# Coda-Research-Group/LearnedMetricIndex

Hardware: AMD Instinct MI355X
Metric: queries/sec @ recall@10, 768-d 10M index, 10k query batch (higher is better)
Workload: dtype f16 prefilter (f32 accumulate) + f32 exact re-rank; outputs identical to the all-f32 path

## Files before the change

### include/lmi_hip.h

```cpp
#ifndef LMI_HIP_H
#define LMI_HIP_H

#include <stdint.h>

#ifdef __cplusplus
extern "C" {
#endif

#define LMI_ABI_VERSION 1
#define LMI_API __attribute__((visibility("default")))
#define LMI_METRIC_IP 0
#define LMI_METRIC_L2 1
#define LMI_K_PER_BUCKET 10
#define LMI_MAX_K 64
#define LMI_MAX_LAYERS 8

typedef struct lmi_index lmi_index;

enum {
    LMI_T_INFERENCE = 0,
    LMI_T_ROUTE = 1,
    LMI_T_SCAN = 2,
    LMI_T_MERGE = 3,
    LMI_T_TOTAL = 4,
// ... 31 lines not shown
LMI_API int lmi_set_metric(lmi_index *h, int metric);

LMI_API int lmi_buckets_begin(lmi_index *h, int64_t N, int d, int L, const int64_t *labels,
                      const uint32_t *ids, const uint8_t *owned);
LMI_API int lmi_buckets_add_rows(lmi_index *h, const float *rows, int64_t row0, int64_t nrows, int on_device);
LMI_API int lmi_buckets_add_owned_rows(lmi_index *h, const float *rows, const int64_t *index, int64_t nrows,
                               int on_device);
LMI_API int lmi_buckets_end(lmi_index *h);
LMI_API int lmi_buckets_insert(lmi_index *h, const float *rows, const int64_t *labels, const uint32_t *ids, int64_t nrows,
                               int on_device, int64_t *n_stored);
LMI_API int lmi_buckets_delete(lmi_index *h, const uint32_t *ids, int64_t n, int64_t *n_removed);
LMI_API int lmi_bucket_sizes(lmi_index *h, int64_t *sizes);
LMI_API int lmi_bucket_read(lmi_index *h, int bucket, float *rows, uint32_t *ids);

LMI_API int lmi_mlp_topk(lmi_index *h, const float *queries_nav, int nq, int nb, int32_t *bucket_order,
                 float *logits, int on_device);

LMI_API int lmi_mlp_proba(lmi_index *h, const float *queries_nav, int nq, float *probs, int32_t *classes,
                  int on_device);

LMI_API int lmi_scan_topk(lmi_index *h, const float *queries_search, int nq, const int32_t *bucket_order,
                  int nb, int k, float *dists, uint32_t *ids, uint32_t *keys, int on_device);

LMI_API int lmi_search(lmi_index *h, const float *queries_nav, const float *queries_search, int nq, int nb,
               int k, float *dists, uint32_t *ids, uint32_t *keys, int32_t *bucket_order,
               int on_device);

LMI_API int lmi_merge_gathered(lmi_index *h, const float *gathered_dists, const uint32_t *gathered_ids,
                       const uint32_t *gathered_keys, int world, int64_t world_stride, int nq,
                       int kout, float *dists, uint32_t *ids, int on_device);

LMI_API int lmi_copy_out(lmi_index *h, void *dst, const void *src, int64_t bytes);
LMI_API int lmi_copy_out_many(lmi_index *h, int n, void *const *dst, const void *const *src, const int64_t *bytes);
LMI_API int lmi_pipeline_submit(lmi_index *h, void *s_in, void *s_nav, void *s_run, void *ev_in, void *ev_nav, void *ev_out,
                                const float *qn_host, const float *qs_host, float *qn_dev, float *qs_dev, int nq, int nb, int k,
                                float *dists_out, uint32_t *ids_out, int32_t *bo_dev, int32_t *bo_host, int overlap_nav);

LMI_API int lmi_comm_unique_id(void *id128);
LMI_API int lmi_comm_init(lmi_index *h, int rank, int world, const void *id128, void **comm);
LMI_API int lmi_comm_destroy(void *comm);
LMI_API int lmi_allgather_merge(lmi_index *h, void *comm, int rank, int world, const float *local_dists,
                        const uint32_t *local_ids, const uint32_t *local_keys, int nq, int kout, float *dists,
                        uint32_t *ids);

LMI_API int lmi_knn_ip(int device, const float *xq, int64_t nq, const float *xb, int64_t nb, int d, int k,
               float *D, int64_t *I);

LMI_API int lmi_timings(lmi_index *h, float *ms );
LMI_API int lmi_timings_reset(lmi_index *h);
LMI_API int lmi_set_timing(lmi_index *h, int level);
LMI_API int lmi_timings_mean(lmi_index *h, float *ms , int *n_calls );
LMI_API int lmi_scan_stats(lmi_index *h, double *flops, int64_t *pairs, int64_t *items);
LMI_API int lmi_set_prefilter(lmi_index *h, int on);
LMI_API int lmi_clone_view(lmi_index *h, lmi_index **out);
LMI_API int lmi_debug_peek(lmi_index *h, const char *name, void *dst, int64_t bytes);
LMI_API int lmi_prefilter_stats(lmi_index *h, int *active, int64_t *survivors, int64_t *fallbacks);
LMI_API int lmi_set_chunk_rows(lmi_index *h, int rows);
LMI_API int lmi_workspace_bytes(lmi_index *h, int nq, int n_buckets, int64_t *bytes);

LMI_API int lmi_debug_emit_all(lmi_index *h, int on);
LMI_API int lmi_debug_read_candidates(lmi_index *h, int64_t slot, int cap, uint32_t *rows, float *shat,
                              int *count, float *eps2, float *qscale, float *xscale);
LMI_API int lmi_debug_layout(lmi_index *h, int32_t *rb_start, int32_t *cap_rb, int64_t *n_rb_total, int64_t *alloc_rb,
                             int64_t *counters);

#ifdef __cplusplus
}
#endif
#endif
```

### learnedmetricindex_amd/_capi.py

```python
from __future__ import annotations

import ctypes
import os
from typing import Optional, Sequence

import numpy as np

_HERE = os.path.dirname(os.path.abspath(__file__))
LIB_PATH = os.environ.get("LMI_LIB") or os.path.join(_HERE, "liblmi_hip.so")
K_PER_BUCKET = 10
T_INFERENCE, T_ROUTE, T_SCAN, T_MERGE, T_TOTAL, T_PF_SAMPLE, T_PF_EMIT, T_RESCORE, T_FALLBACK, T_CLOCK_MHZ, T_COUNT = (
    0, 1, 2, 3, 4, 5, 6, 7, 8, 9, 12)

_lib = None

_f32p = ctypes.POINTER(ctypes.c_float)
_i32p = ctypes.POINTER(ctypes.c_int32)
_i64p = ctypes.POINTER(ctypes.c_int64)
_u32p = ctypes.POINTER(ctypes.c_uint32)
_u8p = ctypes.POINTER(ctypes.c_uint8)
_vp = ctypes.c_void_p

SIGNATURES = {
    "lmi_abi_version": (ctypes.c_int, []),
    "lmi_last_error": (ctypes.c_char_p, []),
    "lmi_build_info": (ctypes.c_char_p, []),
    "lmi_create": (ctypes.c_int, [ctypes.c_int, ctypes.POINTER(_vp)]),
    "lmi_destroy": (ctypes.c_int, [_vp]),
    "lmi_set_stream": (ctypes.c_int, [_vp, _vp]),
    "lmi_set_mlp": (ctypes.c_int, [_vp, ctypes.c_int, _i32p, ctypes.POINTER(_vp), ctypes.POINTER(_vp)]),
    "lmi_set_fused_mlp": (ctypes.c_int, [_vp, ctypes.c_int]),
    "lmi_set_metric": (ctypes.c_int, [_vp, ctypes.c_int]),
    "lmi_nav_set_model": (ctypes.c_int, [_vp, ctypes.c_int, ctypes.c_int, _i32p, ctypes.POINTER(_vp), ctypes.POINTER(_vp)]),
    "lmi_nav_set_tree": (ctypes.c_int, [_vp, ctypes.c_int, _vp, _vp, _vp]),
    "lmi_nav_order": (ctypes.c_int, [_vp, _vp, ctypes.c_int, ctypes.c_int, _vp, _vp, ctypes.c_int]),
    "lmi_search_tree": (ctypes.c_int, [_vp, _vp, _vp, ctypes.c_int, ctypes.c_int, ctypes.c_int, _vp, _vp, _vp, _vp, _vp, ctypes.c_int]),
    "lmi_buckets_begin": (ctypes.c_int, [_vp, ctypes.c_int64, ctypes.c_int, ctypes.c_int, _vp, _vp, _vp]),
    "lmi_buckets_add_rows": (ctypes.c_int, [_vp, _vp, ctypes.c_int64, ctypes.c_int64, ctypes.c_int]),
    "lmi_buckets_add_owned_rows": (ctypes.c_int, [_vp, _vp, _vp, ctypes.c_int64, ctypes.c_int]),
    "lmi_buckets_end": (ctypes.c_int, [_vp]),
    "lmi_buckets_insert": (ctypes.c_int, [_vp, _vp, _vp, _vp, ctypes.c_int64, ctypes.c_int, _i64p]),
    "lmi_buckets_delete": (ctypes.c_int, [_vp, _vp, ctypes.c_int64, _i64p]),
    "lmi_bucket_sizes": (ctypes.c_int, [_vp, _vp]),
    "lmi_mlp_topk": (ctypes.c_int, [_vp, _vp, ctypes.c_int, ctypes.c_int, _vp, _vp, ctypes.c_int]),
    "lmi_mlp_proba": (ctypes.c_int, [_vp, _vp, ctypes.c_int, _vp, _vp, ctypes.c_int]),
    "lmi_scan_topk": (ctypes.c_int, [_vp, _vp, ctypes.c_int, _vp, ctypes.c_int, ctypes.c_int, _vp, _vp, _vp,
                                     ctypes.c_int]),
    "lmi_search": (ctypes.c_int, [_vp, _vp, _vp, ctypes.c_int, ctypes.c_int, ctypes.c_int, _vp, _vp, _vp, _vp,
                                  ctypes.c_int]),
    "lmi_merge_gathered": (ctypes.c_int, [_vp, _vp, _vp, _vp, ctypes.c_int, ctypes.c_int64, ctypes.c_int,
                                          ctypes.c_int, _vp, _vp, ctypes.c_int]),
    "lmi_comm_unique_id": (ctypes.c_int, [_vp]),
    "lmi_comm_init": (ctypes.c_int, [_vp, ctypes.c_int, ctypes.c_int, _vp, ctypes.POINTER(_vp)]),
    "lmi_comm_destroy": (ctypes.c_int, [_vp]),
    "lmi_allgather_merge": (ctypes.c_int, [_vp, _vp, ctypes.c_int, ctypes.c_int, _vp, _vp, _vp, ctypes.c_int, ctypes.c_int,
                                           _vp, _vp]),
    "lmi_bucket_read": (ctypes.c_int, [_vp, ctypes.c_int, _vp, _vp]),
    "lmi_copy_out": (ctypes.c_int, [_vp, _vp, _vp, ctypes.c_int64]),
    "lmi_copy_out_many": (ctypes.c_int, [_vp, ctypes.c_int, _vp, _vp, _vp]),
    "lmi_pipeline_submit": (ctypes.c_int, [_vp] * 7 + [_vp, _vp, _vp, _vp, ctypes.c_int, ctypes.c_int, ctypes.c_int, _vp, _vp, _vp, _vp, ctypes.c_int]),
    "lmi_knn_ip": (ctypes.c_int, [ctypes.c_int, _vp, ctypes.c_int64, _vp, ctypes.c_int64, ctypes.c_int,
                                  ctypes.c_int, _vp, _vp]),
    "lmi_timings": (ctypes.c_int, [_vp, _vp]),
    "lmi_timings_reset": (ctypes.c_int, [_vp]),
    "lmi_set_timing": (ctypes.c_int, [_vp, ctypes.c_int]),
    "lmi_timings_mean": (ctypes.c_int, [_vp, _vp, ctypes.POINTER(ctypes.c_int)]),
    "lmi_scan_stats": (ctypes.c_int, [_vp, ctypes.POINTER(ctypes.c_double), _i64p, _i64p]),
    "lmi_set_chunk_rows": (ctypes.c_int, [_vp, ctypes.c_int]),
    "lmi_workspace_bytes": (ctypes.c_int, [_vp, ctypes.c_int, ctypes.c_int, _i64p]),
    "lmi_set_prefilter": (ctypes.c_int, [_vp, ctypes.c_int]),
    "lmi_debug_peek": (ctypes.c_int, [_vp, ctypes.c_char_p, _vp, ctypes.c_int64]),
    "lmi_clone_view": (ctypes.c_int, [_vp, ctypes.POINTER(_vp)]),
    "lmi_prefilter_stats": (ctypes.c_int, [_vp, ctypes.POINTER(ctypes.c_int), _i64p, _i64p]),
    "lmi_debug_emit_all": (ctypes.c_int, [_vp, ctypes.c_int]),
    "lmi_debug_read_candidates": (ctypes.c_int, [_vp, ctypes.c_int64, ctypes.c_int, _vp, _vp,
                                                 ctypes.POINTER(ctypes.c_int), _f32p, _f32p, _f32p]),
    "lmi_debug_layout": (ctypes.c_int, [_vp, _vp, _vp, _i64p, _i64p, _vp]),
}


class LmiError(RuntimeError):
    """Raised when a C-ABI call returns non-zero (message from lmi_last_error)."""


def lib() -> ctypes.CDLL:
    global _lib
    if _lib is None:
        if not os.path.exists(LIB_PATH):
            raise LmiError(
                f"{LIB_PATH} is missing: build it with learnedmetricindex_amd/csrc/build.sh "
                "(or __graft_entry__.build()); there is no CPU fallback")
        import torch

        L = ctypes.CDLL(LIB_PATH)
        for name, (res, args) in SIGNATURES.items():
            fn = getattr(L, name)
            fn.restype = res
            fn.argtypes = args
        if L.lmi_abi_version() != 1:
            raise LmiError("liblmi_hip.so ABI version mismatch")
        _lib = L
    return _lib


def _check(rc: int) -> None:
    if rc != 0:
        raise LmiError(lib().lmi_last_error().decode("utf-8", "replace"))


def _ptr(a) -> int:
    if a is None:
        return None
    if isinstance(a, np.ndarray):
        return a.ctypes.data
    return a.data_ptr()


def _np(a, dtype) -> np.ndarray:
    return np.ascontiguousarray(a, dtype=dtype)


class Index:

    METRICS = {"ip": 0, "l2": 1}

    def __init__(self, device: int = 0, chunk_rows: Optional[int] = None, prefilter: Optional[bool] = None,
                 metric: str = "ip"):
        self._h = _vp()
        _check(lib().lmi_create(int(device), ctypes.byref(self._h)))
        self.device = int(device)
        self.n_classes = None
        self.d_nav = None
        self.d = None
        self.L = None
        if chunk_rows is not None:
            _check(lib().lmi_set_chunk_rows(self._h, int(chunk_rows)))
        if prefilter is None and os.environ.get("LMI_PREFILTER") is not None:
            prefilter = os.environ["LMI_PREFILTER"] not in ("0", "off", "false")
        if prefilter is not None:
            self.set_prefilter(prefilter)
        if metric != "ip":
            _check(lib().lmi_set_metric(self._h, self.METRICS[metric]))
        self.metric = metric

    def close(self) -> None:
        for c in getattr(self, "_views", []):
            c.close()
        self._views = []
        if getattr(self, "_h", None) is not None and self._h:
            lib().lmi_destroy(self._h)
            self._h = None

    def clone_view(self) -> "Index":
        v = Index.__new__(Index)
        v._h = _vp()
        _check(lib().lmi_clone_view(self._h, ctypes.byref(v._h)))
        for a in ("device", "n_classes", "d_nav", "d", "L", "N", "metric"):
            setattr(v, a, getattr(self, a, None))
        v._views = []
        v._parent = self
        self.__dict__.setdefault("_views", []).append(v)
        return v

    def __del__(self):
        try:
            self.close()
        except Exception:
            pass

    def set_prefilter(self, on) -> None:
        _check(lib().lmi_set_prefilter(self._h, int(on)))

    def debug_peek(self, name: str, nbytes: int) -> np.ndarray:
        out = np.empty(nbytes, np.uint8)
        _check(lib().lmi_debug_peek(self._h, name.encode(), out.ctypes.data_as(_vp), nbytes))
        return out

    def prefilter_stats(self):
        a = ctypes.c_int(0)
        sv = ctypes.c_int64(0)
        fb = ctypes.c_int64(0)
        _check(lib().lmi_prefilter_stats(self._h, ctypes.byref(a), ctypes.byref(sv), ctypes.byref(fb)))
        return bool(a.value), sv.value, fb.value

    def debug_emit_all(self, on: bool) -> None:
        _check(lib().lmi_debug_emit_all(self._h, 1 if on else 0))

    def debug_read_candidates(self, slot: int, cap: int = 1024):
        rows = np.empty(cap, dtype=np.uint32)
        shat = np.empty(cap, dtype=np.float32)
        cnt = ctypes.c_int(0)
        e2, qs, xs = ctypes.c_float(0), ctypes.c_float(0), ctypes.c_float(0)
        _check(lib().lmi_debug_read_candidates(self._h, int(slot), int(cap), _ptr(rows), _ptr(shat), ctypes.byref(cnt),
                                               ctypes.byref(e2), ctypes.byref(qs), ctypes.byref(xs)))
        n = max(0, min(cnt.value, cap))
        return rows[:n], shat[:n], cnt.value, e2.value, qs.value, xs.value

    def debug_layout(self) -> dict:
        rb_start = np.empty(self.L + 1, dtype=np.int32)
        cap_rb = np.empty(self.L, dtype=np.int32)
        counters = np.empty(4, dtype=np.int64)
        n_rb, alloc = ctypes.c_int64(0), ctypes.c_int64(0)
        _check(lib().lmi_debug_layout(self._h, _ptr(rb_start), _ptr(cap_rb), ctypes.byref(n_rb), ctypes.byref(alloc),
                                      _ptr(counters)))
        return dict(rb_start=rb_start, cap_rb=cap_rb, n_rb_total=n_rb.value, alloc_rb=alloc.value, counters=counters)

    def set_stream(self, stream_ptr: int) -> None:
        _check(lib().lmi_set_stream(self._h, _vp(stream_ptr)))

    def set_mlp(self, layers: Sequence) -> None:
        Ws = [_np(W, np.float32) for W, _ in layers]
        bs = [_np(b, np.float32) for _, b in layers]
        dims = [Ws[0].shape[1]] + [W.shape[0] for W in Ws]
        for i, (W, b) in enumerate(zip(Ws, bs)):
            assert W.shape == (dims[i + 1], dims[i]) and b.shape == (dims[i + 1],)
        n = len(Ws)
        dims_c = (ctypes.c_int32 * (n + 1))(*dims)
        Wp = (_vp * n)(*[W.ctypes.data for W in Ws])
        bp = (_vp * n)(*[b.ctypes.data for b in bs])
        _check(lib().lmi_set_mlp(self._h, n, dims_c, Wp, bp))
        self.d_nav, self.n_classes = dims[0], dims[-1]

    def set_fused_mlp(self, mode: int) -> None:
        _check(lib().lmi_set_fused_mlp(self._h, int(mode)))

# ... 261 lines not shown
```

### learnedmetricindex_amd/csrc/lmi_front.h

```cpp
#pragma once
#include "lmi_prefilter.h"

namespace lmi {

constexpr int FR_THREADS = 1024, FR_WAVES = FR_THREADS / 64;
constexpr int FR_MAX_L = 512;
constexpr int FR_MAX_SLOTS = 1 << 17;
constexpr int FR_SLICE_G = 48;
constexpr int FR_LIST = 512;
constexpr int FP_THREADS = 512, FP_WAVES = FP_THREADS / 64;
constexpr int FR_MAX_D = 64 * 4 * 8;
static_assert(FR_SLICE_G % 2 == 0, "the 16 x 32 fragment shape pairs k16-groups");

struct FrontParams {
    const int* bucket_order;
    int nq, nb, L;
    const unsigned* epoch_dev;
    unsigned long long* gran;
    int* cb_bucket;
    int* colmap;
    RouteArrays R;
    FillRanges Z;
    const float* q;
    int d, KG16, f16x16;
    float* qnorm; float* qdelta; float* qscale;
    uint4* qfrag16;
    int* slot_col;
    float* eps2;
    const unsigned* bnorm; const unsigned* bdelta;
    float* pf_bound;
    long long ncols;
    int bound_rows;
    unsigned long long* ts;
    unsigned long long* dbg;
};
#define FR_DBG(base, slot) do { if (P.dbg && threadIdx.x == 0 && (base) >= 0) P.dbg[(base) + (slot)] = wall_clock64(); } while (0)

__host__ __device__ inline int fr_lpad(int L) { return (L + 3) & ~3; }
__host__ __device__ inline size_t fr_route_lds(int L) { return (size_t)fr_lpad(L) * 4; }
__host__ __device__ inline size_t fr_pack_lds(int L, int KG16) {
    const size_t pack = (size_t)(KG16 < FR_SLICE_G ? KG16 : FR_SLICE_G) * 1024, grp = (size_t)fr_lpad(L) * 12 + route_group_lds(L) + 16;
    return pack > grp ? pack : grp;
}

template <bool VEC>
__device__ __forceinline__ void fr_load8(const float* __restrict__ row, int d, int k0, bool ok, float (&v)[8]) {
    if constexpr (VEC) {
        const int kk = ok ? k0 : 0;
        const float4 lo = *reinterpret_cast<const float4*>(row + kk), hi = *reinterpret_cast<const float4*>(row + kk + 4);
        v[0] = ok ? lo.x : 0.0f; v[1] = ok ? lo.y : 0.0f; v[2] = ok ? lo.z : 0.0f; v[3] = ok ? lo.w : 0.0f;
        v[4] = ok ? hi.x : 0.0f; v[5] = ok ? hi.y : 0.0f; v[6] = ok ? hi.z : 0.0f; v[7] = ok ? hi.w : 0.0f;
    } else {
#pragma unroll
        for (int j = 0; j < 8; ++j) {
            const bool in = ok && k0 + j < d;
            const float x = row[in ? k0 + j : 0];
            v[j] = in ? x : 0.0f;
        }
    }
}

template <int NB, int U>
struct FrChunk {
    int id[U][NB];
    int rows[U][NB];
    __device__ __forceinline__ void load(const int* __restrict__ bo, int q_first, int lane, int q_end) {
#pragma unroll
        for (int u = 0; u < U; ++u) {
            const int q = q_first + 64 * u + lane;
            const int qq = min(q, q_end - 1);
#pragma unroll
            for (int r = 0; r < NB; ++r) id[u][r] = bo[(size_t)qq * NB + r];
        }
#pragma unroll
        for (int u = 0; u < U; ++u) {
            const bool live = q_first + 64 * u + lane < q_end;
#pragma unroll
            for (int r = 0; r < NB; ++r) id[u][r] = live ? id[u][r] : -1;
        }
    }
    __device__ __forceinline__ void sizes(const int* nbr, int L) {
// ... 207 lines not shown
        return;
    }
    const unsigned long long alloc = P.gran[P.L];
    const int n_cb = (unsigned)(alloc >> 32) == epoch_v ? (int)(unsigned)alloc : 0;
    const int cb = bid - 1;
    if (cb >= n_cb) return;
    char* stage = fp_smem;
    const int b = P.cb_bucket[cb];
    const int d = P.d, KG16 = P.KG16;
    const int nchunk_row = (d + 7) >> 3;
    constexpr int CPW = 64 / GS;
    constexpr int NCOL = (32 + FP_WAVES * CPW - 1) / (FP_WAVES * CPW);
    const int gl = lane % GS, sub = lane / GS;
    const float xn = __uint_as_float(P.bnorm[b]), dx = __uint_as_float(P.bdelta[b]);
    const float guard = norm_guard(d);
    {
        const float ninf = -INFINITY;
        const float4 f4 = make_float4(ninf, ninf, ninf, ninf);
        const long long per_row = (long long)n_cb * 8;
        const long long total = (long long)P.bound_rows * per_row;
        const long long lo = (long long)cb * P.bound_rows * 8, hi = min(total, lo + (long long)P.bound_rows * 8);
        for (long long i = lo + tid; i < hi; i += FP_THREADS) {
            const long long row = i / per_row, x = i - row * per_row;
            *reinterpret_cast<float4*>(P.pf_bound + (size_t)row * (size_t)P.ncols + (size_t)x * 4) = f4;
        }
    }
    float v[NCOL][CP][8];
    int qi[NCOL];
#pragma unroll
    for (int c = 0; c < NCOL; ++c) {
        const int cc = w * CPW + sub + c * FP_WAVES * CPW;
        qi[c] = cc < 32 ? P.colmap[(size_t)cb * 32 + cc] : -1;
    }
#pragma unroll
    for (int c = 0; c < NCOL; ++c) {
        const float* row = P.q + (size_t)(qi[c] < 0 ? 0 : qi[c]) * d;
#pragma unroll
        for (int i = 0; i < CP; ++i) {
            const int j = gl + GS * i;
            fr_load8<VEC>(row, d, 8 * j, qi[c] >= 0 && j < nchunk_row, v[c][i]);
        }
    }
#pragma unroll
    for (int c = 0; c < NCOL; ++c) {
        const int cc = w * CPW + sub + c * FP_WAVES * CPW;
        float mx = 0.0f;
#pragma unroll
        for (int i = 0; i < CP; ++i)
#pragma unroll
            for (int t = 0; t < 8; ++t) mx = fmaxf(mx, fabsf(v[c][i][t]));
#pragma unroll
        for (int o = GS / 2; o > 0; o >>= 1) mx = fmaxf(mx, __shfl_xor(mx, o));
        const float s = scale_of_max(__float_as_uint(mx));
        float acc = 0.0f, dl = 0.0f;
#pragma unroll
        for (int i = 0; i < CP; ++i)
#pragma unroll
            for (int t = 0; t < 8; ++t) {
                const float vs = v[c][i][t] * s;
                const float e = (float)(_Float16)vs - vs;
                acc += vs * vs;
                dl += e * e;
                v[c][i][t] = vs;
            }
#pragma unroll
        for (int o = GS / 2; o > 0; o >>= 1) { acc += __shfl_xor(acc, o); dl += __shfl_xor(dl, o); }
        if (gl == 0 && cc < 32) {
            const size_t col = (size_t)cb * 32 + cc;
            if (qi[c] >= 0) {
                const float qn = sqrtf(acc) * guard, dq = sqrtf(dl) * guard;
                P.qnorm[qi[c]] = qn; P.qdelta[qi[c]] = dq; P.qscale[qi[c]] = s;
                const float e = dq * (xn + dx) + qn * dx + 4.0f * (float)(KG16 * 16) * 5.96046448e-8f * (qn + dq) * (xn + dx);
                P.eps2[col] = 2.0f * e * 1.001f;
            } else {
                P.eps2[col] = 0.0f;
            }
        }
    }
    for (int g0 = 0; g0 < KG16; g0 += FR_SLICE_G) {
        const int gs = min(FR_SLICE_G, KG16 - g0);
#pragma unroll
        for (int c = 0; c < NCOL; ++c) {
            const int cc = w * CPW + sub + c * FP_WAVES * CPW;
#pragma unroll
            for (int i = 0; i < CP; ++i) {
                const int j = gl + GS * i;
                const int g = j >> 1, hh = j & 1;
                if (cc < 32 && g >= g0 && g < g0 + gs) {
                    half8 h;
#pragma unroll
                    for (int t = 0; t < 8; ++t) h[t] = (_Float16)v[c][i][t];
                    int slot;
                    if (P.f16x16) {
                        slot = (2 * (g >> 1) + (cc >> 4) - g0) * 64 + 16 * (2 * (g & 1) + hh) + (cc & 15);
                        slot ^= ((slot >> 4) & 3) | (((slot >> 7) & 3) << 2);
                    } else {
                        slot = (g - g0) * 64 + hh * 32 + cc;
                    }
                    *reinterpret_cast<uint4*>(stage + (size_t)slot * 16) = *reinterpret_cast<uint4*>(&h);
                }
            }
        }
        __syncthreads();
        uint4* dst = P.qfrag16 + ((size_t)cb * (size_t)KG16 + (size_t)g0) * 64;
        for (int i = tid; i < gs * 64; i += FP_THREADS) {
            const int src = P.f16x16 ? (i ^ (((i >> 4) & 3) | (((i >> 7) & 3) << 2))) : i;
            dst[i] = *reinterpret_cast<const uint4*>(stage + (size_t)src * 16);
        }
        __syncthreads();
    }
}
#undef FR_DBG

}
```

### learnedmetricindex_amd/csrc/lmi_hip.hip

```cpp
#include "lmi_kernels.h"
#include "lmi_prefilter.h"
#include "lmi_pass2.h"
#include "lmi_pass2_small.h"
#include "lmi_mlp_fused.h"
#include "lmi_rescore.h"
#include "lmi_front.h"
#include "lmi_tail.h"
#include "lmi_mutate.h"

#include <algorithm>
#include <cfloat>
#include <cstdarg>
#include <cstdio>
#include <cstring>
#include <dlfcn.h>
#include <mutex>
#include <string>
#include <vector>

#include "lmi_hip.h"
#include <rccl/rccl.h>

using namespace lmi;

// ... 57 lines not shown
}

struct lmi_index {
    int device = 0;
    hipStream_t stream = nullptr;
    hipStream_t side = nullptr;
    hipEvent_t side_fork = nullptr, side_join = nullptr;
    int num_cus = 256;
    int scan_blocks_per_cu = 2;

    int n_layers = 0;
    std::vector<int> dims;
    std::vector<int> n_rb;
    std::vector<int> KG;
    std::vector<DevBuf> Wf;
    std::vector<DevBuf> bias;

    struct NodeModel {
        int n_layers = 0;
        std::vector<int> dims, n_rb, KG;
        std::vector<DevBuf> Wf, bias;
    };
    std::vector<NodeModel> node_models;
    int fused_mlp = 1;
    bool desc_dirty = true;
    DevBuf d_models;
    int fm_s0 = 0, fm_s1 = 0, fm_act0 = 0, fm_lds = 0, fm_logits_lds = 0;
    bool fm_ok = false;
    std::vector<int> h_child_offset, h_child_model, h_child_bucket;
    DevBuf d_child_offset, d_child_model, d_child_bucket;
    bool tree_set = false;
    DevBuf gather_send, gather_recv;
    DevBuf pq_prob, pq_ent, pq_len, nav_len, nav_slab, nav_ent, nav_count, nav_colq, nav_active;

    bool building = false, built = false;
    int64_t N = 0;
    int d = 0, L = 0, KGs = 0;
    int metric = 0, d_user = 0;
    DevBuf aug_rows, q_aug, qn2;
    int chunk_rows = 2048;
    bool chunk_rows_auto = true;
    int64_t n_rb_total = 0;
    std::vector<int> h_nb_rows, h_rb_start, h_nch;
    DevBuf slab, ids_slab, pos, d_nb_rows, d_rb_start, d_nch;
    int64_t rows_added = 0, owned_total = 0;
    bool indexed_ingest = false;
    DevBuf stage;
    bool prefilter = true;
    bool pf_hw_ok = false;
    bool have16 = false;
    int KG16 = 0;
    int dp = 0;
    DevBuf slab16, rowmajor, xscale, xmaxbits, bnorm, bdelta, qdelta;
    DevBuf qnorm, qscale, qfrag16, eps2, cand_cnt, cand_row, cand_s, fallback, pf_bound, nkeep, surv_row, rs_flag, rs_active;
    DevBuf grp_scratch;
    bool ps_wide = false;
    int ps_force_wide = -1;
    int n_nonempty = 1;
    DevBuf x_log, x_ext, x_off, fb_list;
    unsigned x_cap = 0;
    DevBuf redo;
    size_t stamps_off = 0;
    bool pf_small = true;
    bool pf_redo = true;
    bool rescore_streamed = true;
    int last_nslots = 0, last_nb = 0;
    long long last_ncols = 0;
    bool last_fast = false;
    bool pf_qbound = true;
    bool pf_primary = true;
    bool debug_emit_all = false;

    DevBuf act[2], xfrag, logits, order, q_nav, q_srch;
    DevBuf m, cb_start, item_base, part_base, stats, head, slot_local, slot_col, colmap, qfrag, grp, col_thr;
    DevBuf part_score, part_row, rank_d, rank_id, out_d, out_id, out_key;
    static constexpr int EV_RING = 128;
    hipEvent_t ev_ring[EV_RING][10] = {};
    bool valid_ring[EV_RING][10] = {};
    int ev_cur = 0;
    int timing_level = 2;
    long long ev_calls = 0;
    hipEvent_t* ev = ev_ring[0];
    bool* ev_valid = valid_ring[0];
    long long h_stats[4] = {0, 0, 0, 0};
    bool stats_pending = false;
    DevBuf ts_ring;
    unsigned ts_mask[EV_RING] = {};
    unsigned long long* ts_set = nullptr;
    double wall_khz = 100000.0;
    DevBuf fr_dbg;
    DevBuf cb_alloc, cb_bucket;
    unsigned* h_oflag = nullptr;
    int overflow_armed = 0;
    bool fr_bump_pending = false;
    int use_tail = 1;
    bool graded_chunks = true;
    int chunk_lvl_rows[3] = {0, 0, 0};
    float chunk_frac[2] = {0.16f, 0.05f};
    bool use_front = true;

    std::vector<int> h_cap_rb;
    std::vector<unsigned char> h_owned;
    std::vector<unsigned char> h_any;
    lmi_index* parent = nullptr;
    int live_clones = 0;
    int64_t mut_paths[4] = {0, 0, 0, 0};
    DevBuf mut_pos, mut_ids, mut_list, mut_keep, mut_src, mut_stage, mut_word;
};

static int frag16x16(const lmi_index* h) { return (h->pf_small && h->KG16 <= PS_MAXKG) ? 0 : 1; }


static int set_dev(lmi_index* h) {
    HIPCHK(hipSetDevice(h->device));
    return 0;
}

extern "C" LMI_API int lmi_abi_version(void) { return LMI_ABI_VERSION; }
#ifndef LMI_SOURCE_SHA16
#define LMI_SOURCE_SHA16 "unknown"
#endif
#define LMI_STR2(x) #x
#define LMI_STR(x) LMI_STR2(x)
extern "C" LMI_API const char* lmi_build_info(void) {
    return "src=" LMI_SOURCE_SHA16 " p2_waves=" LMI_STR(LMI_P2_WAVES) " p2_bring=" LMI_STR(LMI_P2_BR) " pf_cap=" LMI_STR(LMI_PF_CAP);
}
extern "C" LMI_API const char* lmi_last_error(void) { return g_err.c_str(); }

extern "C" LMI_API int lmi_create(int device, lmi_index** out) {
    if (!out) return fail("lmi_create: out is NULL");
    int ndev = 0;
    HIPCHK(hipGetDeviceCount(&ndev));
    if (device < 0 || device >= ndev) return fail("lmi_create: device %d out of range (%d devices)", device, ndev);
    HIPCHK(hipSetDevice(device));
    hipDeviceProp_t prop;
    HIPCHK(hipGetDeviceProperties(&prop, device));
    if (std::string(prop.gcnArchName).rfind("gfx950", 0) != 0)
        return fail("lmi_create: device %d is %s; this library is built for gfx950 only", device, prop.gcnArchName);
    lmi_index* h = new lmi_index();
    h->device = device;
    h->num_cus = prop.multiProcessorCount;
    HIPCHK(hipFuncSetAttribute(reinterpret_cast<const void*>(&route_group_kernel<false>),
                               hipFuncAttributeMaxDynamicSharedMemorySize, 160 * 1024 - 256));
    int occ = 0;
    HIPCHK(hipOccupancyMaxActiveBlocksPerMultiprocessor(&occ, scan_kernel, 256, SCAN_LDS));
    h->scan_blocks_per_cu = std::max(1, std::min(occ, RB == 1 ? 2 : 1));
    {
        static std::mutex mu;
        static int cached = -1;
        std::lock_guard<std::mutex> lock(mu);
        if (cached < 0) {
            int* d_ok = nullptr;
            int ok = 0;
            HIPCHK(hipMalloc(&d_ok, sizeof(int)));
            pf_selftest_kernel<<<1, 64>>>(d_ok);
            HIPCHK(hipGetLastError());
            HIPCHK(hipMemcpy(&ok, d_ok, sizeof(int), hipMemcpyDeviceToHost));
            HIPCHK(hipFree(d_ok));
            cached = ok;
        }
        h->pf_hw_ok = cached == 1;
        if (!h->pf_hw_ok) h->prefilter = false;
    }
// ... 4 lines not shown
    if (const char* e = getenv("LMI_PF_PRIMARY")) h->pf_primary = e[0] && e[0] != '0';
    if (const char* e = getenv("LMI_PS_WIDE")) h->ps_force_wide = e[0] == '1' ? 1 : e[0] == '0' ? 0 : -1;
    if (const char* e = getenv("LMI_FRONT")) h->use_front = !(e[0] == '0');
    if (const char* e = getenv("LMI_P2_GRADED")) h->graded_chunks = !(e[0] == '0');
    if (const char* e = getenv("LMI_P2_CHUNKS")) (void)sscanf(e, "%d,%d,%d", &h->chunk_lvl_rows[0], &h->chunk_lvl_rows[1], &h->chunk_lvl_rows[2]);
    if (const char* e = getenv("LMI_P2_CHUNK_FRAC")) (void)sscanf(e, "%f,%f", &h->chunk_frac[0], &h->chunk_frac[1]);
    if (const char* e = getenv("LMI_TAIL")) h->use_tail = e[0] == '0' ? 0 : e[0] == '2' ? 2 : 1;
    if (const char* e = getenv("LMI_FR_DEBUG")) { if (e[0] == '1') { CHK(h->fr_dbg.reserve(256)); HIPCHK(hipMemset(h->fr_dbg.p, 0, 256)); } }
    {
        int khz = 0;
        if (hipDeviceGetAttribute(&khz, hipDeviceAttributeWallClockRate, device) == hipSuccess && khz > 0) h->wall_khz = (double)khz;
    }
#define LMI_PS_ATTR(K) \
    HIPCHK(hipFuncSetAttribute(reinterpret_cast<const void*>(&pass2_small_kernel<K, false, false>), hipFuncAttributeMaxDynamicSharedMemorySize, ps_lds_bytes(K, false))); \
    HIPCHK(hipFuncSetAttribute(reinterpret_cast<const void*>(&pass2_small_kernel<K, true, false>), hipFuncAttributeMaxDynamicSharedMemorySize, ps_lds_bytes(K, false))); \
    if constexpr (ps_has_wide(K)) { \
        HIPCHK(hipFuncSetAttribute(reinterpret_cast<const void*>(&pass2_small_kernel<K, false, ps_has_wide(K)>), hipFuncAttributeMaxDynamicSharedMemorySize, ps_lds_bytes(K, true))); \
        HIPCHK(hipFuncSetAttribute(reinterpret_cast<const void*>(&pass2_small_kernel<K, true, ps_has_wide(K)>), hipFuncAttributeMaxDynamicSharedMemorySize, ps_lds_bytes(K, true))); \
    }
    LMI_PS_ATTR(1) LMI_PS_ATTR(2) LMI_PS_ATTR(3) LMI_PS_ATTR(4) LMI_PS_ATTR(5) LMI_PS_ATTR(6) LMI_PS_ATTR(7) LMI_PS_ATTR(8)
#undef LMI_PS_ATTR
    HIPCHK(hipFuncSetAttribute(reinterpret_cast<const void*>(&rescore_kernel<1, false>), hipFuncAttributeMaxDynamicSharedMemorySize, 160 * 1024));
    HIPCHK(hipFuncSetAttribute(reinterpret_cast<const void*>(&rescore_kernel<1, true>), hipFuncAttributeMaxDynamicSharedMemorySize, RC_SMALL_LDS_CAP));
    HIPCHK(hipFuncSetAttribute(reinterpret_cast<const void*>(&rescore_kernel<2, false>), hipFuncAttributeMaxDynamicSharedMemorySize, 160 * 1024));
    HIPCHK(hipFuncSetAttribute(reinterpret_cast<const void*>(&rescore_kernel<2, true>), hipFuncAttributeMaxDynamicSharedMemorySize, RC_SMALL_LDS_CAP));
    HIPCHK(hipFuncSetAttribute(reinterpret_cast<const void*>(&rescore_kernel<3, false>), hipFuncAttributeMaxDynamicSharedMemorySize, 160 * 1024));
    HIPCHK(hipFuncSetAttribute(reinterpret_cast<const void*>(&rescore_kernel<3, true>), hipFuncAttributeMaxDynamicSharedMemorySize, RC_SMALL_LDS_CAP));
    HIPCHK(hipFuncSetAttribute(reinterpret_cast<const void*>(&rescore_kernel<4, false>), hipFuncAttributeMaxDynamicSharedMemorySize, 160 * 1024));
    HIPCHK(hipFuncSetAttribute(reinterpret_cast<const void*>(&rescore_kernel<4, true>), hipFuncAttributeMaxDynamicSharedMemorySize, RC_SMALL_LDS_CAP));
#define LMI_TL_ATTR(GV) \
    HIPCHK(hipFuncSetAttribute(reinterpret_cast<const void*>(&tail_kernel<GV>), hipFuncAttributeMaxDynamicSharedMemorySize, RC_SMALL_LDS_CAP));
    LMI_TL_ATTR(1) LMI_TL_ATTR(2) LMI_TL_ATTR(3) LMI_TL_ATTR(4)
#undef LMI_TL_ATTR
    *out = h;
    return 0;
}

extern "C" LMI_API int lmi_destroy(lmi_index* h) {
    if (!h) return 0;
    (void)hipSetDevice(h->device);
    (void)hipStreamSynchronize(h->stream);
    if (h->parent) h->parent->live_clones--;
    if (h->side) {
        (void)hipStreamSynchronize(h->side);
        (void)hipStreamDestroy(h->side);
        (void)hipEventDestroy(h->side_fork);
        (void)hipEventDestroy(h->side_join);
    }
    for (auto& b : h->Wf) b.release();
    for (auto& b : h->bias) b.release();
    DevBuf* bufs[] = {&h->slab, &h->ids_slab, &h->pos, &h->d_nb_rows, &h->d_rb_start, &h->d_nch, &h->stage,
                      &h->act[0], &h->act[1], &h->xfrag, &h->logits, &h->order, &h->q_nav, &h->q_srch, &h->m,
                      &h->cb_start, &h->item_base, &h->part_base, &h->stats, &h->head, &h->slot_local,
                      &h->slot_col, &h->colmap, &h->qfrag, &h->grp, &h->col_thr, &h->slab16, &h->rowmajor, &h->xscale, &h->xmaxbits, &h->bnorm, &h->bdelta, &h->qdelta, &h->qnorm, &h->qscale, &h->qfrag16, &h->eps2, &h->cand_cnt, &h->cand_row, &h->cand_s, &h->fallback, &h->pf_bound, &h->nkeep, &h->redo, &h->part_score, &h->part_row, &h->rank_d,
                      &h->rank_id, &h->out_d, &h->out_id, &h->out_key, &h->x_log, &h->x_ext, &h->x_off, &h->fb_list, &h->grp_scratch, &h->ts_ring, &h->fr_dbg, &h->cb_alloc, &h->cb_bucket};
    for (DevBuf* b : bufs) b->release();
    if (h->h_oflag) (void)hipHostFree(h->h_oflag);
    for (auto& m : h->node_models) { for (auto& b : m.Wf) b.release(); for (auto& b : m.bias) b.release(); }
    DevBuf* nav[] = {&h->d_models, &h->d_child_offset, &h->d_child_model, &h->d_child_bucket, &h->pq_prob, &h->pq_ent, &h->pq_len, &h->surv_row, &h->rs_flag, &h->rs_active, &h->gather_send, &h->gather_recv, &h->aug_rows, &h->q_aug, &h->qn2,
                     &h->nav_len, &h->nav_slab, &h->nav_ent, &h->nav_count, &h->nav_colq, &h->nav_active,
                     &h->mut_pos, &h->mut_ids, &h->mut_list, &h->mut_keep, &h->mut_src, &h->mut_stage, &h->mut_word};
    for (DevBuf* b : nav) b->release();
    for (int r = 0; r < lmi_index::EV_RING; ++r)
        for (int i = 0; i < 10; ++i)
            if (h->ev_ring[r][i]) (void)hipEventDestroy(h->ev_ring[r][i]);
    delete h;
    return 0;
}

static int build_descs(lmi_index* h);

extern "C" LMI_API int lmi_clone_view(lmi_index* h, lmi_index** out) {
    if (!h || !out) return fail("lmi_clone_view: NULL argument");
    if (h->building) return fail("lmi_clone_view: the parent's index is being built");
    CHK(set_dev(h));
    CHK(build_descs(h));
    HIPCHK(hipStreamSynchronize(h->stream));
    lmi_index* c = new lmi_index(*h);
    c->stream = nullptr; c->side = nullptr; c->side_fork = nullptr; c->side_join = nullptr;
    for (auto& b : c->Wf) b.borrow();
    for (auto& b : c->bias) b.borrow();
    for (auto& m : c->node_models) { for (auto& b : m.Wf) b.borrow(); for (auto& b : m.bias) b.borrow(); }
    DevBuf* shared[] = {&c->d_models, &c->d_child_offset, &c->d_child_model, &c->d_child_bucket, &c->slab, &c->ids_slab, &c->pos,
                        &c->d_nb_rows, &c->d_rb_start, &c->d_nch, &c->slab16, &c->rowmajor, &c->xscale, &c->xmaxbits, &c->bnorm, &c->bdelta};
    for (DevBuf* b : shared) b->borrow();
    DevBuf* own[] = {&c->gather_send, &c->gather_recv, &c->pq_prob, &c->pq_ent, &c->pq_len, &c->nav_len, &c->nav_slab, &c->nav_ent,
                     &c->nav_count, &c->nav_colq, &c->nav_active, &c->aug_rows, &c->q_aug, &c->qn2, &c->stage, &c->qdelta, &c->qnorm,
                     &c->qscale, &c->qfrag16, &c->eps2, &c->cand_cnt, &c->cand_row, &c->cand_s, &c->fallback, &c->pf_bound, &c->nkeep, &c->redo,
                     &c->surv_row, &c->rs_flag, &c->rs_active, &c->act[0], &c->act[1], &c->xfrag, &c->logits, &c->order, &c->q_nav,
                     &c->q_srch, &c->m, &c->cb_start, &c->item_base, &c->part_base, &c->stats, &c->head, &c->slot_local, &c->slot_col,
                     &c->colmap, &c->qfrag, &c->grp, &c->col_thr, &c->part_score, &c->part_row, &c->rank_d, &c->rank_id, &c->out_d,
                     &c->out_id, &c->out_key, &c->x_log, &c->x_ext, &c->x_off, &c->fb_list, &c->grp_scratch, &c->ts_ring, &c->fr_dbg, &c->cb_alloc, &c->cb_bucket,
                     &c->mut_pos, &c->mut_ids, &c->mut_list, &c->mut_keep, &c->mut_src, &c->mut_stage, &c->mut_word};
    for (DevBuf* b : own) b->forget();
    c->ts_set = nullptr;
    memset(c->ts_mask, 0, sizeof(c->ts_mask));
    c->h_oflag = nullptr;
    c->overflow_armed = 0;
    c->x_cap = 0;
    memset(c->ev_ring, 0, sizeof(c->ev_ring));
    memset(c->valid_ring, 0, sizeof(c->valid_ring));
    c->ev_cur = 0; c->ev_calls = 0;
    c->ev = c->ev_ring[0]; c->ev_valid = c->valid_ring[0];
    c->stats_pending = false;
    c->last_nslots = 0; c->last_fast = false;
    c->parent = h;
    c->live_clones = 0;
    h->live_clones++;
    *out = c;
    return 0;
}

extern "C" LMI_API int lmi_set_stream(lmi_index* h, void* s) {
    if (!h) return fail("lmi_set_stream: NULL handle");
    h->stream = reinterpret_cast<hipStream_t>(s);
    return 0;
}

extern "C" LMI_API int lmi_set_chunk_rows(lmi_index* h, int rows) {
    if (!h) return fail("lmi_set_chunk_rows: NULL handle");
    if (rows < P2_TILE_ROWS || rows % P2_TILE_ROWS) return fail("lmi_set_chunk_rows: rows must be a positive multiple of %d", P2_TILE_ROWS);
    if (h->building || h->built) return fail("lmi_set_chunk_rows: must be called before lmi_buckets_begin");
    h->chunk_rows = rows;
    h->chunk_rows_auto = false;
    return 0;
}

extern "C" LMI_API int lmi_set_metric(lmi_index* h, int metric) {
    if (!h) return fail("lmi_set_metric: NULL handle");
    if (metric != LMI_METRIC_IP && metric != LMI_METRIC_L2) return fail("lmi_set_metric: unknown metric %d", metric);
    if ((h->built || h->building) && metric != h->metric) return fail("lmi_set_metric: the metric is fixed once lmi_buckets_begin has run");
    h->metric = metric;
    return 0;
}

extern "C" LMI_API int lmi_set_prefilter(lmi_index* h, int on) {
    if (!h) return fail("lmi_set_prefilter: NULL handle");
    if ((h->built || h->building) && (on != 0) != h->prefilter)
        return fail("lmi_set_prefilter: the mode is fixed once lmi_buckets_begin has run (the index is stored differently)");
    if (on && !h->pf_hw_ok) return fail("lmi_set_prefilter: fp16 subnormal self-test failed on this device; the prefilter's error bound does not hold");
    if (on != 0 && on != 1) return fail("lmi_set_prefilter: mode %d unknown (0: all-f32 scan, 1: fp16 prefilter + exact re-rank)", on);
    h->prefilter = on != 0;
    return 0;
}

static int pack_from_host(lmi_index* h, const float* src, int rows, int cols, int n_rb, int KG, DevBuf& dst) {
    CHK(h->stage.reserve((size_t)rows * cols * sizeof(float)));
    HIPCHK(hipMemcpyAsync(h->stage.p, src, (size_t)rows * cols * sizeof(float), hipMemcpyHostToDevice, h->stream));
    CHK(dst.reserve((size_t)n_rb * KG * 1024));
    long long total = (long long)n_rb * 32 * KG;
    pack_gather_kernel<<<cdiv(total, 256), 256, 0, h->stream>>>(h->stage.as<float>(), cols, nullptr, rows,
                                                               (long long)n_rb * 32, KG, dst.as<float4>());
    HIPCHK(hipGetLastError());
    HIPCHK(hipStreamSynchronize(h->stream));
    return 0;
}

static int pack_model(lmi_index* h, const char* who, int n_layers, const int* dims, const float* const* W, const float* const* b,
                      std::vector<int>& o_dims, std::vector<int>& o_nrb, std::vector<int>& o_KG, std::vector<DevBuf>& o_W,
                      std::vector<DevBuf>& o_b) {
    if (n_layers < 1 || n_layers > LMI_MAX_LAYERS) return fail("%s: n_layers %d out of range", who, n_layers);
    for (int i = 0; i <= n_layers; ++i)
        if (dims[i] < 1) return fail("%s: dims[%d] = %d", who, i, dims[i]);
    for (auto& x : o_W) x.release();
    for (auto& x : o_b) x.release();
    o_dims.assign(dims, dims + n_layers + 1);
    o_nrb.assign(n_layers, 0);
    o_KG.assign(n_layers, 0);
    o_W.assign(n_layers, DevBuf());
    o_b.assign(n_layers, DevBuf());
    for (int i = 0; i < n_layers; ++i) {
        o_nrb[i] = cdiv(dims[i + 1], 32);
        o_KG[i] = (i == 0) ? cdiv(dims[0], 8) : o_nrb[i - 1] * 4;
        if (!W[i] || !b[i]) return fail("%s: NULL weight/bias for layer %d", who, i);
        CHK(pack_from_host(h, W[i], dims[i + 1], dims[i], o_nrb[i], o_KG[i], o_W[i]));
        std::vector<float> bp((size_t)o_nrb[i] * 32, 0.0f);
        std::copy(b[i], b[i] + dims[i + 1], bp.begin());
        CHK(o_b[i].reserve(bp.size() * sizeof(float)));
        HIPCHK(hipMemcpy(o_b[i].p, bp.data(), bp.size() * sizeof(float), hipMemcpyHostToDevice));
    }
    return 0;
}

extern "C" LMI_API int lmi_set_mlp(lmi_index* h, int n_layers, const int* dims, const float* const* W,
                           const float* const* b) {
    if (!h) return fail("lmi_set_mlp: NULL handle");
    CHK(set_dev(h));
    h->desc_dirty = true;
// ... 235 lines not shown
            augment_copy_kernel<<<cdiv((long long)n * h->d, 256), 256, 0, h->stream>>>(src, h->d_user, h->d, n, h->aug_rows.as<float>());
            HIPCHK(hipGetLastError());
            augment_norm_kernel<<<cdiv(n, 256), 256, 0, h->stream>>>(src, h->d_user, h->d, n, h->aug_rows.as<float>(), nullptr);
            HIPCHK(hipGetLastError());
            src = h->aug_rows.as<float>();
        }
        if (h->prefilter) {
            long long total = (long long)n * h->d;
            scatter_rows_kernel<<<cdiv(total, 256), 256, 0, h->stream>>>(src, h->d, pos, row0 + off, idx, (long long)n_total, n,
                                                                        h->rowmajor.as<float>(), h->dp);
        } else {
            long long total = (long long)n * h->KGs;
            pack_scatter_kernel<<<cdiv(total, 256), 256, 0, h->stream>>>(src, h->d, pos, row0 + off, idx, (long long)n_total, n,
                                                                        h->KGs, h->slab.as<float4>());
        }
        HIPCHK(hipGetLastError());
        if (!on_device) HIPCHK(hipStreamSynchronize(h->stream));
    }
    return 0;
}

extern "C" LMI_API int lmi_buckets_add_rows(lmi_index* h, const float* rows, int64_t row0, int64_t nrows, int on_device) {
    if (!h || !h->building) return fail("lmi_buckets_add_rows: call lmi_buckets_begin first");
    if (h->indexed_ingest) return fail("lmi_buckets_add_rows: this build already uses lmi_buckets_add_owned_rows");
    if (row0 < 0 || nrows < 0 || row0 + nrows > h->N) return fail("lmi_buckets_add_rows: rows [%lld,%lld) outside [0,%lld)", (long long)row0, (long long)(row0 + nrows), (long long)h->N);
    if (nrows == 0) return 0;
    CHK(add_rows_impl(h, rows, row0, nullptr, nrows, on_device, h->pos.as<int>(), h->N));
    h->rows_added += nrows;
    return 0;
}

extern "C" LMI_API int lmi_buckets_add_owned_rows(lmi_index* h, const float* rows, const int64_t* index, int64_t nrows,
                                          int on_device) {
    if (!h || !h->building) return fail("lmi_buckets_add_owned_rows: call lmi_buckets_begin first");
    if (h->rows_added > 0 && !h->indexed_ingest) return fail("lmi_buckets_add_owned_rows: this build already uses lmi_buckets_add_rows");
    if (nrows < 0 || (nrows > 0 && (!rows || !index))) return fail("lmi_buckets_add_owned_rows: bad arguments");
    if (!on_device)
        for (int64_t i = 0; i < nrows; ++i)
            if (index[i] < 0 || index[i] >= h->N) return fail("lmi_buckets_add_owned_rows: index[%lld] = %lld outside [0,%lld)", (long long)i, (long long)index[i], (long long)h->N);
    h->indexed_ingest = true;
    if (nrows == 0) return 0;
    CHK(add_rows_impl(h, rows, 0, index, nrows, on_device, h->pos.as<int>(), h->N));
    h->rows_added += nrows;
    return 0;
}

static int prefilter_images(lmi_index* h) {
    h->KG16 = (h->pf_small && cdiv(h->d, 16) <= PS_MAXKG) ? (int)cdiv(h->d, 16) : (int)rup(cdiv(h->d, 16), PF_STAGE_G);
    const long long n_rows = (long long)h->n_rb_total * 32;
    CHK(h->xmaxbits.reserve(16));
    CHK(h->xscale.reserve(16));
    CHK(h->bnorm.reserve((size_t)h->L * 4));
    CHK(h->bdelta.reserve((size_t)h->L * 4));
    CHK(h->slab16.reserve((size_t)h->n_rb_total * h->KG16 * 1024 + 8192));
    HIPCHK(hipMemsetAsync(h->xmaxbits.p, 0, 16, h->stream));
    HIPCHK(hipMemsetAsync(h->bnorm.p, 0, (size_t)h->L * 4, h->stream));
    HIPCHK(hipMemsetAsync(h->bdelta.p, 0, (size_t)h->L * 4, h->stream));
    absmax_kernel<<<h->num_cus * 8, 256, 0, h->stream>>>(h->rowmajor.as<float>(), n_rows * h->dp, h->xmaxbits.as<unsigned>());
    HIPCHK(hipGetLastError());
    make_scale_kernel<<<1, 1, 0, h->stream>>>(h->xmaxbits.as<unsigned>(), h->xscale.as<float>());
    HIPCHK(hipGetLastError());
    const long long total = n_rows * h->KG16 * 2;
    convert16_kernel<<<cdiv(total, 256), 256, 0, h->stream>>>(h->rowmajor.as<float>(), h->d, h->dp, n_rows, h->KG16,
                                                             h->xscale.as<float>(), h->slab16.as<uint4>(), frag16x16(h));
    HIPCHK(hipGetLastError());
    dim3 g(64, h->L);
    bucket_norm_kernel<<<g, 256, 0, h->stream>>>(h->rowmajor.as<float>(), h->d, h->dp, h->d_rb_start.as<int>(),
                                                h->d_nb_rows.as<int>(), h->xscale.as<float>(), h->bnorm.as<unsigned>(),
                                                h->bdelta.as<unsigned>());
    HIPCHK(hipGetLastError());
    HIPCHK(hipStreamSynchronize(h->stream));
    h->have16 = true;
    return 0;
}

extern "C" LMI_API int lmi_buckets_end(lmi_index* h) {
    if (!h || !h->building) return fail("lmi_buckets_end: call lmi_buckets_begin first");
    const int64_t expect = h->indexed_ingest ? h->owned_total : h->N;
    if (h->rows_added != expect) return fail("lmi_buckets_end: %lld of %lld rows were added", (long long)h->rows_added, (long long)expect);
    CHK(set_dev(h));
    HIPCHK(hipStreamSynchronize(h->stream));
    h->pos.release();
    h->have16 = false;
    if (h->prefilter && h->n_rb_total > 0) CHK(prefilter_images(h));
    h->building = false;
    h->built = true;
    return 0;
}

extern "C" LMI_API int lmi_bucket_sizes(lmi_index* h, int64_t* sizes) {
    if (!h || !(h->built || h->building)) return fail("lmi_bucket_sizes: no buckets");
    for (int b = 0; b < h->L; ++b) sizes[b] = h->h_nb_rows[b];
    return 0;
}

extern "C" LMI_API int lmi_bucket_read(lmi_index* h, int bucket, float* rows, uint32_t* ids) {
    if (!h || !h->built) return fail("lmi_bucket_read: the bucket index is not built");
    if (bucket < 0 || bucket >= h->L) return fail("lmi_bucket_read: bucket %d outside [0,%d)", bucket, h->L);
    const int64_t n = h->h_nb_rows[bucket];
    if (n == 0) return 0;
    CHK(set_dev(h));
    const int64_t p0 = (int64_t)h->h_rb_start[bucket] * 32;
    const int du = h->d_user;
    if (rows && h->prefilter) {
        HIPCHK(hipMemcpy2DAsync(rows, (size_t)du * 4, h->rowmajor.as<float>() + (size_t)p0 * h->dp, (size_t)h->dp * 4, (size_t)du * 4, (size_t)n,
                                hipMemcpyDeviceToHost, h->stream));
    } else if (rows) {
        CHK(h->stage.reserve((size_t)n * du * 4));
        long long total = n * cdiv(du, 8);
        unpack_kernel<<<cdiv(total, 256), 256, 0, h->stream>>>(h->slab.as<float4>(), h->KGs, p0, n, du, h->stage.as<float>());
        HIPCHK(hipGetLastError());
        HIPCHK(hipMemcpyAsync(rows, h->stage.p, (size_t)n * du * 4, hipMemcpyDeviceToHost, h->stream));
    }
    if (ids) HIPCHK(hipMemcpyAsync(ids, h->ids_slab.as<uint32_t>() + p0, (size_t)n * 4, hipMemcpyDeviceToHost, h->stream));
    HIPCHK(hipStreamSynchronize(h->stream));
    return 0;
}

namespace {
struct SlabImage { DevBuf* buf; size_t rb_bytes, extra; };
int slab_images(lmi_index* h, SlabImage* im) {
    int n = 0;
// ... 173 lines not shown
    HIPCHK(hipGetLastError());
    CHK(add_rows_impl(h, rows, 0, nullptr, nrows, on_device, h->mut_pos.as<int>(), nrows));
    std::vector<int> list((size_t)L * 5);
    int* l_b = list.data();
    int* l_row0 = l_b + L;
    int* l_nrows = l_row0 + L;
    int* l_rb0 = l_nrows + L;
    int* l_nrb = l_rb0 + L;
    int nr = 0, max_rows = 0, max_rb = 0;
    for (int b = 0; b < L; ++b) {
        if (!add[b]) continue;
        const int r0 = start[b] * 32 + h->h_nb_rows[b], r1 = r0 + (int)add[b];
        l_b[nr] = b;
        l_row0[nr] = r0;
        l_nrows[nr] = r1 - r0;
        l_rb0[nr] = r0 / 32;
        l_nrb[nr] = cdiv(r1, 32) - r0 / 32;
        max_rows = std::max(max_rows, l_nrows[nr]);
        max_rb = std::max(max_rb, l_nrb[nr]);
        ++nr;
        h->h_nb_rows[b] += (int)add[b];
        h->h_any[b] = 1;
    }
    for (int64_t i = 0; i < nrows; ++i) h->h_any[labels[i]] = 1;
    h->N += nrows;
    CHK(mut_derive(h));
    if (h->prefilter) {
        HIPCHK(hipMemcpyAsync(h->mut_list.p, list.data(), list.size() * 4, hipMemcpyHostToDevice, h->stream));
        const int* d_list = h->mut_list.as<int>();
        bool rescale = !h->have16;
        if (!rescale) {
            HIPCHK(hipMemsetAsync(h->mut_word.p, 0, 4, h->stream));
            dim3 g(std::min(64, cdiv((long long)max_rows * h->d, 256)), nr);
            absmax_ranges_kernel<<<g, 256, 0, h->stream>>>(h->rowmajor.as<float>(), h->d, h->dp, d_list + L, d_list + 2 * L, h->mut_word.as<unsigned>());
            HIPCHK(hipGetLastError());
            unsigned mbits = 0;
            float sc = 1.0f;
            HIPCHK(hipMemcpyAsync(&mbits, h->mut_word.p, 4, hipMemcpyDeviceToHost, h->stream));
            HIPCHK(hipMemcpyAsync(&sc, h->xscale.p, 4, hipMemcpyDeviceToHost, h->stream));
            HIPCHK(hipStreamSynchronize(h->stream));
            float m;
            memcpy(&m, &mbits, 4);
            rescale = !(m * sc < 1.0f);
        }
        if (rescale) {
            CHK(prefilter_images(h));
        } else {
            dim3 gc(std::min(1024, cdiv((long long)max_rb * 32 * h->KG16 * 2, 256)), nr);
            convert16_ranges_kernel<<<gc, 256, 0, h->stream>>>(h->rowmajor.as<float>(), h->d, h->dp, d_list + 3 * L, d_list + 4 * L, h->KG16,
                                                               h->xscale.as<float>(), h->slab16.as<uint4>(), frag16x16(h));
            HIPCHK(hipGetLastError());
            dim3 gn(std::min(64, cdiv(max_rows, 256)), nr);
            bucket_norm_ranges_kernel<<<gn, 256, 0, h->stream>>>(h->rowmajor.as<float>(), h->d, h->dp, d_list, d_list + L, d_list + 2 * L,
                                                                  h->xscale.as<float>(), h->bnorm.as<unsigned>(), h->bdelta.as<unsigned>());
            HIPCHK(hipGetLastError());
        }
    }
    HIPCHK(hipStreamSynchronize(h->stream));
    for (int i = 0; i < 4; ++i) h->mut_paths[i] += paths[i];
    if (n_stored) *n_stored = stored;
    return 0;
}

extern "C" LMI_API int lmi_buckets_delete(lmi_index* h, const uint32_t* ids, int64_t n, int64_t* n_removed) {
    CHK(mut_check(h, "lmi_buckets_delete"));
    if (n < 0 || (n > 0 && !ids)) return fail("lmi_buckets_delete: bad arguments");
    if (n_removed) *n_removed = 0;
    if (n == 0 || h->owned_total == 0) return 0;
    std::vector<uint32_t> del(ids, ids + n);
    std::sort(del.begin(), del.end());
    del.erase(std::unique(del.begin(), del.end()), del.end());
    const int L = h->L;
    const int64_t slab_rows = h->n_rb_total * 32;
    CHK(set_dev(h));
    CHK(h->mut_ids.reserve(del.size() * 4));
    CHK(h->mut_keep.reserve((size_t)slab_rows * 4));
    CHK(h->mut_src.reserve((size_t)slab_rows * 4));
    CHK(h->mut_word.reserve((size_t)L * 4));
    CHK(h->mut_list.reserve((size_t)L * 4 * 4 + (size_t)L * 8 + 16));
    CHK(h->mut_pos.reserve((size_t)L * 5 * 4));
    HIPCHK(hipStreamSynchronize(h->stream));
    HIPCHK(hipMemcpyAsync(h->mut_ids.p, del.data(), del.size() * 4, hipMemcpyHostToDevice, h->stream));
    HIPCHK(hipMemsetAsync(h->mut_word.p, 0, (size_t)L * 4, h->stream));
    int max_n = 0;
    for (int b = 0; b < L; ++b) max_n = std::max(max_n, h->h_nb_rows[b]);
    mark_deleted_kernel<<<dim3(std::max(1, std::min(64, cdiv(max_n, 256))), L), 256, 0, h->stream>>>(
        h->ids_slab.as<uint32_t>(), h->d_rb_start.as<int>(), h->d_nb_rows.as<int>(), h->mut_ids.as<uint32_t>(), (int)del.size(),
        h->mut_keep.as<int>(), h->mut_word.as<int>());
    HIPCHK(hipGetLastError());
    std::vector<int> cnt(L);
    HIPCHK(hipMemcpyAsync(cnt.data(), h->mut_word.p, (size_t)L * 4, hipMemcpyDeviceToHost, h->stream));
    HIPCHK(hipStreamSynchronize(h->stream));
    std::vector<int> hit, span;
    int64_t removed = 0, max_span = 0;
    for (int b = 0; b < L; ++b)
        if (cnt[b] > 0) {
            hit.push_back(b);
            span.push_back(cdiv(h->h_nb_rows[b], 32) * 32);
            max_span = std::max<int64_t>(max_span, span.back());
            removed += cnt[b];
        }
    if (removed == 0) return 0;
    const int nh = (int)hit.size();
    const bool frag = !h->prefilter;
    const int pitch = frag ? h->d : h->dp;
    const int64_t budget = std::max<int64_t>(max_span, (1ll << 30) / ((int64_t)pitch * 4));
    std::vector<int> gb, gspan, gfirst;
// ... 27 lines not shown
    const int* d_hit = h->mut_list.as<int>();
    const long long* d_goff = reinterpret_cast<const long long*>(h->mut_list.as<char>() + off_bytes);
    compact_map_kernel<<<nh, CM_THREADS, 0, h->stream>>>(d_hit, d_hit + nh, h->d_rb_start.as<int>(), h->d_nb_rows.as<int>(), h->mut_keep.as<int>(),
                                                        h->mut_src.as<int>());
    HIPCHK(hipGetLastError());
    const int per_row = frag ? cdiv(pitch, 8) : pitch / 4;
    for (size_t g = 0; g + 1 < gfirst.size(); ++g) {
        const int i0 = gfirst[g], ng = gfirst[g + 1] - i0;
        int64_t gmax = 0;
        for (int i = i0; i < i0 + ng; ++i) gmax = std::max<int64_t>(gmax, gspan[i]);
        dim3 gg(std::max(1, std::min(1024, cdiv(gmax * per_row, 256))), ng);
        if (frag)
            gather_compact_kernel<true><<<gg, 256, 0, h->stream>>>(h->slab.as<float>(), pitch, h->KGs, h->ids_slab.as<uint32_t>(), d_hit + 2 * nh + i0,
                                                                  d_goff + i0, d_hit + 3 * nh + i0, h->d_rb_start.as<int>(), h->mut_src.as<int>(), st_rows, st_ids);
        else
            gather_compact_kernel<false><<<gg, 256, 0, h->stream>>>(h->rowmajor.as<float>(), pitch, 0, h->ids_slab.as<uint32_t>(), d_hit + 2 * nh + i0,
                                                                   d_goff + i0, d_hit + 3 * nh + i0, h->d_rb_start.as<int>(), h->mut_src.as<int>(), st_rows, st_ids);
        HIPCHK(hipGetLastError());
        for (int i = i0; i < i0 + ng; ++i) {
            const int b = gb[i];
            const size_t p0 = (size_t)h->h_rb_start[b] * 32;
            const long long sp = gspan[i], off = goff[i];
            if (frag) {
                pack_gather_kernel<<<cdiv(sp * h->KGs, 256), 256, 0, h->stream>>>(st_rows + off * pitch, pitch, nullptr, (int)sp, sp, h->KGs,
                                                                                  h->slab.as<float4>() + (p0 >> 5) * h->KGs * 64);
                HIPCHK(hipGetLastError());
            } else {
                HIPCHK(hipMemcpyAsync(h->rowmajor.as<float>() + p0 * pitch, st_rows + off * pitch, (size_t)sp * pitch * 4, hipMemcpyDeviceToDevice, h->stream));
            }
            HIPCHK(hipMemcpyAsync(h->ids_slab.as<uint32_t>() + p0, st_ids + off, (size_t)sp * 4, hipMemcpyDeviceToDevice, h->stream));
        }
    }
    std::vector<int> old_nrb(nh);
    for (int i = 0; i < nh; ++i) {
        const int b = hit[i];
        old_nrb[i] = span[i] / 32;
        h->h_nb_rows[b] -= cnt[b];
        if (h->h_nb_rows[b] == 0) h->h_any[b] = 0;
    }
    h->N -= removed;
    CHK(mut_derive(h));
    std::vector<int> list((size_t)5 * nh);
    if (h->prefilter && h->have16) {
        for (int i = 0; i < nh; ++i) {
            const int b = hit[i];
            list[i] = b;
            list[nh + i] = h->h_rb_start[b] * 32;
            list[2 * nh + i] = h->h_nb_rows[b];
            list[3 * nh + i] = h->h_rb_start[b];
            list[4 * nh + i] = old_nrb[i];
        }
        HIPCHK(hipMemcpyAsync(h->mut_pos.p, list.data(), list.size() * 4, hipMemcpyHostToDevice, h->stream));
        const int* d_list = h->mut_pos.as<int>();
        reset_norms_kernel<<<cdiv(nh, 256), 256, 0, h->stream>>>(d_list, nh, h->bnorm.as<unsigned>(), h->bdelta.as<unsigned>());
        HIPCHK(hipGetLastError());
        int max_rb = 0, max_rows = 1;
        for (int i = 0; i < nh; ++i) { max_rb = std::max(max_rb, old_nrb[i]); max_rows = std::max(max_rows, list[2 * nh + i]); }
        dim3 gc(std::max(1, std::min(1024, cdiv((long long)max_rb * 32 * h->KG16 * 2, 256))), nh);
        convert16_ranges_kernel<<<gc, 256, 0, h->stream>>>(h->rowmajor.as<float>(), h->d, h->dp, d_list + 3 * nh, d_list + 4 * nh, h->KG16,
                                                           h->xscale.as<float>(), h->slab16.as<uint4>(), frag16x16(h));
        HIPCHK(hipGetLastError());
        dim3 gn(std::min(64, cdiv(max_rows, 256)), nh);
        bucket_norm_ranges_kernel<<<gn, 256, 0, h->stream>>>(h->rowmajor.as<float>(), h->d, h->dp, d_list, d_list + nh, d_list + 2 * nh,
                                                              h->xscale.as<float>(), h->bnorm.as<unsigned>(), h->bdelta.as<unsigned>());
        HIPCHK(hipGetLastError());
    }
    HIPCHK(hipStreamSynchronize(h->stream));
    if (n_removed) *n_removed = removed;
    return 0;
}

static void begin_call(lmi_index* h) {
    h->ev_cur = (h->ev_cur + 1) % lmi_index::EV_RING;
    h->ev = h->ev_ring[h->ev_cur];
    h->ev_valid = h->valid_ring[h->ev_cur];
    for (int i = 0; i < 10; ++i) h->ev_valid[i] = false;
    ++h->ev_calls;
    h->ts_mask[h->ev_cur] = 0u;
    h->ts_set = nullptr;
    if (h->timing_level == 2) {
        if (!h->ts_ring.p && h->ts_ring.reserve((size_t)lmi_index::EV_RING * ST_COUNT * 8) != 0) return;
        h->ts_set = h->ts_ring.as<unsigned long long>() + (size_t)h->ev_cur * ST_COUNT;
    }
}
static unsigned long long* tsp(lmi_index* h, int idx) {
    if (!h->ts_set) return nullptr;
    h->ts_mask[h->ev_cur] |= 1u << idx;
    return h->ts_set + idx;
}
static int stamp_end(lmi_index* h, int idx) {
    if (unsigned long long* p = tsp(h, idx)) {
        stamp_kernel<<<1, 1, 0, h->stream>>>(p);
        HIPCHK(hipGetLastError());
    }
    return 0;
}

static int record(lmi_index* h, int i) {
    if (h->timing_level == 0 || h->timing_level == 2 || (h->timing_level == 1 && i != 0 && i != 1 && i != 4)) return 0;
    if (!h->ev[i]) HIPCHK(hipEventCreateWithFlags(&h->ev[i], hipEventDisableSystemFence));
    HIPCHK(hipEventRecord(h->ev[i], h->stream));
    h->ev_valid[i] = true;
    return 0;
}

static int input_ptr(lmi_index* h, const void* src, size_t bytes, int on_device, DevBuf& buf, const void** out) {
    if (on_device) { *out = src; return 0; }
    CHK(buf.reserve(bytes));
    HIPCHK(hipMemcpyAsync(buf.p, src, bytes, hipMemcpyHostToDevice, h->stream));
    *out = buf.p;
    return 0;
}

static int side_ensure(lmi_index* h) {
    if (!h->side) {
        HIPCHK(hipStreamCreateWithFlags(&h->side, hipStreamNonBlocking));
        HIPCHK(hipEventCreateWithFlags(&h->side_fork, hipEventDisableTiming));
// ... 233 lines not shown
    CHK(h->part_score.reserve((size_t)part_lists * KPB * 4));
    CHK(h->part_row.reserve((size_t)part_lists * KPB * 4));
    CHK(h->rank_d.reserve((size_t)nslots * KPB * 4));
    CHK(h->rank_id.reserve((size_t)nslots * KPB * 4));

    RouteArrays R;
    R.nb_rows = h->d_nb_rows.as<int>();
    R.nch = h->d_nch.as<int>();
    R.m = h->m.as<int>();
    R.m0 = R.m + L;
    R.cb_start = h->cb_start.as<int>();
    R.item_base = h->item_base.as<int>();
    R.part_base = h->part_base.as<long long>();
    R.stats = h->stats.as<long long>();
    R.grp_bucket = h->grp.as<int>();
    R.grp_base = R.grp_bucket + (size_t)NGRP * L;
    R.grp_n = R.grp_base + (size_t)NGRP * (L + 1);
    R.grp_total = R.grp_n + NGRP;
    R.grp_base1 = R.grp_total + NGRP;
    R.grp_total1 = R.grp_base1 + (size_t)NGRP * (L + 1);
    R.dbg = nullptr;
    const bool v2 = h->prefilter && h->have16;
    R.chunk_rb = h->chunk_rows / 32;
    R.chunk_rb_b = (v2 && h->graded_chunks) ? R.grp_total1 + NGRP : nullptr;
    {
        const int base = h->chunk_rows;
        int rows[3] = {base, base / 2, base / 4};
        if (h->pf_small && h->KG16 <= PS_MAXKG) rows[0] = 2 * base;
        for (int i = 0; i < 3; ++i) {
            if (h->chunk_lvl_rows[i] > 0) rows[i] = h->chunk_lvl_rows[i];
            rows[i] = std::max(P2_TILE_ROWS, rows[i] / P2_TILE_ROWS * P2_TILE_ROWS);
            R.chunk_lvl[i] = rows[i] / 32;
        }
        R.chunk_frac[0] = h->chunk_frac[0];
        R.chunk_frac[1] = h->chunk_frac[1];
    }
    h->ps_wide = false;
    if (v2 && h->pf_small && h->KG16 <= PS_MAXKG) {
        const double per_bucket = (double)nq * nb / std::max(1, std::min(h->n_nonempty, (int)std::min<long long>((long long)nq * nb, 1 << 30)));
        h->ps_wide = h->ps_force_wide >= 0 ? h->ps_force_wide != 0 : ps_use_wide(h->KG16, per_bucket);
    }
    R.tile_cb = !v2 ? 4 : (h->pf_small && h->KG16 <= PS_MAXKG) ? ps_tile_cb(h->KG16, h->ps_wide) : P2_MAXCB;
    R.sample_max = (v2 && h->pf_small && h->KG16 <= PF_SAMPLE_LOWD_KG) ? PF_SAMPLE_LOWD : PF_SAMPLE;
    R.sample_items = v2 ? 1 : 0;
    const bool qbound = v2 && h->pf_qbound && nb > 1 && kout <= KPB;
    R.primary_nb = (qbound && h->pf_primary) ? nb : 0;

    const size_t ncols = (size_t)ncb_bound * 32;
    FillRanges Z;
    Z.count = 0;
    bool fill_ok = true;
    auto fill = [&](void* ptr, long long words, unsigned value) { fill_ok = Z.add(ptr, words, value) && fill_ok; };
    const bool use_front = fast && h->use_front && L <= FR_MAX_L && nslots <= FR_MAX_SLOTS && h->d <= FR_MAX_D;
    if (!use_front) fill(h->m.p, 3ll * L, 0u);
    fill(h->head.p, 64, 0u);
    if (!use_front) fill(h->colmap.p, (long long)ncols, 0xFFFFFFFFu);
    fill(h->col_thr.p, (long long)ncols, 0xFF800000u );
    if (fast) {
        CHK(h->qnorm.reserve((size_t)nq * 4));
        CHK(h->qdelta.reserve((size_t)nq * 4));
        CHK(h->qscale.reserve((size_t)nq * 4));
        CHK(h->qfrag16.reserve((size_t)ncb_bound * h->KG16 * 1024 + 8192));
        CHK(h->eps2.reserve(ncols * 4));
        CHK(h->cand_cnt.reserve(ncols * 4));
        CHK(h->cand_row.reserve(ncols * PF_CAP * 4));
        CHK(h->cand_s.reserve(ncols * PF_CAP * 4));
        CHK(h->fallback.reserve((size_t)nslots * 4));
        CHK(h->nkeep.reserve((size_t)nslots * 4));
        const size_t bound_words = ncols * P2_NSL * 16;
        CHK(h->pf_bound.reserve(bound_words * 4 + 4096));
        if (!use_front) fill(h->pf_bound.p, (long long)bound_words, 0xFF800000u );
        fill(h->cand_cnt.p, (long long)ncols, 0u);
        fill(h->stats.as<long long>() + 2, 4, 0u);
        CHK(h->redo.reserve((size_t)(1 + L) * 4 + ncols));
        fill(h->redo.p, (long long)(1 + L) + (long long)((ncols + 3) / 4), 0u);
        CHK(h->fb_list.reserve((size_t)(8 + nslots) * 4));
        fill(h->fb_list.p, 8, 0u);
        if (h->x_cap == 0) {
            const size_t cap = (size_t)1 << LMI_PF_X_LOG2;
            CHK(h->x_log.reserve(cap * 16));
            CHK(h->x_ext.reserve(cap * 8));
            h->x_cap = (unsigned)cap;
        }
        CHK(h->x_off.reserve(ncols * 4));
        if (rescore_is_streamed(h)) {
            const int groups = nslots / rescore_group_size(nb), sub_cap = cdiv(groups, RC_SUB);
            CHK(h->rs_flag.reserve((size_t)groups * 4));
            CHK(h->rs_active.reserve((size_t)(RC_SUB + RC_SUB * sub_cap) * 4 + (size_t)(1 + groups) * 4));
            fill(h->rs_flag.p, groups, 0u);
            fill(h->rs_active.p, RC_SUB, 0u);
            fill(h->rs_active.as<int>() + RC_SUB + RC_SUB * sub_cap, 1, 0u);
        }
    }
    if (!fill_ok) return fail("internal: more than %d fill ranges queued (%s:%d)", FillRanges::MAXR, __FILE__, __LINE__);
    Z.ts = nullptr;
    if (!use_front) {
    Z.ts = tsp(h, ST_FRONT);
    fill_ranges_kernel<<<h->num_cus * 4, 256, 0, h->stream>>>(Z);
    HIPCHK(hipGetLastError());
    route_count_kernel<<<cdiv(nslots, 256), 256, 0, h->stream>>>(d_order, nslots, L, R, h->slot_local.as<int>());
    HIPCHK(hipGetLastError());
    route_scan_kernel<<<1, 256, 0, h->stream>>>(L, R);
    HIPCHK(hipGetLastError());
    CHK(side_fork(h));
    if (L <= ROUTE_MAX_BUCKETS) {
        route_group_kernel<false><<<1, 1024, route_group_lds(L), h->side>>>(L, R, nullptr);
    } else {
        CHK(h->grp_scratch.reserve(route_group_lds(L) + (size_t)L * 4));
        route_group_kernel<true><<<1, 1024, 0, h->side>>>(L, R, h->grp_scratch.as<char>());
    }
    HIPCHK(hipGetLastError());
    route_fill_kernel<<<cdiv(nslots, 256), 256, 0, h->stream>>>(d_order, h->slot_local.as<int>(), nslots, nb,
                                                               R.cb_start, R.m0, h->colmap.as<int>(), h->slot_col.as<int>());
    HIPCHK(hipGetLastError());
    }
    ScanParams S;
// ... 13 lines not shown
    S.grp_total = R.grp_total;
    S.part_base = R.part_base;
    S.head = h->head.as<unsigned>();
    S.col_thr = h->col_thr.as<float>();
    S.part_score = h->part_score.as<float>();
    S.part_row = h->part_row.as<unsigned>();
    S.ts_start = nullptr;
    S.ts_end_cell = nullptr;
    unsigned long long* const p2_end_cell = reinterpret_cast<unsigned long long*>(h->head.as<unsigned>() + 32);
    unsigned long long* const scan_end_cell = reinterpret_cast<unsigned long long*>(h->head.as<unsigned>() + 34);
    if (!fast) {
        long long total = ncb_bound * 32 * h->KGs;
        pack_gather_kernel<<<cdiv(total, 256), 256, 0, h->stream>>>(d_qs, h->d, h->colmap.as<int>(), nq, ncb_bound * 32,
                                                                   h->KGs, h->qfrag.as<float4>());
        HIPCHK(hipGetLastError());
        CHK(side_join(h));
        CHK(record(h, 2));
        S.ts_start = tsp(h, ST_SCAN0);
        if (S.ts_start) { S.ts_end_cell = scan_end_cell; (void)tsp(h, ST_SCAN1); }
        scan_kernel<<<h->num_cus * h->scan_blocks_per_cu, 256, SCAN_LDS, h->stream>>>(S);
        HIPCHK(hipGetLastError());
        CHK(record(h, 3));
    } else {
        if (use_front) {
            FrontParams A;
            A.bucket_order = d_order;
            A.nq = nq; A.nb = nb; A.L = L;
            if (!h->cb_alloc.p) {
                CHK(h->cb_alloc.reserve((size_t)(FR_MAX_L + 2) * 8));
                HIPCHK(hipMemsetAsync(h->cb_alloc.p, 0, (size_t)(FR_MAX_L + 2) * 8, h->stream));
                front_epoch_bump_kernel<<<1, 1, 0, h->stream>>>(reinterpret_cast<unsigned*>(h->cb_alloc.as<unsigned long long>() + FR_MAX_L + 1));
                HIPCHK(hipGetLastError());
            }
            CHK(h->cb_bucket.reserve((size_t)ncb_bound * 4));
            unsigned* const epoch_dev = reinterpret_cast<unsigned*>(h->cb_alloc.as<unsigned long long>() + FR_MAX_L + 1);
            if (h->fr_bump_pending) {
                front_epoch_bump_kernel<<<1, 1, 0, h->stream>>>(epoch_dev);
                HIPCHK(hipGetLastError());
            }
            h->fr_bump_pending = true;
            A.epoch_dev = epoch_dev;
            A.gran = h->cb_alloc.as<unsigned long long>();
            A.cb_bucket = h->cb_bucket.as<int>();
            A.colmap = h->colmap.as<int>();
            A.R = R;
            A.R.dbg = h->fr_dbg.as<unsigned long long>();
            A.Z = Z;
            A.q = d_qs;
            A.d = h->d; A.KG16 = h->KG16; A.f16x16 = frag16x16(h);
            A.qnorm = h->qnorm.as<float>(); A.qdelta = h->qdelta.as<float>(); A.qscale = h->qscale.as<float>();
            A.qfrag16 = h->qfrag16.as<uint4>();
            A.slot_col = h->slot_col.as<int>();
            A.eps2 = h->eps2.as<float>();
            A.bnorm = h->bnorm.as<unsigned>(); A.bdelta = h->bdelta.as<unsigned>();
            A.pf_bound = h->pf_bound.as<float>();
            A.ncols = (long long)ncols;
            A.bound_rows = P2_NSL * 16;
            A.ts = tsp(h, ST_FRONT);
            A.dbg = h->fr_dbg.as<unsigned long long>();
            const size_t rlds = fr_route_lds(L);
            switch (nb) {
#define LMI_FR_CASE(NBV) case NBV: route_kernel<NBV><<<L, FR_THREADS, rlds, h->stream>>>(A); break;
                LMI_FR_CASE(1) LMI_FR_CASE(2) LMI_FR_CASE(3) LMI_FR_CASE(4) LMI_FR_CASE(5) LMI_FR_CASE(6) LMI_FR_CASE(8) LMI_FR_CASE(10) LMI_FR_CASE(16)
#undef LMI_FR_CASE
                default: route_kernel<0><<<L, FR_THREADS, rlds, h->stream>>>(A); break;
            }
            HIPCHK(hipGetLastError());
            A.ts = nullptr;
            const int pgrid = 1 + (int)ncb_bound;
            const size_t plds = fr_pack_lds(L, h->KG16);
            const int nchunk = (h->d + 7) / 8;
            const bool vec = h->d % 8 == 0;
#define LMI_FP_LAUNCH(GSV, CPV) { if (vec) pack_kernel<GSV, CPV, true><<<pgrid, FP_THREADS, plds, h->stream>>>(A); \
                                  else pack_kernel<GSV, CPV, false><<<pgrid, FP_THREADS, plds, h->stream>>>(A); }
            if (nchunk <= 8) LMI_FP_LAUNCH(8, 1)
            else if (nchunk <= 16) LMI_FP_LAUNCH(16, 1)
            else if (nchunk <= 32) LMI_FP_LAUNCH(32, 1)
            else if (nchunk <= 64) LMI_FP_LAUNCH(64, 1)
            else if (nchunk <= 128) LMI_FP_LAUNCH(64, 2)
            else LMI_FP_LAUNCH(64, 4)
#undef LMI_FP_LAUNCH
            HIPCHK(hipGetLastError());
        } else {
        query_norm_kernel<<<cdiv(nq, 4), 256, 0, h->stream>>>(d_qs, nq, h->d, h->qnorm.as<float>(), h->qdelta.as<float>(),
                                                              h->qscale.as<float>());
        HIPCHK(hipGetLastError());
        {
            long long total = (long long)ncols * h->KG16 * 2;
            pack_queries16_kernel<<<cdiv(total, 256), 256, 0, h->stream>>>(d_qs, h->d, h->colmap.as<int>(), (long long)ncols,
                                                                          h->KG16, h->qscale.as<float>(), h->qfrag16.as<uint4>(), frag16x16(h));
            HIPCHK(hipGetLastError());
        }
        slot_bound_kernel<<<cdiv(nslots, 256), 256, 0, h->stream>>>(d_order, h->slot_col.as<int>(), nslots, nb, h->KG16 * 16,
                                                                   h->qnorm.as<float>(), h->qdelta.as<float>(),
                                                                   h->bnorm.as<unsigned>(), h->bdelta.as<unsigned>(), h->eps2.as<float>());
        HIPCHK(hipGetLastError());
        CHK(side_join(h));
        }
        CHK(record(h, 2));
        PrefilterParams F;
        F.slab16 = h->slab16.as<uint4>();
        F.qfrag16 = h->qfrag16.as<uint4>();
        F.KG16 = h->KG16;
        F.L = L;
        F.chunk_rb = S.chunk_rb;
        F.chunk_rb_b = R.chunk_rb_b;
        F.tile_cb = R.tile_cb;
        F.sample_max = R.sample_max;
        F.rb_start = S.rb_start;
        F.nb_rows = R.nb_rows;
        F.nch = R.nch;
        F.m = R.m;
        F.m0 = R.m0;
        F.cb_start = R.cb_start;
        F.grp_bucket = R.grp_bucket;
        F.grp_base = R.grp_base;
        F.grp_n = R.grp_n;
        F.grp_total = R.grp_total;
        F.grp_base1 = R.grp_base1;
        F.grp_total1 = R.grp_total1;
        F.ncols = (long long)ncols;
        F.head = S.head;
        F.bound = h->pf_bound.as<float>();
        F.bound1 = S.col_thr;
        F.eps2 = h->eps2.as<float>();
        F.cand_cnt = h->cand_cnt.as<unsigned>();
        F.cand_row = h->cand_row.as<unsigned>();
        F.cand_s = h->cand_s.as<float>();
        F.redo_count = nullptr; F.redo_bucket = nullptr; F.redo_col = nullptr;
        unsigned* fbw = h->fb_list.as<unsigned>();
        F.x.log = h->x_log.as<uint4>();
        F.x.cap = h->x_cap;
        F.x.head = fbw + 3;
        F.x.fail = fbw + 1;
        F.x.launch = 0;
        h->stamps_off = (ncols * P2_NSL * 16 * 4 + 255) / 256 * 256;
        F.stamps = reinterpret_cast<unsigned long long*>(static_cast<char*>(h->pf_bound.p) + h->stamps_off);
        F.ts_start = tsp(h, ST_P1);
        F.ts_end_cell = nullptr;
#if defined(LMI_P2_STAMPS)
        HIPCHK(hipMemsetAsync(F.stamps, 0, 2 * 8 * 12 * 8, h->stream));
#endif
        {
            CHK(launch_pass2<true>(h, F));
            bound_merge2_kernel<<<cdiv((long long)ncols, 64), 256, 0, h->stream>>>(F.bound, (long long)ncols, F.bound1,
                use_front ? reinterpret_cast<unsigned*>(h->cb_alloc.as<unsigned long long>() + FR_MAX_L + 1) : nullptr);
            HIPCHK(hipGetLastError());
            h->fr_bump_pending = false;
            if (qbound) {
                query_bound_kernel<<<cdiv(nq, 256), 256, 0, h->stream>>>(h->slot_col.as<int>(), nq, nb, F.eps2, F.bound1);
                HIPCHK(hipGetLastError());
            }
        }
        if (h->debug_emit_all) {
            FillRanges D;
            D.count = 1; D.p[0] = reinterpret_cast<unsigned*>(F.bound1); D.n[0] = (long long)ncols; D.v[0] = 0xFF800000u; D.ts = nullptr;
            fill_ranges_kernel<<<h->num_cus * 4, 256, 0, h->stream>>>(D);
            HIPCHK(hipGetLastError());
        }
        CHK(record(h, 5));

        F.ts_start = tsp(h, ST_P2);
        F.ts_end_cell = F.ts_start ? p2_end_cell : nullptr;
        if (F.ts_start) { (void)tsp(h, ST_CLK_WALL); (void)tsp(h, ST_CLK_CYC); }
        CHK(launch_pass2<false>(h, F));
        F.ts_start = nullptr;
        F.ts_end_cell = nullptr;
        CHK(record(h, 6));
        use_tail = rescore_is_streamed(h) && h->use_tail && (rescore_group_size(nb) == nb || h->use_tail == 2) &&
                   RC_WAVES * tail_wave_lds(h->dp, rescore_group_size(nb), true) <= RC_SMALL_LDS_CAP;
        tail_merges = use_tail && rescore_group_size(nb) == nb;
        if (use_tail && !h->h_oflag) {
            HIPCHK(hipHostMalloc(reinterpret_cast<void**>(&h->h_oflag), 64, hipHostMallocMapped));
            *h->h_oflag = 0u;
        }
        if (use_tail && *reinterpret_cast<volatile unsigned*>(h->h_oflag) != 0u) { h->overflow_armed = 1000; *h->h_oflag = 0u; }
        const bool overflow_sorted = h->pf_redo && !h->debug_emit_all && (!use_tail || h->overflow_armed > 0);
        if (use_tail && h->overflow_armed > 0) --h->overflow_armed;
        if (overflow_sorted) {
            unsigned* rc = h->redo.as<unsigned>();
            int* rb = reinterpret_cast<int*>(rc + 1);
            unsigned char* rcol = reinterpret_cast<unsigned char*>(rc + 1 + L);
            overflow_rebound_kernel<<<cdiv(nslots, 256), 256, 0, h->stream>>>(h->slot_col.as<int>(), d_order, nslots, F.cand_cnt, F.cand_s,
                                                                             F.bound1, rc, rb, rcol, F.x.fail, F.x.cap, h->x_off.as<unsigned>(), fbw + 4);
            HIPCHK(hipGetLastError());
            PrefilterParams F2 = F;
            F2.x.cap = 0;
            F2.x.fail = fbw + 2;
            F2.x.launch = 1;
            F2.head = F.head + 16;
            F2.redo_count = rc; F2.redo_bucket = rb; F2.redo_col = rcol;
            CHK(launch_pass2<false>(h, F2));
        }
        RescoreParams Q;
        Q.bucket_order = d_order;
        Q.slot_col = h->slot_col.as<int>();
        Q.nslots = nslots;
        Q.nb = nb;
        Q.d = h->d;
        Q.raw = raw;
        Q.rb_start = S.rb_start;
        Q.nb_rows = R.nb_rows;
        Q.cand_cnt = F.cand_cnt;
        Q.cand_row = F.cand_row;
        Q.cand_s = F.cand_s;
        Q.eps2 = F.eps2;
        Q.rows = h->rowmajor.as<float>();
        Q.dp = h->dp;
        Q.q = d_qs;
        Q.qn2 = d_qn2;
        Q.ids_slab = h->ids_slab.as<unsigned>();
        Q.rank_d = h->rank_d.as<float>();
        Q.rank_id = h->rank_id.as<unsigned>();
        Q.fallback = h->fallback.as<int>();
        Q.nkeep = h->nkeep.as<int>();
        Q.fb_count = reinterpret_cast<int*>(fbw);
        Q.fb_list = reinterpret_cast<int*>(fbw + 8);
        const bool sorted_overflow = overflow_sorted;
        Q.x_fail = fbw + 1;
        Q.x_off = sorted_overflow ? h->x_off.as<unsigned>() : nullptr;
        Q.x_ext = h->x_ext.as<uint2>();
        Q.x_log = F.x.log;
        Q.x_head = F.x.head;
        Q.x_cap = F.x.cap;
        Q.redo_col = sorted_overflow ? reinterpret_cast<const unsigned char*>(h->redo.as<unsigned>() + 1 + L) : nullptr;
        Q.ts = h->ts_set;
        Q.p2_end = p2_end_cell;
        if (Q.ts) { (void)tsp(h, ST_TAIL); (void)tsp(h, ST_P2END); (void)tsp(h, ST_FB); }
        Q.merge_pending = nullptr; Q.m_kout = 0; Q.m_out_d = nullptr; Q.m_out_id = nullptr; Q.m_out_key = nullptr;
        Q.host_oflag = use_tail ? h->h_oflag : nullptr;
#ifndef LMI_ABL_NOEMIT
        if (use_tail) {
            const int G = rescore_group_size(nb), groups = nslots / G;
            CHK(h->surv_row.reserve((size_t)nslots * RC_KEEP * 4));
            const int sub_cap = cdiv(groups, RC_SUB);
            SelectOut O;
            O.surv_row = h->surv_row.as<unsigned>();
            O.G = G;
            O.grp_flag = nullptr;
            O.active = h->rs_active.as<int>();
            O.sub_cap = sub_cap;
            O.big = O.active + RC_SUB + RC_SUB * sub_cap;
            TailParams T;
            T.ngroups = groups; T.merge = tail_merges ? 1 : 0; T.kout = kout;
// ... 723 lines not shown
    if (cap_rb) std::copy(h->h_cap_rb.begin(), h->h_cap_rb.end(), cap_rb);
    if (n_rb_total) *n_rb_total = h->n_rb_total;
    if (alloc) *alloc = alloc_rb(h);
    if (counters) std::copy(h->mut_paths, h->mut_paths + 4, counters);
    return 0;
}

extern "C" LMI_API int lmi_debug_read_candidates(lmi_index* h, int64_t slot, int cap, uint32_t* rows, float* shat,
                                         int* count, float* eps2, float* qscale, float* xscale) {
    if (!h) return fail("lmi_debug_read_candidates: NULL handle");
    if (!h->last_fast) return fail("lmi_debug_read_candidates: the last scan did not use the prefilter");
    if (slot < 0 || slot >= h->last_nslots) return fail("lmi_debug_read_candidates: slot outside the last scan's %d", h->last_nslots);
    CHK(set_dev(h));
    HIPCHK(hipStreamSynchronize(h->stream));
    int col = -1;
    HIPCHK(hipMemcpy(&col, h->slot_col.as<int>() + slot, 4, hipMemcpyDeviceToHost));
    unsigned cnt = 0;
    float e2 = 0.0f, qs = 1.0f, xs[2] = {1.0f, 1.0f};
    if (col >= 0) {
        HIPCHK(hipMemcpy(&cnt, h->cand_cnt.as<unsigned>() + col, 4, hipMemcpyDeviceToHost));
        HIPCHK(hipMemcpy(&e2, h->eps2.as<float>() + col, 4, hipMemcpyDeviceToHost));
        HIPCHK(hipMemcpy(&qs, h->qscale.as<float>() + slot / h->last_nb, 4, hipMemcpyDeviceToHost));
        HIPCHK(hipMemcpy(xs, h->xscale.p, 8, hipMemcpyDeviceToHost));
        const unsigned n = std::min<unsigned>(std::min<unsigned>(cnt, (unsigned)PF_CAP), (unsigned)std::max(cap, 0));
        if (n && rows) HIPCHK(hipMemcpy(rows, h->cand_row.as<unsigned>() + (size_t)col * PF_CAP, (size_t)n * 4, hipMemcpyDeviceToHost));
        if (n && shat) HIPCHK(hipMemcpy(shat, h->cand_s.as<float>() + (size_t)col * PF_CAP, (size_t)n * 4, hipMemcpyDeviceToHost));
    }
    if (count) *count = col >= 0 ? (int)cnt : -1;
    if (eps2) *eps2 = e2;
    if (qscale) *qscale = qs;
    if (xscale) *xscale = xs[0];
    return 0;
}

extern "C" LMI_API int lmi_debug_peek(lmi_index* h, const char* name, void* dst, int64_t bytes) {
    if (!h || !name || !dst) return fail("lmi_debug_peek: NULL argument");
    CHK(set_dev(h));
    HIPCHK(hipStreamSynchronize(h->stream));
    DevBuf* b = nullptr;
    size_t off = 0;
    if (!strcmp(name, "pf_bound")) b = &h->pf_bound;
    if (!strcmp(name, "fr_dbg")) b = &h->fr_dbg;
    if (!strcmp(name, "pf_stamps")) { b = &h->pf_bound; off = h->stamps_off; }
    if (!strcmp(name, "cand_total")) {
        if (bytes != 8 || !h->last_fast) return fail("lmi_debug_peek: cand_total is 8 bytes after a prefilter scan");
        unsigned long long* d_acc = reinterpret_cast<unsigned long long*>(h->stats.as<long long>() + 2);
        HIPCHK(hipMemsetAsync(d_acc, 0, 8, h->stream));
        sum_u32_kernel<<<64, 256, 0, h->stream>>>(h->cand_cnt.as<unsigned>(), h->last_ncols, d_acc);
        HIPCHK(hipGetLastError());
        HIPCHK(hipStreamSynchronize(h->stream));
        HIPCHK(hipMemcpy(dst, d_acc, 8, hipMemcpyDeviceToHost));
        return 0;
    }
    if (!strcmp(name, "pf_redo")) b = &h->redo;
    if (!strcmp(name, "pf_fallback")) b = &h->fb_list;
    if (!b) return fail("lmi_debug_peek: unknown buffer '%s'", name);
    if (bytes < 0 || off + (size_t)bytes > b->cap) return fail("lmi_debug_peek: %lld bytes asked of a %zu-byte buffer", (long long)bytes, b->cap);
    if (bytes) HIPCHK(hipMemcpy(dst, static_cast<char*>(b->p) + off, (size_t)bytes, hipMemcpyDeviceToHost));
    return 0;
}

extern "C" LMI_API int lmi_scan_stats(lmi_index* h, double* flops, int64_t* pairs, int64_t* items) {
    if (!h) return fail("lmi_scan_stats: NULL handle");
    CHK(set_dev(h));
    if (h->stats_pending) {
        HIPCHK(hipStreamSynchronize(h->stream));
        HIPCHK(hipMemcpy(h->h_stats, h->stats.p, 32, hipMemcpyDeviceToHost));
        h->stats_pending = false;
    }
    if (pairs) *pairs = h->h_stats[0];
    if (items) *items = h->h_stats[1];
    if (flops) *flops = 2.0 * h->d * (double)h->h_stats[0];
    return 0;
}
```

### learnedmetricindex_amd/csrc/lmi_mutate.h

```cpp
#pragma once
#include "lmi_prefilter.h"

namespace lmi {

__global__ void scatter_ids_kernel(const uint32_t* __restrict__ ids, const int* __restrict__ pos, long long n,
                                   uint32_t* __restrict__ ids_slab) {
    const long long i = (long long)blockIdx.x * blockDim.x + threadIdx.x;
    if (i >= n) return;
    const int p = pos[i];
    if (p >= 0) ids_slab[p] = ids[i];
}


__global__ void absmax_ranges_kernel(const float* __restrict__ rows, int d, int pitch, const int* __restrict__ row0,
                                     const int* __restrict__ nrows, unsigned* __restrict__ out) {
    const int r = blockIdx.y;
    const long long n = (long long)nrows[r] * d;
    const float* x = rows + (size_t)row0[r] * pitch;
    float m = 0.0f;
    for (long long i = (long long)blockIdx.x * blockDim.x + threadIdx.x; i < n; i += (long long)gridDim.x * blockDim.x) {
        const long long row = i / d;
        m = fmaxf(m, fabsf(x[row * pitch + (i - row * d)]));
    }
#pragma unroll
    for (int o = 32; o > 0; o >>= 1) m = fmaxf(m, __shfl_xor(m, o));
    if ((threadIdx.x & 63) == 0) atomicMax(out, __float_as_uint(m));
}

__global__ void convert16_ranges_kernel(const float* __restrict__ rows, int d, int pitch, const int* __restrict__ rb0,
                                        const int* __restrict__ nrb, int KG16, const float* __restrict__ scale,
                                        uint4* __restrict__ dst, int f16x16) {
    const int r = blockIdx.y;
    const long long p0 = (long long)rb0[r] * 32;
    const long long n = (long long)nrb[r] * 32 * KG16 * 2;
    const float s = scale[0];
    for (long long idx = (long long)blockIdx.x * blockDim.x + threadIdx.x; idx < n; idx += (long long)gridDim.x * blockDim.x)
        convert16_one(rows, d, pitch, p0 + (idx >> 1) / KG16, (int)((idx >> 1) % KG16), (int)(idx & 1), KG16, s, dst, f16x16);
}

__global__ void bucket_norm_ranges_kernel(const float* __restrict__ rows, int d, int pitch, const int* __restrict__ bucket,
                                          const int* __restrict__ row0, const int* __restrict__ nrows,
                                          const float* __restrict__ scale, unsigned* __restrict__ bnorm_bits,
                                          unsigned* __restrict__ bdelta_bits) {
    const int r = blockIdx.y;
    const float s = scale[0];
    const float guard = norm_guard(d);
    float best = 0.0f, bestd = 0.0f;
    for (int row = blockIdx.x * blockDim.x + threadIdx.x; row < nrows[r]; row += gridDim.x * blockDim.x)
        row_norms(rows + ((size_t)row0[r] + row) * pitch, d, s, guard, best, bestd);
    if (best > 0.0f) atomicMax(bnorm_bits + bucket[r], __float_as_uint(best));
    if (bestd > 0.0f) atomicMax(bdelta_bits + bucket[r], __float_as_uint(bestd));
}

__global__ void reset_norms_kernel(const int* __restrict__ bucket, int n, unsigned* __restrict__ bnorm_bits,
                                   unsigned* __restrict__ bdelta_bits) {
    const int i = blockIdx.x * blockDim.x + threadIdx.x;
    if (i >= n) return;
    bnorm_bits[bucket[i]] = 0u;
    bdelta_bits[bucket[i]] = 0u;
}

__global__ void mark_deleted_kernel(const uint32_t* __restrict__ ids_slab, const int* __restrict__ rb_start,
                                    const int* __restrict__ nb_rows, const uint32_t* __restrict__ del, int n_del,
                                    int* __restrict__ keep, int* __restrict__ removed) {
    const int b = blockIdx.y;
    const int n_b = nb_rows[b];
    const size_t base = (size_t)rb_start[b] * 32;
    int cnt = 0;
    for (int row = blockIdx.x * blockDim.x + threadIdx.x; row < n_b; row += gridDim.x * blockDim.x) {
        const uint32_t id = ids_slab[base + row];
        int lo = 0, hi = n_del;
        while (lo < hi) {
            const int mid = (lo + hi) >> 1;
            if (del[mid] < id) lo = mid + 1;
            else hi = mid;
        }
        const int hit = lo < n_del && del[lo] == id;
        keep[base + row] = !hit;
        cnt += hit;
    }
#pragma unroll
    for (int o = 32; o > 0; o >>= 1) cnt += __shfl_xor(cnt, o);
    if ((threadIdx.x & 63) == 0 && cnt) atomicAdd(removed + b, cnt);
}

constexpr int CM_THREADS = 1024;
__global__ __launch_bounds__(CM_THREADS) void compact_map_kernel(const int* __restrict__ hit, const int* __restrict__ span,
                                                                const int* __restrict__ rb_start, const int* __restrict__ nb_rows,
                                                                const int* __restrict__ keep, int* __restrict__ src) {
    __shared__ int sc[CM_THREADS];
    const int b = hit[blockIdx.x];
    const int n_b = nb_rows[b];
    const size_t base = (size_t)rb_start[b] * 32;
    const int t = threadIdx.x;
    int carry = 0;
    for (int r0 = 0; r0 < n_b; r0 += CM_THREADS) {
        const int row = r0 + t;
        const int f = row < n_b ? keep[base + row] : 0;
        sc[t] = f;
        __syncthreads();
        for (int o = 1; o < CM_THREADS; o <<= 1) {
            const int v = t >= o ? sc[t - o] : 0;
            __syncthreads();
            sc[t] += v;
            __syncthreads();
        }
        if (f) src[base + carry + sc[t] - 1] = row;
        carry += sc[CM_THREADS - 1];
        __syncthreads();
    }
    for (int j = carry + t; j < span[blockIdx.x]; j += CM_THREADS) src[base + j] = -1;
}
// ... 36 lines not shown
```

### learnedmetricindex_amd/csrc/lmi_pass2.h

```cpp
#pragma once
#include <type_traits>

#include "lmi_prefilter.h"

namespace lmi {

constexpr int P2_G = 2;
constexpr int P2_MAXCB = 12;
#ifndef LMI_P2_WAVES
#define LMI_P2_WAVES 8
#endif
constexpr int P2_WAVES = LMI_P2_WAVES;
static_assert(P2_WAVES == 4 || P2_WAVES == 8, "");
constexpr int P2_BLOCKS_PER_CU = 8 / P2_WAVES;
constexpr int P2_TILE_RB = 8;
constexpr int P2_TILE_ROWS = 32 * P2_TILE_RB;
constexpr int P2_SLOT_BYTES = P2_MAXCB * P2_G * 1024;
constexpr int P2_RING = 3;
constexpr int P2_NSL = 16;
constexpr int P2_NSL_BIG = 8;
static_assert(P2_NSL * 16 == P2_NSL_BIG * 32, "bound_merge2_kernel reads 256 values per column either way");
constexpr int P2_LIST = 64 + 1;
constexpr int P2_AREG0 = 232;
#define LMI_P2_NUM_VGPR_ATTR 116
static_assert(2 * LMI_P2_NUM_VGPR_ATTR == P2_AREG0 && P2_AREG0 + 8 * P2_RING == 256, "three 8-register sets at the top of the file");

typedef unsigned u32x2 __attribute__((ext_vector_type(2)));
typedef unsigned u32x4 __attribute__((ext_vector_type(4)));

template <int I, int N, class F>
__device__ __forceinline__ void static_for(F&& f) {
    if constexpr (I < N) {
        f(std::integral_constant<int, I>{});
        static_for<I + 1, N>(f);
    }
}

__device__ __forceinline__ int p2_sample_tiles(int n_b, int smax) { return sample_tiles256(n_b, smax); }
static_assert(P2_TILE_RB == 8, "sample_tiles256 counts 256-row tiles");

#ifdef LMI_P2_STAMPS
#ifndef LMI_P2_STAMPS_SAMPLE
#define LMI_P2_STAMPS_SAMPLE 0
#endif
#define P2_STAMP(PH) if (SAMPLE == (LMI_P2_STAMPS_SAMPLE != 0)) { const unsigned long long t_ = __builtin_readcyclecounter(); st_acc[PH] += t_ - st_last; st_last = t_; }
#else
#define P2_STAMP(PH)
#endif
#if defined(LMI_P2_STAMPS) && defined(LMI_P2_STAMPS_FINE)
#define P2_STAMP_FINE(PH) P2_STAMP(PH)
#else
#define P2_STAMP_FINE(PH)
#endif

template <int NCB, bool SAMPLE>
struct Tile2 {
    static constexpr int G = P2_G;
    static constexpr int Q = G * NCB;
#ifndef LMI_P2_BR
#define LMI_P2_BR 3
#endif
    static constexpr int BR = LMI_P2_BR;
    static_assert(BR == 3 || BR == 6, "3 Q must be a multiple of BR for every NCB");
    static constexpr int D = NCB < BR - 1 ? NCB : BR - 1;
    static constexpr int PBL = (NCB + 1) / 2;
    static constexpr int PA = G;
    static_assert(G == 2, "written out for two k-groups per stage");

    const PrefilterParams& P;
    unsigned ring;
    uint4* ring_p;
    uint2* sList;
    float* sThr;
    uint4* sPend;
    int lane, w;
    unsigned lds_lane;
    typedef float f32x4v __attribute__((ext_vector_type(4)));
    f32x4v acc[NCB][2][2];
    half8 b[BR];
    unsigned pend_pos;
#ifdef LMI_P2_STAMPS
    unsigned long long st_acc[12], st_last;
#endif

    static constexpr int breg(int slot, int q) { return (slot * Q + q) % BR; }
    static constexpr int areg(int set, int g) { return P2_AREG0 + 8 * set + 4 * g; }
    static constexpr int younger(int q) {
#if defined(LMI_ABL_NOLDSB) || defined(LMI_ABL_NOLGKM) || defined(LMI_ABL_NOLDS)
        return 15;
#endif
        return (q + D - 1 < Q - 1 ? q + D - 1 : Q - 1) - q;
    }

    template <int OFF>
    static __device__ __forceinline__ void lds_rd(half8& r, unsigned addr) {
        asm volatile("ds_read_b128 %0, %1 offset:%2" : "=v"(r) : "v"(addr), "n"(OFF) : "memory");
    }
    template <int N>
    static __device__ __forceinline__ void lgkm_wait(half8& y) {
        asm volatile("s_waitcnt lgkmcnt(%1)" : "+v"(y) : "n"(N) : "memory");
    }

    template <int SLOT, int QI>
    __device__ __forceinline__ void mfma_q() {
        constexpr int ch = QI / NCB, n = QI % NCB, R = areg(SLOT, 0);
        asm volatile("v_mfma_f32_16x16x32_f16 %0, v[%c3:%c4], %2, %0\n\tv_mfma_f32_16x16x32_f16 %1, v[%c5:%c6], %2, %1"
                     : "+v"(acc[n][0][ch]), "+v"(acc[n][1][ch]) : "v"(b[breg(SLOT, QI)]), "n"(R), "n"(R + 3), "n"(R + 4), "n"(R + 7));
    }
    template <int SLOT, int QI>
    __device__ __forceinline__ void mfma_q0() {
        constexpr int ch = QI / NCB, n = QI % NCB, R = areg(SLOT, 0);
        asm volatile("v_mfma_f32_16x16x32_f16 %0, v[%c3:%c4], %2, 0\n\tv_mfma_f32_16x16x32_f16 %1, v[%c5:%c6], %2, 0"
                     : "=&v"(acc[n][0][ch]), "=&v"(acc[n][1][ch]) : "v"(b[breg(SLOT, QI)]), "n"(R), "n"(R + 3), "n"(R + 4), "n"(R + 7));
    }
    template <int SLOT, int QI>
    __device__ __forceinline__ void read_b() {
        constexpr int g = QI / NCB, n = QI % NCB;
#ifdef LMI_ABL_NOLDSB
        if constexpr (QI % 4 != 0) { asm volatile("" : "+v"(b[breg(SLOT, QI)])); return; }
#endif
#ifdef LMI_ABL_NOLDS
        asm volatile("" : "+v"(b[breg(SLOT, QI)])); return;
#endif
        lds_rd<(n * G + g) * 1024>(b[breg(SLOT, QI)], lds_lane + SLOT * P2_SLOT_BYTES);
    }

    template <int SLOT, int QI, int WAIT, bool ZERO, int RSLOT, int RQ>
    __device__ __forceinline__ void step() {
        constexpr int ch = QI / NCB, n = QI % NCB, R = areg(SLOT, 0);
#if defined(LMI_ABL_NOLDS) || defined(LMI_ABL_NOLDSB)
        if constexpr (WAIT >= 0) lgkm_wait<WAIT>(b[breg(SLOT, QI)]);
        if constexpr (ZERO) mfma_q0<SLOT, QI>(); else mfma_q<SLOT, QI>();
        if constexpr (RQ >= 0) read_b<RSLOT, RQ>();
        return;
#endif
#define P2_MFMA_ACC "v_mfma_f32_16x16x32_f16 %0, v[%c4:%c5], %3, %0\n\tv_mfma_f32_16x16x32_f16 %1, v[%c6:%c7], %3, %1"
#define P2_MFMA_ZERO "v_mfma_f32_16x16x32_f16 %0, v[%c4:%c5], %3, 0\n\tv_mfma_f32_16x16x32_f16 %1, v[%c6:%c7], %3, 0"
        if constexpr (RQ >= 0) {
            constexpr int rg = RQ / NCB, rn = RQ % NCB;
            constexpr int OFF = (rn * G + rg) * 1024;
            const unsigned addr = lds_lane + RSLOT * P2_SLOT_BYTES;
            half8& bn = b[breg(RSLOT, RQ)];
            static_assert(breg(RSLOT, RQ) != breg(SLOT, QI), "the read's destination is the MFMAs' operand");
            if constexpr (WAIT >= 0) {
                if constexpr (ZERO)
                    asm volatile("s_waitcnt lgkmcnt(%c10)\n\tds_read_b128 %2, %8 offset:%c9\n\t" P2_MFMA_ZERO
                                 : "=&v"(acc[n][0][ch]), "=&v"(acc[n][1][ch]), "=&v"(bn) : "v"(b[breg(SLOT, QI)]), "n"(R), "n"(R + 3), "n"(R + 4), "n"(R + 7), "v"(addr), "n"(OFF), "n"(WAIT) : "memory");
                else
                    asm volatile("s_waitcnt lgkmcnt(%c10)\n\tds_read_b128 %2, %8 offset:%c9\n\t" P2_MFMA_ACC
                                 : "+v"(acc[n][0][ch]), "+v"(acc[n][1][ch]), "=&v"(bn) : "v"(b[breg(SLOT, QI)]), "n"(R), "n"(R + 3), "n"(R + 4), "n"(R + 7), "v"(addr), "n"(OFF), "n"(WAIT) : "memory");
            } else {
                if constexpr (ZERO)
                    asm volatile("ds_read_b128 %2, %8 offset:%c9\n\t" P2_MFMA_ZERO
                                 : "=&v"(acc[n][0][ch]), "=&v"(acc[n][1][ch]), "=&v"(bn) : "v"(b[breg(SLOT, QI)]), "n"(R), "n"(R + 3), "n"(R + 4), "n"(R + 7), "v"(addr), "n"(OFF) : "memory");
                else
                    asm volatile("ds_read_b128 %2, %8 offset:%c9\n\t" P2_MFMA_ACC
                                 : "+v"(acc[n][0][ch]), "+v"(acc[n][1][ch]), "=&v"(bn) : "v"(b[breg(SLOT, QI)]), "n"(R), "n"(R + 3), "n"(R + 4), "n"(R + 7), "v"(addr), "n"(OFF) : "memory");
            }
        } else {
            static_assert(WAIT >= 0, "");
            half8 dummy;
            if constexpr (ZERO)
                asm volatile("s_waitcnt lgkmcnt(%c8)\n\t" P2_MFMA_ZERO
                             : "=&v"(acc[n][0][ch]), "=&v"(acc[n][1][ch]), "=&v"(dummy) : "v"(b[breg(SLOT, QI)]), "n"(R), "n"(R + 3), "n"(R + 4), "n"(R + 7), "n"(WAIT) : "memory");
            else
                asm volatile("s_waitcnt lgkmcnt(%c8)\n\t" P2_MFMA_ACC
                             : "+v"(acc[n][0][ch]), "+v"(acc[n][1][ch]), "=&v"(dummy) : "v"(b[breg(SLOT, QI)]), "n"(R), "n"(R + 3), "n"(R + 4), "n"(R + 7), "n"(WAIT) : "memory");
        }
#undef P2_MFMA_ACC
#undef P2_MFMA_ZERO
    }

    __device__ __forceinline__ bool is_loader() const { return P2_WAVES == 4 ? true : w >= 4; }
    struct Stream {
        const char* a;
        const uint4* b0;
        int bo[PBL];
    };
    template <int SET>
    __device__ __forceinline__ void load_a(const Stream& S) {
#ifdef LMI_ABL_NOLOAD
        return;
#endif
        constexpr int R = areg(SET, 0);
        asm volatile("s_nop 4\n\tglobal_load_dwordx4 v[%c2:%c3], %0, %1\n\tglobal_load_dwordx4 v[%c4:%c5], %0, %1 offset:1024"
                     :: "v"(lds_lane), "s"(S.a), "n"(R), "n"(R + 3), "n"(R + 4), "n"(R + 7) : "memory");
    }
    template <int DST>
    __device__ __forceinline__ void dma_b(const Stream& S) {
#ifdef LMI_ABL_NOLOAD
        return;
#endif
        uint4* slot = ring_p + DST * (P2_SLOT_BYTES / 16);
        const int lw = w & 3;
        static_for<0, PBL>([&](auto jc) {
            constexpr int j = decltype(jc)::value;
            const int cb = min((lw >> 1) + 2 * j, NCB - 1);
            glds16(reinterpret_cast<const float4*>(S.b0 + S.bo[j] + lane), reinterpret_cast<float4*>(slot + (cb * G + (lw & 1)) * 64));
        });
    }

    template <int SLOT, int DST>
    __device__ __forceinline__ void stage(const Stream& S, bool loader, bool pend, bool last, bool first, bool prev_first) {
        constexpr int PS = (SLOT + P2_RING - 1) % P2_RING;
        static_assert(PS == DST, "ring of three: the stage two ahead reuses the previous stage's slot");
        if (loader) dma_b<DST>(S);
        static_for<0, D>([&](auto i) {
            constexpr int I = decltype(i)::value;
            if (pend) {
                if constexpr (PS == 0) {
                    if (prev_first) step<PS, Q - D + I, -1, true, SLOT, I>(); else step<PS, Q - D + I, -1, false, SLOT, I>();
                } else {
                    step<PS, Q - D + I, -1, false, SLOT, I>();
                }
            } else {
                read_b<SLOT, I>();
            }
        });
        load_a<DST>(S);
        static_for<0, Q - D>([&](auto qi) {
            constexpr int q = decltype(qi)::value;
            if constexpr (SLOT == 0) {
                if (first) step<SLOT, q, younger(q), true, SLOT, q + D>(); else step<SLOT, q, younger(q), false, SLOT, q + D>();
            } else {
                step<SLOT, q, younger(q), false, SLOT, q + D>();
            }
        });
        if (last) {
            static_for<Q - D, Q>([&](auto qi) {
                constexpr int q = decltype(qi)::value;
                if constexpr (SLOT == 0) {
                    if (first) step<SLOT, q, 0, true, -1, -1>(); else step<SLOT, q, 0, false, -1, -1>();
                } else {
                    step<SLOT, q, 0, false, -1, -1>();
                }
            });
        }
    }

    static __device__ __forceinline__ int lane_id() {
        unsigned z = 0u;
        asm volatile("" : "+v"(z));
        return (int)__builtin_amdgcn_mbcnt_hi(~0u, __builtin_amdgcn_mbcnt_lo(~0u, z));
    }
    __device__ __forceinline__ void flush_pending(int ln) {
        if (is_loader()) asm volatile("s_waitcnt vmcnt(%1)" : "+v"(pend_pos) : "n"(2 * (PA + PBL)) : "memory");
        else asm volatile("s_waitcnt vmcnt(%1)" : "+v"(pend_pos) : "n"(2 * PA) : "memory");
        if (pend_pos != 0xffffffffu) {
            u32x4 e;
            const unsigned pa = (unsigned)reinterpret_cast<uintptr_t>(sPend + w * 64) + (unsigned)ln * 16u;
            asm volatile("ds_read_b128 %0, %1\n\ts_waitcnt lgkmcnt(0)" : "=v"(e) : "v"(pa) : "memory");
            cand_store(P, (size_t)e.x, pend_pos, e.y, __uint_as_float(e.z));
        }
        pend_pos = 0xffffffffu;
    }

    __device__ __forceinline__ void epilogue_emit(int rb_tile0, int n_b, size_t col0) {
        const int ln = lane_id();
        const int quad = ln >> 4, c16 = ln & 15;
#ifdef LMI_ABL_NOEPI
#pragma unroll
        for (int n = 0; n < NCB; ++n) asm volatile("" :: "v"(acc[n][0][0]), "v"(acc[n][1][0]), "v"(acc[n][0][1]), "v"(acc[n][1][1]));
        return;
#endif
        const unsigned row0 = (unsigned)((rb_tile0 + w) * 32);
        if (row0 + 32u > (unsigned)n_b) {
            int lim = n_b - (int)row0 - 4 * quad;
#pragma unroll
            for (int n = 0; n < NCB; ++n) {
                asm volatile("" : "+v"(lim));
#pragma unroll
                for (int rh = 0; rh < 2; ++rh)
#pragma unroll
                    for (int r = 0; r < 4; ++r)
                        if (16 * rh + r >= lim) { acc[n][rh][0][r] = __builtin_nanf(""); acc[n][rh][1][r] = __builtin_nanf(""); }
            }
        }
        const unsigned list_addr = (unsigned)reinterpret_cast<uintptr_t>(sList + w * P2_LIST);
        int tot = 0;
        const unsigned kb = (unsigned)((c16 << 8) | (4 * quad));
        const unsigned thr_addr = (unsigned)reinterpret_cast<uintptr_t>(sThr) + (unsigned)c16 * 4u;
        constexpr int TB = 2;
        float thr[2][TB][2];
        auto thr_load = [&](int nb0, float (&t)[TB][2]) __attribute__((always_inline)) {
#pragma unroll
            for (int i = 0; i < TB; ++i) {
                const int n = min(nb0 + i, NCB - 1);
                asm volatile("ds_read_b32 %0, %1" : "=v"(t[i][0]) : "v"(thr_addr + (unsigned)(n * 128)) : "memory");
                asm volatile("ds_read_b32 %0, %1" : "=v"(t[i][1]) : "v"(thr_addr + (unsigned)(n * 128 + 64)) : "memory");
            }
        };
        thr_load(0, thr[0]);
#pragma unroll
        for (int n = 0; n < NCB; ++n) {
            constexpr int dummy = 0; (void)dummy;
            if (n % TB == 0) {
                asm volatile("s_waitcnt lgkmcnt(0)" ::: "memory");
#pragma unroll
                for (int i = 0; i < TB; ++i) asm volatile("" : "+v"(thr[(n / TB) & 1][i][0]), "+v"(thr[(n / TB) & 1][i][1]));
                if (n + TB < NCB) thr_load(n + TB, thr[((n / TB) + 1) & 1]);
            }
            float gm[2][2], t0, mh[2];
#pragma unroll
            for (int ch = 0; ch < 2; ++ch) {
#pragma unroll
                for (int rh = 0; rh < 2; ++rh) {
                    asm("v_max3_f32 %0, %1, %2, %3" : "=v"(t0) : "v"(acc[n][rh][ch][0]), "v"(acc[n][rh][ch][1]), "v"(acc[n][rh][ch][2]));
                    asm("v_max_f32 %0, %1, %2" : "=v"(gm[ch][rh]) : "v"(t0), "v"(acc[n][rh][ch][3]));
                }
                asm("v_max_f32 %0, %1, %2" : "=v"(mh[ch]) : "v"(gm[ch][0]), "v"(gm[ch][1]));
            }
            const float th0 = thr[(n / TB) & 1][n % TB][0], th1 = thr[(n / TB) & 1][n % TB][1];
            bool any = (mh[0] >= th0) | (mh[1] >= th1);
#ifdef LMI_ABL_NOEMIT
            any = any && th0 == 12345.678f;
#endif
            if (__builtin_expect(__ballot(any) == 0ull, 1)) continue;
#pragma unroll
            for (int ch = 0; ch < 2; ++ch) {
                const float th = ch ? th1 : th0;
#pragma unroll
                for (int rh = 0; rh < 2; ++rh) {
                    if (__ballot(gm[ch][rh] >= th) == 0ull) continue;
#pragma unroll
                    for (int r = 0; r < 4; ++r) {
                        const bool pass = acc[n][rh][ch][r] >= th;
                        const unsigned long long mask = __ballot(pass);
                        if (__builtin_expect(mask != 0ull, 0)) {
                            if (pass) {
                                const int my = tot + (int)__builtin_amdgcn_mbcnt_hi((unsigned)(mask >> 32), __builtin_amdgcn_mbcnt_lo((unsigned)mask, 0u));
                                const unsigned key = kb + (unsigned)(((n * 32 + 16 * ch) << 8) | (16 * rh + r));
                                const unsigned la = list_addr + (unsigned)min(my, 64) * 8u;
                                const unsigned sb = __float_as_uint(acc[n][rh][ch][r]);
                                const u32x2 ent = {key, sb};
                                asm volatile("ds_write_b64 %0, %1" :: "v"(la), "v"(ent) : "memory");
                            }
                            tot += (int)__popcll(mask);
                        }
                    }
                }
            }
        }
        flush_pending(ln);
        if (tot > 0 && tot <= 64) {
            if (ln < tot) {
                u32x2 e;
                const unsigned la = list_addr + (unsigned)ln * 8u;
                asm volatile("s_waitcnt lgkmcnt(0)\n\tds_read_b64 %0, %1\n\ts_waitcnt lgkmcnt(0)" : "=v"(e) : "v"(la) : "memory");
                const unsigned pcol = (unsigned)(col0 + (e.x >> 8));
                const u32x4 pe = {pcol, row0 + (e.x & 255u), e.y, 0u};
                const unsigned pa = (unsigned)reinterpret_cast<uintptr_t>(sPend + w * 64) + (unsigned)ln * 16u;
                asm volatile("ds_write_b128 %0, %1" :: "v"(pa), "v"(pe) : "memory");
#ifdef LMI_ABL_NOATOMIC
                pend_pos = (unsigned)ln;
#else
                const unsigned* cnt_addr = P.cand_cnt + pcol;
                const unsigned one = 1u;
                asm volatile("global_atomic_add %0, %1, %2, off sc0" : "=v"(pend_pos) : "v"(cnt_addr), "v"(one) : "memory");
#endif
            }
        } else if (tot > 64) {
#pragma unroll
            for (int n = 0; n < NCB; ++n) {
#pragma unroll
                for (int ch = 0; ch < 2; ++ch) {
                    const float th = sThr[n * 32 + 16 * ch + c16];
                    unsigned rowq = row0 + 4u * (unsigned)quad;
                    asm volatile("" : "+v"(rowq));
#pragma unroll
                    for (int rh = 0; rh < 2; ++rh)
#pragma unroll
                        for (int r = 0; r < 4; ++r)
                            if (acc[n][rh][ch][r] >= th) {
                                const size_t col = col0 + n * 32 + 16 * ch + c16;
                                const unsigned pos = atomicAdd(P.cand_cnt + col, 1u);
                                cand_store(P, col, pos, rowq + (unsigned)(16 * rh + r), acc[n][rh][ch][r]);
                            }
                }
            }
        }
    }

    __device__ __forceinline__ void epilogue_sample(int rb_tile0, int n_b, size_t col0, int m_left, int list_j, bool use_atomic, int rb_in_tile) {
        const int ln = lane_id();
        const int quad = ln >> 4, c16 = ln & 15;
        const unsigned row0 = (unsigned)((rb_tile0 + w) * 32);
        const bool ragged = row0 + 32u > (unsigned)n_b;
        int lim = ragged ? n_b - (int)row0 - 4 * quad : 64;
#pragma unroll
        for (int n = 0; n < NCB; ++n) {
            if (ragged) {
                asm volatile("" : "+v"(lim));
#pragma unroll
                for (int rh = 0; rh < 2; ++rh)
#pragma unroll
                    for (int r = 0; r < 4; ++r)
                        if (16 * rh + r >= lim) { acc[n][rh][0][r] = -INFINITY; acc[n][rh][1][r] = -INFINITY; }
            }
#pragma unroll
            for (int ch = 0; ch < 2; ++ch) {
                float m0, m1, m2;
                asm("v_max3_f32 %0, %1, %2, %3" : "=v"(m0) : "v"(acc[n][0][ch][0]), "v"(acc[n][0][ch][1]), "v"(acc[n][0][ch][2]));
                asm("v_max3_f32 %0, %1, %2, %3" : "=v"(m1) : "v"(acc[n][1][ch][0]), "v"(acc[n][1][ch][1]), "v"(acc[n][1][ch][2]));
                asm("v_max3_f32 %0, %1, %2, %3" : "=v"(m2) : "v"(m0), "v"(m1), "v"(acc[n][0][ch][3]));
                asm("v_max_f32 %0, %1, %2" : "=v"(m2) : "v"(m2), "v"(acc[n][1][ch][3]));
                const float mx = m2;
                if (n * 32 + 16 * ch + c16 < m_left) {
                    float* dst = P.bound + ((size_t)(list_j * 32 + (rb_in_tile + w) * 4 + quad)) * (size_t)P.ncols + (col0 + n * 32 + 16 * ch + c16);
                    if (!use_atomic) *dst = mx;
                    else {
                        if (mx >= 0.0f) atomicMax(reinterpret_cast<int*>(dst), __float_as_int(mx));
                        else atomicMin(reinterpret_cast<unsigned*>(dst), __float_as_uint(mx));
                    }
                }
            }
        }
    }

    template <typename Q>
    __device__ __forceinline__ void run(int b_, int cbt0_, int ch_, int m_use_, int nt_, Q& queue) {
        const int b = __builtin_amdgcn_readfirstlane(b_), cbt0 = __builtin_amdgcn_readfirstlane(cbt0_);
        const int ch = __builtin_amdgcn_readfirstlane(ch_), m_use = __builtin_amdgcn_readfirstlane(m_use_);
        const int nt = __builtin_amdgcn_readfirstlane(nt_);
#ifdef LMI_P2_STAMPS
        for (int i = 0; i < 12; ++i) st_acc[i] = 0;
        st_last = __builtin_readcyclecounter();
#endif
        const int tid = threadIdx.x;
        lane = tid & 63;
        w = __builtin_amdgcn_readfirstlane(tid >> 6);
        lds_lane = ring + (unsigned)lane * 16u;
        const int KG = P.KG16, NS = KG / G;
        const int n_b = P.nb_rows[b];
        const int nrb_b = (n_b + 31) >> 5;
        const int stride = SAMPLE ? sample_stride(n_b, P.sample_max) : 1;
        const int crb = (!SAMPLE && P.chunk_rb_b) ? P.chunk_rb_b[b] : P.chunk_rb;
        const int rb0 = SAMPLE ? ch * stride * P2_TILE_RB : ch * crb;
        const int nrb_all = SAMPLE ? P2_TILE_RB : min(crb, nrb_b - rb0);
        constexpr int VPT = P2_TILE_RB / P2_WAVES;
        const int nvt = SAMPLE ? nt * VPT : (nrb_all + P2_WAVES - 1) / P2_WAVES;
        const int tile_step = 2 * stride * P2_TILE_RB;
        auto vt_rb = [&](int v) __attribute__((always_inline)) { return SAMPLE ? rb0 + (v / VPT) * tile_step + (v % VPT) * P2_WAVES : rb0 + v * P2_WAVES; };
        const int cb_tile = P.cb_start[b] + cbt0;
        const int m_left = m_use - cbt0 * 32;
        const size_t col0 = (size_t)cb_tile * 32;
        const uint4* aslab = P.slab16 + ((size_t)P.rb_start[b] * KG) * 64;
        const size_t rb_stride = (size_t)KG * 64;
        const int rb_last = nrb_b - 1;
        const bool loader = is_loader();
        const int lw = w & 3;
        const uint4* bbase0 = P.qfrag16 + ((size_t)cb_tile * KG) * 64;
        pend_pos = 0xffffffffu;
        int vt_n = 0, t_n = 0;
        Stream S;
        const char* abase = reinterpret_cast<const char*>(aslab) - ring;
        S.a = abase + ((size_t)min(rb0 + w, rb_last) * rb_stride) * 16;
        S.b0 = bbase0;
#pragma unroll
        for (int j = 0; j < PBL; ++j) S.bo[j] = (min((lw >> 1) + 2 * j, NCB - 1) * KG + (lw & 1)) * 64;
        const int NSR = (NS + P2_RING - 1) / P2_RING * P2_RING;
#define P2_ADVANCE                                                                               \
        if (++t_n < NS) { S.a += G * 1024; S.b0 += G * 64; }                                     \
        else if (t_n == NSR) {                                                                   \
            t_n = 0;                                                                             \
            if (vt_n + 1 < nvt) {                                                                \
                ++vt_n; S.b0 = bbase0;                                                           \
                S.a = abase + ((size_t)min(vt_rb(vt_n) + w, rb_last) * rb_stride) * 16;          \
            }                                                                                    \
        }
#ifdef LMI_ABL_NOWAIT
#define P2_WAIT_LANDED
#elif defined(LMI_DBG_VM0)
#define P2_WAIT_LANDED asm volatile("s_waitcnt vmcnt(0)" ::: "memory");
#else
#define P2_WAIT_LANDED if (loader) asm volatile("s_waitcnt vmcnt(%0)" :: "n"(PA + PBL) : "memory"); else asm volatile("s_waitcnt vmcnt(%0)" :: "n"(PA) : "memory");
#endif
#if defined(LMI_ABL_NOBAR) && defined(LMI_ABL_NOBARLGKM)
#define P2_BARRIER
#elif defined(LMI_ABL_NOBAR)
#define P2_BARRIER asm volatile("s_waitcnt lgkmcnt(0)" ::: "memory");
#elif defined(LMI_ABL_NOBARLGKM)
#define P2_BARRIER __builtin_amdgcn_s_barrier();
#else
#define P2_BARRIER asm volatile("s_waitcnt lgkmcnt(0)" ::: "memory"); __builtin_amdgcn_s_barrier();
#endif
#define P2_STEP(SLOT, LIVE, LAST)                                                                \
        P2_WAIT_LANDED                                                                           \
        P2_STAMP_FINE(0)                                                                         \
        P2_BARRIER                                                                               \
        P2_STAMP_FINE(1)                                                                         \
        if (LIVE) {                                                                              \
            stage<SLOT, (SLOT + P2_RING - 1) % P2_RING>(S, loader, pend, (LAST), SLOT == 0 && t == 0, SLOT == 1 && t == 0); \
            pend = !(LAST);                                                                      \
        } else {                                                                                 \
            if (loader) dma_b<(SLOT + P2_RING - 1) % P2_RING>(S);                                \
            load_a<(SLOT + P2_RING - 1) % P2_RING>(S);                                           \
        }                                                                                        \
        P2_ADVANCE                                                                               \
        P2_STAMP_FINE(2)
        P2_STAMP(4)
        if (nvt > 0) {
            if (loader) dma_b<0>(S);
            load_a<0>(S);
            P2_ADVANCE
            if (loader) dma_b<1>(S);
            load_a<1>(S);
            P2_ADVANCE
        }
        if (!SAMPLE) {
            for (int i = tid; i < NCB * 32; i += 64 * P2_WAVES) {
                const bool wanted = i < m_left && (!P.redo_col || P.redo_col[col0 + i]);
                sThr[i] = wanted ? P.bound1[col0 + i] - P.eps2[col0 + i] : INFINITY;
            }
        }
        for (int vt = 0; vt < nvt; ++vt) {
            bool pend = false;
            for (int t = 0; t < NSR; t += P2_RING) {
                P2_STEP(0, true, t + 1 >= NS)
                P2_STEP(1, t + 1 < NS, t + 2 >= NS)
                P2_STEP(2, t + 2 < NS, t + 3 >= NS)
            }
            asm volatile("s_nop 15\n\ts_nop 3" ::: "memory");
            P2_STAMP(2)
            if (SAMPLE) epilogue_sample(vt_rb(vt), n_b, col0, m_left, (ch + 2 * (vt / VPT)) % P2_NSL_BIG, p2_sample_tiles(n_b, P.sample_max) > P2_NSL_BIG, (vt % VPT) * P2_WAVES);
            else epilogue_emit(rb0 + vt * P2_WAVES, n_b, col0);
            P2_STAMP(3)
        }
        asm volatile("s_waitcnt vmcnt(0)" ::: "memory");
        queue.prefetch();
        __syncthreads();
        P2_STAMP(5)
#ifdef LMI_P2_STAMPS
        if (SAMPLE == (LMI_P2_STAMPS_SAMPLE != 0)) {
            st_acc[7] = (unsigned long long)nvt;
            if (lane == 0) {
                unsigned long long* g = P.stamps + w * 12;
                for (int i = 0; i < 12; ++i) atomicAdd(g + i, st_acc[i]);
            }
        }
#endif
#undef P2_STEP
#undef P2_ADVANCE
#undef P2_WAIT_LANDED
#undef P2_BARRIER
        if (!SAMPLE) flush_pending(lane_id());
    }
};

__device__ __forceinline__ void front_epoch_bump(unsigned* epoch_bump) {
    if (epoch_bump && blockIdx.x == 0 && threadIdx.x == 0) { const unsigned e = *epoch_bump + 1u; *epoch_bump = e ? e : 1u; }
}
__global__ void front_epoch_bump_kernel(unsigned* epoch_bump) { front_epoch_bump(epoch_bump); }
__global__ __launch_bounds__(256) void bound_merge2_kernel(const float* __restrict__ lists, long long ncols, float* __restrict__ bound1, unsigned* epoch_bump = nullptr) {
    __shared__ float part[4][KPB][64];
    front_epoch_bump(epoch_bump);
    const int c = threadIdx.x & 63, qd = threadIdx.x >> 6;
    const long long col = (long long)blockIdx.x * 64 + c;
    float v[KPB];
#pragma unroll
    for (int j = 0; j < KPB; ++j) v[j] = -INFINITY;
    auto insert = [&](float s) {
        if (s > v[KPB - 1]) {
#pragma unroll
            for (int t = 0; t < KPB; ++t) {
                const float hi = fmaxf(v[t], s);
                s = fminf(v[t], s);
                v[t] = hi;
            }
        }
    };
    if (col < ncols) {
        const float* src = lists + (size_t)(qd * (P2_NSL / 4) * 16) * ncols + col;
        float in[(P2_NSL / 4) * 16];
#pragma unroll
        for (int i = 0; i < (P2_NSL / 4) * 16; ++i) in[i] = __builtin_nontemporal_load(src + (size_t)i * ncols);
#pragma unroll
        for (int i = 0; i < (P2_NSL / 4) * 16; ++i) insert(in[i]);
    }
#pragma unroll
    for (int j = 0; j < KPB; ++j) part[qd][j][c] = v[j];
    __syncthreads();
    if (qd == 0 && col < ncols) {
#pragma unroll
        for (int o = 1; o < 4; ++o)
#pragma unroll
            for (int j = 0; j < KPB; ++j) insert(part[o][j][c]);
        bound1[col] = v[KPB - 1];
    }
}

__global__ void query_bound_kernel(const int* __restrict__ slot_col, int nq, int nb, const float* __restrict__ eps2, float* __restrict__ bound1) {
    const int q = blockIdx.x * blockDim.x + threadIdx.x;
    if (q >= nq) return;
    float lq = -INFINITY;
    for (int r = 0; r < nb; ++r) {
        const int col = slot_col[q * nb + r];
        if (col >= 0) lq = fmaxf(lq, bound1[col] - 0.5f * eps2[col]);
    }
    if (!(lq > -INFINITY)) return;
    lq -= fabsf(lq) * 4.8e-7f;
    for (int r = 0; r < nb; ++r) {
        const int col = slot_col[q * nb + r];
        if (col >= 0) bound1[col] = fmaxf(bound1[col], lq + 0.5f * eps2[col] * 0.9999f);
    }
}

struct P2Item { int b, cbt0, ncb_tile, ch, m_use, nt; };
template <bool SAMPLE>
// ... 79 lines not shown
                s_prefix[i] = own_base[i];
                if (s_gb && i < own_n) s_gb[i] = P.grp_bucket[own * P.L + i];
            }
        own_live = own_tot > 0 && !(!SAMPLE && P.redo_bucket);
        ticket = -1;
        if (PREFETCH == 1 && own_live && threadIdx.x == 0) ticket = (int)atomicAdd(own_head, 1u);
        __syncthreads();
    }
    __device__ __forceinline__ void prefetch() {
        if (PREFETCH == 2 && own_live && threadIdx.x == 0) ticket = (int)atomicAdd(own_head, 1u);
    }
    __device__ __forceinline__ bool next(P2Item& it) {
        if (own_live) {
            if (threadIdx.x == 0) {
                int b = -1, local = 0;
                if (PREFETCH == 0 || (PREFETCH == 2 && ticket < 0)) ticket = (int)atomicAdd(own_head, 1u);
                if (ticket < own_tot) {
                    int lo = 0, hi = own_n;
                    if (prefix_lds) {
                        while (hi - lo > 1) { const int mid = (lo + hi) >> 1; if (s_prefix[mid] <= ticket) lo = mid; else hi = mid; }
                        local = ticket - s_prefix[lo];
                    } else {
                        while (hi - lo > 1) { const int mid = (lo + hi) >> 1; if (own_base[mid] <= ticket) lo = mid; else hi = mid; }
                        local = ticket - own_base[lo];
                    }
                    b = (s_gb && prefix_lds) ? s_gb[lo] : P.grp_bucket[own * P.L + lo];
                    if (PREFETCH == 1) ticket = (int)atomicAdd(own_head, 1u);
                }
                if (PREFETCH == 2) ticket = -1;
                s_item[0] = b;
                s_item[1] = local;
            }
            __syncthreads();
            const int b = s_item[0], local = s_item[1];
            __syncthreads();
            if (b >= 0) { p2_decode_item<SAMPLE>(P, b, local, it); return true; }
            own_live = false;
            grp = (own + 1) & (NGRP - 1);
        }
        return p2_pop_item<SAMPLE>(P, grp, s_item, it);
    }
};

template <bool SAMPLE>
__global__ __launch_bounds__(64 * P2_WAVES, 2) __attribute__((amdgpu_num_vgpr(LMI_P2_NUM_VGPR_ATTR))) void pass2_kernel(PrefilterParams P) {
#pragma clang diagnostic push
#pragma clang diagnostic ignored "-Winline-asm"
    asm volatile("" ::: "v255");
#pragma clang diagnostic pop
    __shared__ __attribute__((aligned(16))) uint4 ring[P2_RING * P2_SLOT_BYTES / 16];
    __shared__ uint2 sList[SAMPLE ? 1 : P2_WAVES * P2_LIST];
    __shared__ float sThr[SAMPLE ? 1 : P2_MAXCB * 32];
    __shared__ __attribute__((aligned(16))) uint4 sPend[SAMPLE ? 1 : P2_WAVES * 64];
    __shared__ int s_item[2];
    __shared__ int s_prefix[P2_PREFIX_CAP_K];
    __shared__ int s_gb[P2_PREFIX_CAP_K];
    if (!SAMPLE && P.redo_count && *P.redo_count == 0u) return;
    ts_first(P.ts_start);
    unsigned long long clk_w0 = 0, clk_c0 = 0;
    if (!SAMPLE) clk_begin(P.ts_end_cell ? P.ts_start : nullptr, clk_w0, clk_c0);
    P2Queue<SAMPLE, 2, 64 * P2_WAVES, P2_PREFIX_CAP_K> queue{P, s_item, s_prefix, s_gb};
    queue.init();
    P2Item item;
    while (queue.next(item)) {
        const int b = item.b, cbt0 = item.cbt0, ch = item.ch, m_use = item.m_use, nt = item.nt;
#define P2_CASE(N) case N: { Tile2<N, SAMPLE> it{P, (unsigned)reinterpret_cast<uintptr_t>(ring), ring, sList, sThr, sPend}; it.run(b, cbt0, ch, m_use, nt, queue); break; }
        switch (item.ncb_tile) {
            P2_CASE(1) P2_CASE(2) P2_CASE(3) P2_CASE(4) P2_CASE(5) P2_CASE(6)
            P2_CASE(7) P2_CASE(8) P2_CASE(9) P2_CASE(10) P2_CASE(11)
            default: { Tile2<12, SAMPLE> it{P, (unsigned)reinterpret_cast<uintptr_t>(ring), ring, sList, sThr, sPend}; it.run(b, cbt0, ch, m_use, nt, queue); break; }
        }
#undef P2_CASE
    }
    if (!SAMPLE) clk_end(P.ts_end_cell ? P.ts_start : nullptr, ST_P2, clk_w0, clk_c0);
#ifdef LMI_P2_ENDS
    if (!SAMPLE && P.ts_end_cell && threadIdx.x == 0 && blockIdx.x < 256) {
        P.stamps[192 + blockIdx.x] = wall_clock64();
        if (blockIdx.x == 0) P.stamps[191] = clk_w0;
    }
#endif
    ts_max(P.ts_end_cell);
}

}
```

### learnedmetricindex_amd/csrc/lmi_prefilter.h

```cpp
#pragma once
#include "lmi_kernels.h"


namespace lmi {

typedef _Float16 half8 __attribute__((ext_vector_type(8)));

constexpr int PF_STAGE_G = 2;
#ifndef LMI_PF_CAP
#define LMI_PF_CAP 1024
#endif
constexpr int PF_CAP = LMI_PF_CAP;
constexpr int PF_KEEP = 64;

__global__ void scatter_rows_kernel(const float* __restrict__ src, int d, const int* __restrict__ pos,
                                    long long row0, const long long* __restrict__ index, long long n_total, long long nrows,
                                    float* __restrict__ dst, int pitch) {
    const long long idx = (long long)blockIdx.x * blockDim.x + threadIdx.x;
    if (idx >= nrows * d) return;
    const long long i = idx / d;
    const int k = (int)(idx - i * d);
    const long long o = index ? index[i] : row0 + i;
    if (o < 0 || o >= n_total) return;
    const long long p = pos[o];
    if (p >= 0) dst[p * pitch + k] = src[idx];
}

__global__ void absmax_kernel(const float* __restrict__ x, long long n, unsigned* __restrict__ out) {
    float m = 0.0f;
    for (long long i = (long long)blockIdx.x * blockDim.x + threadIdx.x; i < n; i += (long long)gridDim.x * blockDim.x)
        m = fmaxf(m, fabsf(x[i]));
#pragma unroll
    for (int o = 32; o > 0; o >>= 1) m = fmaxf(m, __shfl_xor(m, o));
    if ((threadIdx.x & 63) == 0) atomicMax(out, __float_as_uint(m));
}

__device__ __forceinline__ float scale_of_max(unsigned maxbits) {
    const float m = __uint_as_float(maxbits);
    int e = 0;
    float s = 1.0f;
    if (m > 0.0f && m < INFINITY) { (void)frexpf(m, &e); s = ldexpf(1.0f, -e); }
    return s;
}
__global__ void make_scale_kernel(const unsigned* __restrict__ maxbits, float* __restrict__ scale) {
    const float s = scale_of_max(*maxbits);
    scale[0] = s;
    scale[1] = 1.0f / s;
}

__device__ __forceinline__ void convert16_one(const float* __restrict__ rows, int d, int pitch, long long p, int g, int hh, int KG16,
                                              float s, uint4* __restrict__ dst, int f16x16) {
    const float* x = rows + p * pitch;
    half8 h;
#pragma unroll
    for (int j = 0; j < 8; ++j) {
        const int k = 16 * g + 8 * hh + j;
        h[j] = (_Float16)(k < d ? x[k] * s : 0.0f);
    }
    const int r = (int)(p & 31);
    if (f16x16) {
        const int kq = 2 * (g & 1) + hh;
        dst[(((size_t)(p >> 5) * (KG16 / 2) + (g >> 1)) * 2 + (r >> 4)) * 64 + 16 * kq + (r & 15)] = *reinterpret_cast<uint4*>(&h);
    } else {
        dst[((size_t)(p >> 5) * KG16 + g) * 64 + hh * 32 + r] = *reinterpret_cast<uint4*>(&h);
    }
}
__global__ void convert16_kernel(const float* __restrict__ rows, int d, int pitch, long long n_rows, int KG16,
                                 const float* __restrict__ scale, uint4* __restrict__ dst, int f16x16 ) {
    const long long idx = (long long)blockIdx.x * blockDim.x + threadIdx.x;
    if (idx >= n_rows * KG16 * 2) return;
    convert16_one(rows, d, pitch, (idx >> 1) / KG16, (int)((idx >> 1) % KG16), (int)(idx & 1), KG16, scale[0], dst, f16x16);
}

__device__ __forceinline__ float norm_guard(int d) { return 1.0001f + (float)d * 5.96046448e-8f; }

__device__ __forceinline__ void row_norms(const float* __restrict__ x, int d, float s, float guard, float& best, float& bestd) {
    float acc = 0.0f, dl = 0.0f;
    for (int k = 0; k < d; ++k) {
        const float xs = x[k] * s;
        const float e = (float)(_Float16)xs - xs;
        acc += xs * xs;
        dl += e * e;
    }
    best = fmaxf(best, sqrtf(acc) * guard);
    bestd = fmaxf(bestd, sqrtf(dl) * guard);
}

__global__ void bucket_norm_kernel(const float* __restrict__ rows, int d, int pitch, const int* __restrict__ rb_start,
                                   const int* __restrict__ nb_rows, const float* __restrict__ scale,
                                   unsigned* __restrict__ bnorm_bits, unsigned* __restrict__ bdelta_bits) {
    const int b = blockIdx.y;
    const int n_b = nb_rows[b];
    const float s = scale[0];
    const float guard = norm_guard(d);
    float best = 0.0f, bestd = 0.0f;
    for (int row = blockIdx.x * blockDim.x + threadIdx.x; row < n_b; row += gridDim.x * blockDim.x) {
        row_norms(rows + ((size_t)rb_start[b] * 32 + row) * pitch, d, s, guard, best, bestd);
    }
    if (best > 0.0f) atomicMax(bnorm_bits + b, __float_as_uint(best));
    if (bestd > 0.0f) atomicMax(bdelta_bits + b, __float_as_uint(bestd));
}

__global__ void pf_selftest_kernel(int* __restrict__ ok) {
    const int lane = threadIdx.x;
    half8 a, b;
    float expect = 0.0f;
#pragma unroll
    for (int j = 0; j < 8; ++j) {
        const float tiny = (float)(8 * (lane >> 5) + j + 1) * 5.9604644775390625e-8f;
        a[j] = (_Float16)tiny;
        b[j] = (_Float16)1024.0f;
    }
    for (int k = 0; k < 16; ++k) expect += (float)(k + 1) * 5.9604644775390625e-8f * 1024.0f;
    f32x16 c;
#pragma unroll
    for (int r = 0; r < 16; ++r) c[r] = 0.0f;
    c = __builtin_amdgcn_mfma_f32_32x32x16_f16(a, b, c, 0, 0, 0);
    bool good = true;
#pragma unroll
    for (int r = 0; r < 16; ++r) good = good && (c[r] == expect);
    const unsigned long long all = __ballot(good);
    if (lane == 0) *ok = (all == ~0ull) ? 1 : 0;
}

struct FillRanges {
    static constexpr int MAXR = 12;
    unsigned* p[MAXR];
    long long n[MAXR];
    unsigned v[MAXR];
    int count;
    unsigned long long* ts;
    bool add(void* ptr, long long words, unsigned value) {
        if (count >= MAXR) return false;
        p[count] = static_cast<unsigned*>(ptr); n[count] = words; v[count] = value; ++count;
        return true;
    }
};
__global__ void fill_ranges_kernel(FillRanges F) {
    ts_first(F.ts);
    const long long stride = (long long)gridDim.x * blockDim.x;
    for (int r = 0; r < F.count; ++r)
        for (long long i = (long long)blockIdx.x * blockDim.x + threadIdx.x; i < F.n[r]; i += stride) F.p[r][i] = F.v[r];
}

__global__ __launch_bounds__(256) void query_norm_kernel(const float* __restrict__ q, int nq, int d,
                                                         float* __restrict__ qnorm, float* __restrict__ qdelta,
                                                         float* __restrict__ qscale) {
    const int wv = threadIdx.x >> 6, lane = threadIdx.x & 63;
    const int i = blockIdx.x * 4 + wv;
    if (i >= nq) return;
    const float* row = q + (size_t)i * d;
    const bool vec = (d & 3) == 0;
    float m = 0.0f;
// ... 82 lines not shown

#ifndef LMI_PF_X_LOG2
#define LMI_PF_X_LOG2 22
#endif
struct OverflowLog {
    uint4* log;
    unsigned cap;
    unsigned* head;
    unsigned* fail;
    unsigned launch;
};
__device__ __forceinline__ void pf_x_append(const OverflowLog& X, size_t col, unsigned e, unsigned row, float s) {
    const unsigned i = X.cap ? atomicAdd(X.head, 1u) : 0xffffffffu;
    if (i < X.cap) X.log[i] = make_uint4((unsigned)col, e | (X.launch << 31), row, __float_as_uint(s));
    else atomicOr(X.fail, 1u);
}

struct PrefilterParams {
    const uint4* slab16;
    const uint4* qfrag16;
    int KG16;
    int L;
    int chunk_rb;
    const int* chunk_rb_b;
    int sample_max;
    int tile_cb;
    const int* rb_start;
    const int* nb_rows;
    const int* nch;
    const int* m;
    const int* m0;
    const int* cb_start;
    const int* grp_bucket;
    const int* grp_base;
    const int* grp_n;
    const int* grp_total;
    const int* grp_base1;
    const int* grp_total1;
    long long ncols;
    unsigned* head;
    float* bound;
    float* bound1;
    const float* eps2;
    unsigned* cand_cnt;
    unsigned* cand_row;
    float* cand_s;
    unsigned long long* stamps;
    unsigned long long* ts_start;
    unsigned long long* ts_end_cell;
    const unsigned* redo_count;
    const int* redo_bucket;
    const unsigned char* redo_col;
    OverflowLog x;
};
__device__ __forceinline__ void cand_store(const PrefilterParams& P, size_t col, unsigned pos, unsigned row, float s) {
    if (__builtin_expect(pos < (unsigned)PF_CAP, 1)) {
        P.cand_row[col * PF_CAP + pos] = row;
        P.cand_s[col * PF_CAP + pos] = s;
    } else {
        pf_x_append(P.x, col, pos - (unsigned)PF_CAP, row, s);
    }
}

struct RescoreParams {
    const int* bucket_order;
    const int* slot_col;
    int nslots, nb, d, raw;
    const int* rb_start;
    const int* nb_rows;
    const unsigned* cand_cnt;
    const unsigned* cand_row;
    const float* cand_s;
    const float* eps2;
    const float* rows;
    int dp;
    const float* q;
    const float* qn2;
    const unsigned* ids_slab;
    float* rank_d;
    unsigned* rank_id;
    int* fallback;
    int* nkeep;
    int* fb_list;
    int* fb_count;
    const unsigned* x_fail;
    const unsigned* x_off;
    uint2* x_ext;
    const uint4* x_log;
    const unsigned* x_head;
    unsigned x_cap;
    const unsigned char* redo_col;
    unsigned long long* ts;
    const unsigned long long* p2_end;
    unsigned* host_oflag;
    int* merge_pending;
    int m_kout;
    float* m_out_d;
    unsigned* m_out_id;
    unsigned* m_out_key;
};
__device__ __forceinline__ void select_stamps(const RescoreParams& P) {
    if (P.ts && threadIdx.x == 0 && blockIdx.x == 0) {
        P.ts[ST_TAIL] = wall_clock64();
        if (P.p2_end) P.ts[ST_P2END] = *P.p2_end;
    }
}
// ... 403 lines not shown
```

Before: 2.088 million.

## Add mid-K checkpoint in pass2 to retire query column tiles early

Precomputes suffix norms of the f16 data past a checkpoint stage, both per bucket and per query column. Inside the pass-2 prefilter kernel each wave stops partway through the K dimension and uses a Cauchy-Schwarz bound on the remaining suffix to test whether some column blocks can no longer produce survivors. It then finishes the remaining K stages with a narrower column count via a compile-time dispatch. This is meant to cut MFMA work for tiles that cannot beat the threshold. In exchange it adds a synchronised checkpoint, extra shared memory, more template instantiations, extra norm computation at build time, and counters.

```diff
diff --git a/include/lmi_hip.h b/include/lmi_hip.h
--- a/include/lmi_hip.h
+++ b/include/lmi_hip.h
@@ -107,6 +107,8 @@
 LMI_API int lmi_timings_mean(lmi_index *h, float *ms , int *n_calls );
 LMI_API int lmi_scan_stats(lmi_index *h, double *flops, int64_t *pairs, int64_t *items);
 LMI_API int lmi_set_prefilter(lmi_index *h, int on);
+LMI_API int lmi_set_pass2_checkpoint(lmi_index *h, int mode);
+LMI_API int lmi_pass2_checkpoint_stats(lmi_index *h, int64_t *wave_tiles_tested, int64_t *wave_tiles_retired);
 LMI_API int lmi_clone_view(lmi_index *h, lmi_index **out);
 LMI_API int lmi_debug_peek(lmi_index *h, const char *name, void *dst, int64_t bytes);
 LMI_API int lmi_prefilter_stats(lmi_index *h, int *active, int64_t *survivors, int64_t *fallbacks);
diff --git a/learnedmetricindex_amd/_capi.py b/learnedmetricindex_amd/_capi.py
--- a/learnedmetricindex_amd/_capi.py
+++ b/learnedmetricindex_amd/_capi.py
@@ -69,6 +69,8 @@
     "lmi_set_chunk_rows": (ctypes.c_int, [_vp, ctypes.c_int]),
     "lmi_workspace_bytes": (ctypes.c_int, [_vp, ctypes.c_int, ctypes.c_int, _i64p]),
     "lmi_set_prefilter": (ctypes.c_int, [_vp, ctypes.c_int]),
+    "lmi_set_pass2_checkpoint": (ctypes.c_int, [_vp, ctypes.c_int]),
+    "lmi_pass2_checkpoint_stats": (ctypes.c_int, [_vp, _i64p, _i64p]),
     "lmi_debug_peek": (ctypes.c_int, [_vp, ctypes.c_char_p, _vp, ctypes.c_int64]),
     "lmi_clone_view": (ctypes.c_int, [_vp, ctypes.POINTER(_vp)]),
     "lmi_prefilter_stats": (ctypes.c_int, [_vp, ctypes.POINTER(ctypes.c_int), _i64p, _i64p]),
@@ -171,6 +173,15 @@
     def set_prefilter(self, on) -> None:
         _check(lib().lmi_set_prefilter(self._h, int(on)))
 
+    def set_pass2_checkpoint(self, mode: int) -> None:
+        _check(lib().lmi_set_pass2_checkpoint(self._h, int(mode)))
+
+    def pass2_checkpoint_stats(self):
+        a = ctypes.c_int64(0)
+        b = ctypes.c_int64(0)
+        _check(lib().lmi_pass2_checkpoint_stats(self._h, ctypes.byref(a), ctypes.byref(b)))
+        return a.value, b.value
+
     def debug_peek(self, name: str, nbytes: int) -> np.ndarray:
         out = np.empty(nbytes, np.uint8)
         _check(lib().lmi_debug_peek(self._h, name.encode(), out.ctypes.data_as(_vp), nbytes))
diff --git a/learnedmetricindex_amd/csrc/lmi_front.h b/learnedmetricindex_amd/csrc/lmi_front.h
--- a/learnedmetricindex_amd/csrc/lmi_front.h
+++ b/learnedmetricindex_amd/csrc/lmi_front.h
@@ -27,6 +27,8 @@
     uint4* qfrag16;
     int* slot_col;
     float* eps2;
+    float* csuf;
+    int ksuf;
     const unsigned* bnorm; const unsigned* bdelta;
     float* pf_bound;
     long long ncols;
@@ -340,21 +342,26 @@
 #pragma unroll
         for (int o = GS / 2; o > 0; o >>= 1) mx = fmaxf(mx, __shfl_xor(mx, o));
         const float s = scale_of_max(__float_as_uint(mx));
-        float acc = 0.0f, dl = 0.0f;
-#pragma unroll
-        for (int i = 0; i < CP; ++i)
+        float acc = 0.0f, dl = 0.0f, suf = 0.0f;
+#pragma unroll
+        for (int i = 0; i < CP; ++i) {
+            const bool in_suf = 8 * (gl + GS * i) >= P.ksuf;
 #pragma unroll
             for (int t = 0; t < 8; ++t) {
                 const float vs = v[c][i][t] * s;
-                const float e = (float)(_Float16)vs - vs;
+                const float hv = (float)(_Float16)vs;
+                const float e = hv - vs;
                 acc += vs * vs;
                 dl += e * e;
+                suf += in_suf ? hv * hv : 0.0f;
                 v[c][i][t] = vs;
             }
-#pragma unroll
-        for (int o = GS / 2; o > 0; o >>= 1) { acc += __shfl_xor(acc, o); dl += __shfl_xor(dl, o); }
+        }
+#pragma unroll
+        for (int o = GS / 2; o > 0; o >>= 1) { acc += __shfl_xor(acc, o); dl += __shfl_xor(dl, o); suf += __shfl_xor(suf, o); }
         if (gl == 0 && cc < 32) {
             const size_t col = (size_t)cb * 32 + cc;
+            if (P.csuf) P.csuf[col] = qi[c] >= 0 ? sqrtf(suf) * guard : 0.0f;
             if (qi[c] >= 0) {
                 const float qn = sqrtf(acc) * guard, dq = sqrtf(dl) * guard;
                 P.qnorm[qi[c]] = qn; P.qdelta[qi[c]] = dq; P.qscale[qi[c]] = s;
diff --git a/learnedmetricindex_amd/csrc/lmi_hip.hip b/learnedmetricindex_amd/csrc/lmi_hip.hip
--- a/learnedmetricindex_amd/csrc/lmi_hip.hip
+++ b/learnedmetricindex_amd/csrc/lmi_hip.hip
@@ -133,6 +133,9 @@
     int KG16 = 0;
     int dp = 0;
     DevBuf slab16, rowmajor, xscale, xmaxbits, bnorm, bdelta, qdelta;
+    DevBuf bsuf, csuf, ck_stats;
+    int ck_mode = 1;
+    int ck_stage = 0;
     DevBuf qnorm, qscale, qfrag16, eps2, cand_cnt, cand_row, cand_s, fallback, pf_bound, nkeep, surv_row, rs_flag, rs_active;
     DevBuf grp_scratch;
     bool ps_wide = false;
@@ -190,6 +193,7 @@
 };
 
 static int frag16x16(const lmi_index* h) { return (h->pf_small && h->KG16 <= PS_MAXKG) ? 0 : 1; }
+static int ck_ksuf(const lmi_index* h) { return h->ck_stage > 0 ? 32 * h->ck_stage : 0x7fffffff; }
 
 
 static int set_dev(lmi_index* h) {
@@ -300,7 +304,7 @@
     DevBuf* bufs[] = {&h->slab, &h->ids_slab, &h->pos, &h->d_nb_rows, &h->d_rb_start, &h->d_nch, &h->stage,
                       &h->act[0], &h->act[1], &h->xfrag, &h->logits, &h->order, &h->q_nav, &h->q_srch, &h->m,
                       &h->cb_start, &h->item_base, &h->part_base, &h->stats, &h->head, &h->slot_local,
-                      &h->slot_col, &h->colmap, &h->qfrag, &h->grp, &h->col_thr, &h->slab16, &h->rowmajor, &h->xscale, &h->xmaxbits, &h->bnorm, &h->bdelta, &h->qdelta, &h->qnorm, &h->qscale, &h->qfrag16, &h->eps2, &h->cand_cnt, &h->cand_row, &h->cand_s, &h->fallback, &h->pf_bound, &h->nkeep, &h->redo, &h->part_score, &h->part_row, &h->rank_d,
+                      &h->slot_col, &h->colmap, &h->qfrag, &h->grp, &h->col_thr, &h->slab16, &h->rowmajor, &h->xscale, &h->xmaxbits, &h->bnorm, &h->bdelta, &h->bsuf, &h->csuf, &h->ck_stats, &h->qdelta, &h->qnorm, &h->qscale, &h->qfrag16, &h->eps2, &h->cand_cnt, &h->cand_row, &h->cand_s, &h->fallback, &h->pf_bound, &h->nkeep, &h->redo, &h->part_score, &h->part_row, &h->rank_d,
                       &h->rank_id, &h->out_d, &h->out_id, &h->out_key, &h->x_log, &h->x_ext, &h->x_off, &h->fb_list, &h->grp_scratch, &h->ts_ring, &h->fr_dbg, &h->cb_alloc, &h->cb_bucket};
     for (DevBuf* b : bufs) b->release();
     if (h->h_oflag) (void)hipHostFree(h->h_oflag);
@@ -330,10 +334,10 @@
     for (auto& b : c->bias) b.borrow();
     for (auto& m : c->node_models) { for (auto& b : m.Wf) b.borrow(); for (auto& b : m.bias) b.borrow(); }
     DevBuf* shared[] = {&c->d_models, &c->d_child_offset, &c->d_child_model, &c->d_child_bucket, &c->slab, &c->ids_slab, &c->pos,
-                        &c->d_nb_rows, &c->d_rb_start, &c->d_nch, &c->slab16, &c->rowmajor, &c->xscale, &c->xmaxbits, &c->bnorm, &c->bdelta};
+                        &c->d_nb_rows, &c->d_rb_start, &c->d_nch, &c->slab16, &c->rowmajor, &c->xscale, &c->xmaxbits, &c->bnorm, &c->bdelta, &c->bsuf};
     for (DevBuf* b : shared) b->borrow();
     DevBuf* own[] = {&c->gather_send, &c->gather_recv, &c->pq_prob, &c->pq_ent, &c->pq_len, &c->nav_len, &c->nav_slab, &c->nav_ent,
-                     &c->nav_count, &c->nav_colq, &c->nav_active, &c->aug_rows, &c->q_aug, &c->qn2, &c->stage, &c->qdelta, &c->qnorm,
+                     &c->nav_count, &c->nav_colq, &c->nav_active, &c->aug_rows, &c->q_aug, &c->qn2, &c->stage, &c->csuf, &c->ck_stats, &c->qdelta, &c->qnorm,
                      &c->qscale, &c->qfrag16, &c->eps2, &c->cand_cnt, &c->cand_row, &c->cand_s, &c->fallback, &c->pf_bound, &c->nkeep, &c->redo,
                      &c->surv_row, &c->rs_flag, &c->rs_active, &c->act[0], &c->act[1], &c->xfrag, &c->logits, &c->order, &c->q_nav,
                      &c->q_srch, &c->m, &c->cb_start, &c->item_base, &c->part_base, &c->stats, &c->head, &c->slot_local, &c->slot_col,
@@ -382,6 +386,25 @@
     return 0;
 }
 
+extern "C" LMI_API int lmi_set_pass2_checkpoint(lmi_index* h, int mode) {
+    if (!h) return fail("lmi_set_pass2_checkpoint: NULL handle");
+    if (mode < 0 || mode > 2) return fail("lmi_set_pass2_checkpoint: mode %d unknown (0: off, 1: automatic, 2: every eligible tile)", mode);
+    h->ck_mode = mode;
+    return 0;
+}
+extern "C" LMI_API int lmi_pass2_checkpoint_stats(lmi_index* h, int64_t* wave_tiles_tested, int64_t* wave_tiles_retired) {
+    if (!h) return fail("lmi_pass2_checkpoint_stats: NULL handle");
+    CHK(set_dev(h));
+    long long v[2] = {0, 0};
+    if (h->last_fast && h->ck_stats.p) {
+        HIPCHK(hipStreamSynchronize(h->stream));
+        HIPCHK(hipMemcpy(v, h->ck_stats.p, 16, hipMemcpyDeviceToHost));
+    }
+    if (wave_tiles_tested) *wave_tiles_tested = v[0];
+    if (wave_tiles_retired) *wave_tiles_retired = v[1];
+    return 0;
+}
+
 extern "C" LMI_API int lmi_set_prefilter(lmi_index* h, int on) {
     if (!h) return fail("lmi_set_prefilter: NULL handle");
     if ((h->built || h->building) && (on != 0) != h->prefilter)
@@ -723,10 +746,13 @@
     CHK(h->xscale.reserve(16));
     CHK(h->bnorm.reserve((size_t)h->L * 4));
     CHK(h->bdelta.reserve((size_t)h->L * 4));
+    CHK(h->bsuf.reserve((size_t)h->L * 4));
+    h->ck_stage = frag16x16(h) ? p2_ck_stage(h->KG16 / PF_STAGE_G) : 0;
     CHK(h->slab16.reserve((size_t)h->n_rb_total * h->KG16 * 1024 + 8192));
     HIPCHK(hipMemsetAsync(h->xmaxbits.p, 0, 16, h->stream));
     HIPCHK(hipMemsetAsync(h->bnorm.p, 0, (size_t)h->L * 4, h->stream));
     HIPCHK(hipMemsetAsync(h->bdelta.p, 0, (size_t)h->L * 4, h->stream));
+    HIPCHK(hipMemsetAsync(h->bsuf.p, 0, (size_t)h->L * 4, h->stream));
     absmax_kernel<<<h->num_cus * 8, 256, 0, h->stream>>>(h->rowmajor.as<float>(), n_rows * h->dp, h->xmaxbits.as<unsigned>());
     HIPCHK(hipGetLastError());
     make_scale_kernel<<<1, 1, 0, h->stream>>>(h->xmaxbits.as<unsigned>(), h->xscale.as<float>());
@@ -738,7 +764,7 @@
     dim3 g(64, h->L);
     bucket_norm_kernel<<<g, 256, 0, h->stream>>>(h->rowmajor.as<float>(), h->d, h->dp, h->d_rb_start.as<int>(),
                                                 h->d_nb_rows.as<int>(), h->xscale.as<float>(), h->bnorm.as<unsigned>(),
-                                                h->bdelta.as<unsigned>());
+                                                h->bdelta.as<unsigned>(), ck_ksuf(h), h->bsuf.as<unsigned>());
     HIPCHK(hipGetLastError());
     HIPCHK(hipStreamSynchronize(h->stream));
     h->have16 = true;
@@ -1018,7 +1044,8 @@
             HIPCHK(hipGetLastError());
             dim3 gn(std::min(64, cdiv(max_rows, 256)), nr);
             bucket_norm_ranges_kernel<<<gn, 256, 0, h->stream>>>(h->rowmajor.as<float>(), h->d, h->dp, d_list, d_list + L, d_list + 2 * L,
-                                                                  h->xscale.as<float>(), h->bnorm.as<unsigned>(), h->bdelta.as<unsigned>());
+                                                                  h->xscale.as<float>(), h->bnorm.as<unsigned>(), h->bdelta.as<unsigned>(),
+                                                                  ck_ksuf(h), h->bsuf.as<unsigned>());
             HIPCHK(hipGetLastError());
         }
     }
@@ -1152,7 +1179,7 @@
         }
         HIPCHK(hipMemcpyAsync(h->mut_pos.p, list.data(), list.size() * 4, hipMemcpyHostToDevice, h->stream));
         const int* d_list = h->mut_pos.as<int>();
-        reset_norms_kernel<<<cdiv(nh, 256), 256, 0, h->stream>>>(d_list, nh, h->bnorm.as<unsigned>(), h->bdelta.as<unsigned>());
+        reset_norms_kernel<<<cdiv(nh, 256), 256, 0, h->stream>>>(d_list, nh, h->bnorm.as<unsigned>(), h->bdelta.as<unsigned>(), h->bsuf.as<unsigned>());
         HIPCHK(hipGetLastError());
         int max_rb = 0, max_rows = 1;
         for (int i = 0; i < nh; ++i) { max_rb = std::max(max_rb, old_nrb[i]); max_rows = std::max(max_rows, list[2 * nh + i]); }
@@ -1162,7 +1189,8 @@
         HIPCHK(hipGetLastError());
         dim3 gn(std::min(64, cdiv(max_rows, 256)), nh);
         bucket_norm_ranges_kernel<<<gn, 256, 0, h->stream>>>(h->rowmajor.as<float>(), h->d, h->dp, d_list, d_list + nh, d_list + 2 * nh,
-                                                              h->xscale.as<float>(), h->bnorm.as<unsigned>(), h->bdelta.as<unsigned>());
+                                                              h->xscale.as<float>(), h->bnorm.as<unsigned>(), h->bdelta.as<unsigned>(),
+                                                              ck_ksuf(h), h->bsuf.as<unsigned>());
         HIPCHK(hipGetLastError());
     }
     HIPCHK(hipStreamSynchronize(h->stream));
@@ -1502,6 +1530,7 @@
     bool fill_ok = true;
     auto fill = [&](void* ptr, long long words, unsigned value) { fill_ok = Z.add(ptr, words, value) && fill_ok; };
     const bool use_front = fast && h->use_front && L <= FR_MAX_L && nslots <= FR_MAX_SLOTS && h->d <= FR_MAX_D;
+    const bool ck_on = fast && h->ck_mode != 0 && h->ck_stage > 0 && frag16x16(h) != 0;
     if (!use_front) fill(h->m.p, 3ll * L, 0u);
     fill(h->head.p, 64, 0u);
     if (!use_front) fill(h->colmap.p, (long long)ncols, 0xFFFFFFFFu);
@@ -1512,6 +1541,8 @@
         CHK(h->qscale.reserve((size_t)nq * 4));
         CHK(h->qfrag16.reserve((size_t)ncb_bound * h->KG16 * 1024 + 8192));
         CHK(h->eps2.reserve(ncols * 4));
+        CHK(h->csuf.reserve(ncols * 4));
+        CHK(h->ck_stats.reserve(16));
         CHK(h->cand_cnt.reserve(ncols * 4));
         CHK(h->cand_row.reserve(ncols * PF_CAP * 4));
         CHK(h->cand_s.reserve(ncols * PF_CAP * 4));
@@ -1631,6 +1662,8 @@
             A.qfrag16 = h->qfrag16.as<uint4>();
             A.slot_col = h->slot_col.as<int>();
             A.eps2 = h->eps2.as<float>();
+            A.csuf = ck_on ? h->csuf.as<float>() : nullptr;
+            A.ksuf = ck_ksuf(h);
             A.bnorm = h->bnorm.as<unsigned>(); A.bdelta = h->bdelta.as<unsigned>();
             A.pf_bound = h->pf_bound.as<float>();
             A.ncols = (long long)ncols;
@@ -1707,6 +1740,11 @@
         F.cand_row = h->cand_row.as<unsigned>();
         F.cand_s = h->cand_s.as<float>();
         F.redo_count = nullptr; F.redo_bucket = nullptr; F.redo_col = nullptr;
+        F.xsuf = h->bsuf.as<unsigned>();
+        F.csuf = (ck_on && use_front) ? h->csuf.as<float>() : nullptr;
+        F.ck_stage = h->ck_stage;
+        F.ck_mode = h->ck_mode;
+        F.ck_stats = h->ck_stats.as<unsigned long long>();
         unsigned* fbw = h->fb_list.as<unsigned>();
         F.x.log = h->x_log.as<uint4>();
         F.x.cap = h->x_cap;
@@ -1723,7 +1761,7 @@
         {
             CHK(launch_pass2<true>(h, F));
             bound_merge2_kernel<<<cdiv((long long)ncols, 64), 256, 0, h->stream>>>(F.bound, (long long)ncols, F.bound1,
-                use_front ? reinterpret_cast<unsigned*>(h->cb_alloc.as<unsigned long long>() + FR_MAX_L + 1) : nullptr);
+                use_front ? reinterpret_cast<unsigned*>(h->cb_alloc.as<unsigned long long>() + FR_MAX_L + 1) : nullptr, F.ck_stats);
             HIPCHK(hipGetLastError());
             h->fr_bump_pending = false;
             if (qbound) {
@@ -1769,6 +1807,7 @@
             F2.x.launch = 1;
             F2.head = F.head + 16;
             F2.redo_count = rc; F2.redo_bucket = rb; F2.redo_col = rcol;
+            F2.csuf = nullptr;
             CHK(launch_pass2<false>(h, F2));
         }
         RescoreParams Q;
@@ -2598,6 +2637,9 @@
         HIPCHK(hipMemcpy(dst, d_acc, 8, hipMemcpyDeviceToHost));
         return 0;
     }
+    if (!strcmp(name, "xsuf")) b = &h->bsuf;
+    if (!strcmp(name, "xn")) b = &h->bnorm;
+    if (!strcmp(name, "dx")) b = &h->bdelta;
     if (!strcmp(name, "pf_redo")) b = &h->redo;
     if (!strcmp(name, "pf_fallback")) b = &h->fb_list;
     if (!b) return fail("lmi_debug_peek: unknown buffer '%s'", name);
diff --git a/learnedmetricindex_amd/csrc/lmi_mutate.h b/learnedmetricindex_amd/csrc/lmi_mutate.h
--- a/learnedmetricindex_amd/csrc/lmi_mutate.h
+++ b/learnedmetricindex_amd/csrc/lmi_mutate.h
@@ -41,23 +41,25 @@
 __global__ void bucket_norm_ranges_kernel(const float* __restrict__ rows, int d, int pitch, const int* __restrict__ bucket,
                                           const int* __restrict__ row0, const int* __restrict__ nrows,
                                           const float* __restrict__ scale, unsigned* __restrict__ bnorm_bits,
-                                          unsigned* __restrict__ bdelta_bits) {
+                                          unsigned* __restrict__ bdelta_bits, int ksuf, unsigned* __restrict__ bsuf_bits) {
     const int r = blockIdx.y;
     const float s = scale[0];
     const float guard = norm_guard(d);
-    float best = 0.0f, bestd = 0.0f;
+    float best = 0.0f, bestd = 0.0f, bests = 0.0f;
     for (int row = blockIdx.x * blockDim.x + threadIdx.x; row < nrows[r]; row += gridDim.x * blockDim.x)
-        row_norms(rows + ((size_t)row0[r] + row) * pitch, d, s, guard, best, bestd);
+        row_norms(rows + ((size_t)row0[r] + row) * pitch, d, s, guard, ksuf, best, bestd, bests);
     if (best > 0.0f) atomicMax(bnorm_bits + bucket[r], __float_as_uint(best));
     if (bestd > 0.0f) atomicMax(bdelta_bits + bucket[r], __float_as_uint(bestd));
+    if (bests > 0.0f) atomicMax(bsuf_bits + bucket[r], __float_as_uint(bests));
 }
 
 __global__ void reset_norms_kernel(const int* __restrict__ bucket, int n, unsigned* __restrict__ bnorm_bits,
-                                   unsigned* __restrict__ bdelta_bits) {
+                                   unsigned* __restrict__ bdelta_bits, unsigned* __restrict__ bsuf_bits) {
     const int i = blockIdx.x * blockDim.x + threadIdx.x;
     if (i >= n) return;
     bnorm_bits[bucket[i]] = 0u;
     bdelta_bits[bucket[i]] = 0u;
+    bsuf_bits[bucket[i]] = 0u;
 }
 
 __global__ void mark_deleted_kernel(const uint32_t* __restrict__ ids_slab, const int* __restrict__ rb_start,
diff --git a/learnedmetricindex_amd/csrc/lmi_pass2.h b/learnedmetricindex_amd/csrc/lmi_pass2.h
--- a/learnedmetricindex_amd/csrc/lmi_pass2.h
+++ b/learnedmetricindex_amd/csrc/lmi_pass2.h
@@ -21,6 +21,8 @@
 constexpr int P2_NSL_BIG = 8;
 static_assert(P2_NSL * 16 == P2_NSL_BIG * 32, "bound_merge2_kernel reads 256 values per column either way");
 constexpr int P2_LIST = 64 + 1;
+__host__ __device__ constexpr int p2_ck_stage(int NS) { return NS < 12 ? 0 : (3 * NS / 4) / P2_RING * P2_RING; }
+constexpr int P2_CK_MAXNL = 4;
 constexpr int P2_AREG0 = 232;
 #define LMI_P2_NUM_VGPR_ATTR 116
 static_assert(2 * LMI_P2_NUM_VGPR_ATTR == P2_AREG0 && P2_AREG0 + 8 * P2_RING == 256, "three 8-register sets at the top of the file");
@@ -66,6 +68,7 @@
     static constexpr int PBL = (NCB + 1) / 2;
     static constexpr int PA = G;
     static_assert(G == 2, "written out for two k-groups per stage");
+    static constexpr bool CK = !SAMPLE && P2_WAVES == 8;
 
     const PrefilterParams& P;
     unsigned ring;
@@ -73,6 +76,9 @@
     uint2* sList;
     float* sThr;
     uint4* sPend;
+    float* sThr2;
+    int* sCkW;
+    unsigned* sCk;
     int lane, w;
     unsigned lds_lane;
     typedef float f32x4v __attribute__((ext_vector_type(4)));
@@ -83,13 +89,15 @@
     unsigned long long st_acc[12], st_last;
 #endif
 
-    static constexpr int breg(int slot, int q) { return (slot * Q + q) % BR; }
+    static constexpr int Qv(int NV) { return G * NV; }
+    static constexpr int Dv(int NV) { return NV < BR - 1 ? NV : BR - 1; }
+    static constexpr int breg(int NV, int slot, int q) { return (slot * Qv(NV) + q) % BR; }
     static constexpr int areg(int set, int g) { return P2_AREG0 + 8 * set + 4 * g; }
-    static constexpr int younger(int q) {
+    static constexpr int younger(int NV, int q) {
 #if defined(LMI_ABL_NOLDSB) || defined(LMI_ABL_NOLGKM) || defined(LMI_ABL_NOLDS)
         return 15;
 #endif
-        return (q + D - 1 < Q - 1 ? q + D - 1 : Q - 1) - q;
+        return (q + Dv(NV) - 1 < Qv(NV) - 1 ? q + Dv(NV) - 1 : Qv(NV) - 1) - q;
     }
 
     template <int OFF>
@@ -101,71 +109,71 @@
         asm volatile("s_waitcnt lgkmcnt(%1)" : "+v"(y) : "n"(N) : "memory");
     }
 
-    template <int SLOT, int QI>
+    template <int NV, int SLOT, int QI>
     __device__ __forceinline__ void mfma_q() {
-        constexpr int ch = QI / NCB, n = QI % NCB, R = areg(SLOT, 0);
+        constexpr int ch = QI / NV, n = QI % NV, R = areg(SLOT, 0);
         asm volatile("v_mfma_f32_16x16x32_f16 %0, v[%c3:%c4], %2, %0\n\tv_mfma_f32_16x16x32_f16 %1, v[%c5:%c6], %2, %1"
-                     : "+v"(acc[n][0][ch]), "+v"(acc[n][1][ch]) : "v"(b[breg(SLOT, QI)]), "n"(R), "n"(R + 3), "n"(R + 4), "n"(R + 7));
-    }
-    template <int SLOT, int QI>
+                     : "+v"(acc[n][0][ch]), "+v"(acc[n][1][ch]) : "v"(b[breg(NV, SLOT, QI)]), "n"(R), "n"(R + 3), "n"(R + 4), "n"(R + 7));
+    }
+    template <int NV, int SLOT, int QI>
     __device__ __forceinline__ void mfma_q0() {
-        constexpr int ch = QI / NCB, n = QI % NCB, R = areg(SLOT, 0);
+        constexpr int ch = QI / NV, n = QI % NV, R = areg(SLOT, 0);
         asm volatile("v_mfma_f32_16x16x32_f16 %0, v[%c3:%c4], %2, 0\n\tv_mfma_f32_16x16x32_f16 %1, v[%c5:%c6], %2, 0"
-                     : "=&v"(acc[n][0][ch]), "=&v"(acc[n][1][ch]) : "v"(b[breg(SLOT, QI)]), "n"(R), "n"(R + 3), "n"(R + 4), "n"(R + 7));
-    }
-    template <int SLOT, int QI>
+                     : "=&v"(acc[n][0][ch]), "=&v"(acc[n][1][ch]) : "v"(b[breg(NV, SLOT, QI)]), "n"(R), "n"(R + 3), "n"(R + 4), "n"(R + 7));
+    }
+    template <int NV, int SLOT, int QI>
     __device__ __forceinline__ void read_b() {
-        constexpr int g = QI / NCB, n = QI % NCB;
+        constexpr int g = QI / NV, n = QI % NV;
 #ifdef LMI_ABL_NOLDSB
-        if constexpr (QI % 4 != 0) { asm volatile("" : "+v"(b[breg(SLOT, QI)])); return; }
+        if constexpr (QI % 4 != 0) { asm volatile("" : "+v"(b[breg(NV, SLOT, QI)])); return; }
 #endif
 #ifdef LMI_ABL_NOLDS
-        asm volatile("" : "+v"(b[breg(SLOT, QI)])); return;
-#endif
-        lds_rd<(n * G + g) * 1024>(b[breg(SLOT, QI)], lds_lane + SLOT * P2_SLOT_BYTES);
-    }
-
-    template <int SLOT, int QI, int WAIT, bool ZERO, int RSLOT, int RQ>
+        asm volatile("" : "+v"(b[breg(NV, SLOT, QI)])); return;
+#endif
+        lds_rd<(n * G + g) * 1024>(b[breg(NV, SLOT, QI)], lds_lane + SLOT * P2_SLOT_BYTES);
+    }
+
+    template <int NV, int SLOT, int QI, int WAIT, bool ZERO, int RSLOT, int RQ>
     __device__ __forceinline__ void step() {
-        constexpr int ch = QI / NCB, n = QI % NCB, R = areg(SLOT, 0);
+        constexpr int ch = QI / NV, n = QI % NV, R = areg(SLOT, 0);
 #if defined(LMI_ABL_NOLDS) || defined(LMI_ABL_NOLDSB)
-        if constexpr (WAIT >= 0) lgkm_wait<WAIT>(b[breg(SLOT, QI)]);
-        if constexpr (ZERO) mfma_q0<SLOT, QI>(); else mfma_q<SLOT, QI>();
-        if constexpr (RQ >= 0) read_b<RSLOT, RQ>();
+        if constexpr (WAIT >= 0) lgkm_wait<WAIT>(b[breg(NV, SLOT, QI)]);
+        if constexpr (ZERO) mfma_q0<NV, SLOT, QI>(); else mfma_q<NV, SLOT, QI>();
+        if constexpr (RQ >= 0) read_b<NV, RSLOT, RQ>();
         return;
 #endif
 #define P2_MFMA_ACC "v_mfma_f32_16x16x32_f16 %0, v[%c4:%c5], %3, %0\n\tv_mfma_f32_16x16x32_f16 %1, v[%c6:%c7], %3, %1"
 #define P2_MFMA_ZERO "v_mfma_f32_16x16x32_f16 %0, v[%c4:%c5], %3, 0\n\tv_mfma_f32_16x16x32_f16 %1, v[%c6:%c7], %3, 0"
         if constexpr (RQ >= 0) {
-            constexpr int rg = RQ / NCB, rn = RQ % NCB;
+            constexpr int rg = RQ / NV, rn = RQ % NV;
             constexpr int OFF = (rn * G + rg) * 1024;
             const unsigned addr = lds_lane + RSLOT * P2_SLOT_BYTES;
-            half8& bn = b[breg(RSLOT, RQ)];
-            static_assert(breg(RSLOT, RQ) != breg(SLOT, QI), "the read's destination is the MFMAs' operand");
+            half8& bn = b[breg(NV, RSLOT, RQ)];
+            static_assert(breg(NV, RSLOT, RQ) != breg(NV, SLOT, QI), "the read's destination is the MFMAs' operand");
             if constexpr (WAIT >= 0) {
                 if constexpr (ZERO)
                     asm volatile("s_waitcnt lgkmcnt(%c10)\n\tds_read_b128 %2, %8 offset:%c9\n\t" P2_MFMA_ZERO
-                                 : "=&v"(acc[n][0][ch]), "=&v"(acc[n][1][ch]), "=&v"(bn) : "v"(b[breg(SLOT, QI)]), "n"(R), "n"(R + 3), "n"(R + 4), "n"(R + 7), "v"(addr), "n"(OFF), "n"(WAIT) : "memory");
+                                 : "=&v"(acc[n][0][ch]), "=&v"(acc[n][1][ch]), "=&v"(bn) : "v"(b[breg(NV, SLOT, QI)]), "n"(R), "n"(R + 3), "n"(R + 4), "n"(R + 7), "v"(addr), "n"(OFF), "n"(WAIT) : "memory");
                 else
                     asm volatile("s_waitcnt lgkmcnt(%c10)\n\tds_read_b128 %2, %8 offset:%c9\n\t" P2_MFMA_ACC
-                                 : "+v"(acc[n][0][ch]), "+v"(acc[n][1][ch]), "=&v"(bn) : "v"(b[breg(SLOT, QI)]), "n"(R), "n"(R + 3), "n"(R + 4), "n"(R + 7), "v"(addr), "n"(OFF), "n"(WAIT) : "memory");
+                                 : "+v"(acc[n][0][ch]), "+v"(acc[n][1][ch]), "=&v"(bn) : "v"(b[breg(NV, SLOT, QI)]), "n"(R), "n"(R + 3), "n"(R + 4), "n"(R + 7), "v"(addr), "n"(OFF), "n"(WAIT) : "memory");
             } else {
                 if constexpr (ZERO)
                     asm volatile("ds_read_b128 %2, %8 offset:%c9\n\t" P2_MFMA_ZERO
-                                 : "=&v"(acc[n][0][ch]), "=&v"(acc[n][1][ch]), "=&v"(bn) : "v"(b[breg(SLOT, QI)]), "n"(R), "n"(R + 3), "n"(R + 4), "n"(R + 7), "v"(addr), "n"(OFF) : "memory");
+                                 : "=&v"(acc[n][0][ch]), "=&v"(acc[n][1][ch]), "=&v"(bn) : "v"(b[breg(NV, SLOT, QI)]), "n"(R), "n"(R + 3), "n"(R + 4), "n"(R + 7), "v"(addr), "n"(OFF) : "memory");
                 else
                     asm volatile("ds_read_b128 %2, %8 offset:%c9\n\t" P2_MFMA_ACC
-                                 : "+v"(acc[n][0][ch]), "+v"(acc[n][1][ch]), "=&v"(bn) : "v"(b[breg(SLOT, QI)]), "n"(R), "n"(R + 3), "n"(R + 4), "n"(R + 7), "v"(addr), "n"(OFF) : "memory");
+                                 : "+v"(acc[n][0][ch]), "+v"(acc[n][1][ch]), "=&v"(bn) : "v"(b[breg(NV, SLOT, QI)]), "n"(R), "n"(R + 3), "n"(R + 4), "n"(R + 7), "v"(addr), "n"(OFF) : "memory");
             }
         } else {
             static_assert(WAIT >= 0, "");
             half8 dummy;
             if constexpr (ZERO)
                 asm volatile("s_waitcnt lgkmcnt(%c8)\n\t" P2_MFMA_ZERO
-                             : "=&v"(acc[n][0][ch]), "=&v"(acc[n][1][ch]), "=&v"(dummy) : "v"(b[breg(SLOT, QI)]), "n"(R), "n"(R + 3), "n"(R + 4), "n"(R + 7), "n"(WAIT) : "memory");
+                             : "=&v"(acc[n][0][ch]), "=&v"(acc[n][1][ch]), "=&v"(dummy) : "v"(b[breg(NV, SLOT, QI)]), "n"(R), "n"(R + 3), "n"(R + 4), "n"(R + 7), "n"(WAIT) : "memory");
             else
                 asm volatile("s_waitcnt lgkmcnt(%c8)\n\t" P2_MFMA_ACC
-                             : "+v"(acc[n][0][ch]), "+v"(acc[n][1][ch]), "=&v"(dummy) : "v"(b[breg(SLOT, QI)]), "n"(R), "n"(R + 3), "n"(R + 4), "n"(R + 7), "n"(WAIT) : "memory");
+                             : "+v"(acc[n][0][ch]), "+v"(acc[n][1][ch]), "=&v"(dummy) : "v"(b[breg(NV, SLOT, QI)]), "n"(R), "n"(R + 3), "n"(R + 4), "n"(R + 7), "n"(WAIT) : "memory");
         }
 #undef P2_MFMA_ACC
 #undef P2_MFMA_ZERO
@@ -200,39 +208,41 @@
         });
     }
 
-    template <int SLOT, int DST>
+    template <int NV, int SLOT, int DST>
     __device__ __forceinline__ void stage(const Stream& S, bool loader, bool pend, bool last, bool first, bool prev_first) {
         constexpr int PS = (SLOT + P2_RING - 1) % P2_RING;
         static_assert(PS == DST, "ring of three: the stage two ahead reuses the previous stage's slot");
+        constexpr int Q = Qv(NV), D = Dv(NV);
+        constexpr bool Z = NV == NCB;
         if (loader) dma_b<DST>(S);
         static_for<0, D>([&](auto i) {
             constexpr int I = decltype(i)::value;
             if (pend) {
-                if constexpr (PS == 0) {
-                    if (prev_first) step<PS, Q - D + I, -1, true, SLOT, I>(); else step<PS, Q - D + I, -1, false, SLOT, I>();
+                if constexpr (PS == 0 && Z) {
+                    if (prev_first) step<NV, PS, Q - D + I, -1, true, SLOT, I>(); else step<NV, PS, Q - D + I, -1, false, SLOT, I>();
                 } else {
-                    step<PS, Q - D + I, -1, false, SLOT, I>();
+                    step<NV, PS, Q - D + I, -1, false, SLOT, I>();
                 }
             } else {
-                read_b<SLOT, I>();
+                read_b<NV, SLOT, I>();
             }
         });
         load_a<DST>(S);
         static_for<0, Q - D>([&](auto qi) {
             constexpr int q = decltype(qi)::value;
-            if constexpr (SLOT == 0) {
-                if (first) step<SLOT, q, younger(q), true, SLOT, q + D>(); else step<SLOT, q, younger(q), false, SLOT, q + D>();
+            if constexpr (SLOT == 0 && Z) {
+                if (first) step<NV, SLOT, q, younger(NV, q), true, SLOT, q + D>(); else step<NV, SLOT, q, younger(NV, q), false, SLOT, q + D>();
             } else {
-                step<SLOT, q, younger(q), false, SLOT, q + D>();
+                step<NV, SLOT, q, younger(NV, q), false, SLOT, q + D>();
             }
         });
         if (last) {
             static_for<Q - D, Q>([&](auto qi) {
                 constexpr int q = decltype(qi)::value;
-                if constexpr (SLOT == 0) {
-                    if (first) step<SLOT, q, 0, true, -1, -1>(); else step<SLOT, q, 0, false, -1, -1>();
+                if constexpr (SLOT == 0 && Z) {
+                    if (first) step<NV, SLOT, q, 0, true, -1, -1>(); else step<NV, SLOT, q, 0, false, -1, -1>();
                 } else {
-                    step<SLOT, q, 0, false, -1, -1>();
+                    step<NV, SLOT, q, 0, false, -1, -1>();
                 }
             });
         }
@@ -255,7 +265,7 @@
         pend_pos = 0xffffffffu;
     }
 
-    __device__ __forceinline__ void epilogue_emit(int rb_tile0, int n_b, size_t col0) {
+    __device__ __forceinline__ void epilogue_emit(int rb_tile0, int n_b, size_t col0, int n_ep) {
         const int ln = lane_id();
         const int quad = ln >> 4, c16 = ln & 15;
 #ifdef LMI_ABL_NOEPI
@@ -293,7 +303,7 @@
         thr_load(0, thr[0]);
 #pragma unroll
         for (int n = 0; n < NCB; ++n) {
-            constexpr int dummy = 0; (void)dummy;
+            if (n >= n_ep) continue;
             if (n % TB == 0) {
                 asm volatile("s_waitcnt lgkmcnt(0)" ::: "memory");
 #pragma unroll
@@ -362,6 +372,7 @@
         } else if (tot > 64) {
 #pragma unroll
             for (int n = 0; n < NCB; ++n) {
+                if (n >= n_ep) continue;
 #pragma unroll
                 for (int ch = 0; ch < 2; ++ch) {
                     const float th = sThr[n * 32 + 16 * ch + c16];
@@ -415,6 +426,47 @@
                 }
             }
         }
+    }
+
+    static __device__ __forceinline__ float ck_thr2(float thr, float xs, float cs, int dpad) {
+        const float u = (float)dpad * 1.1920929e-7f;
+        const float R = xs * cs * (1.0f + (2.0f * u + 1.52587890625e-5f));
+        const float A = thr - R;
+        return A - fabsf(A) * (4.0f * u + 1.52587890625e-5f);
+    }
+    __device__ __forceinline__ int checkpoint() {
+        asm volatile("s_nop 15\n\ts_nop 3" ::: "memory");
+        const int ln = lane_id();
+        int nlv;
+        const unsigned wa = (unsigned)reinterpret_cast<uintptr_t>(sCkW + w);
+        asm volatile("ds_read_b32 %0, %1\n\ts_waitcnt lgkmcnt(0)" : "=v"(nlv) : "v"(wa) : "memory");
+        const int nl = __builtin_amdgcn_readfirstlane(nlv);
+        const unsigned thr_addr = (unsigned)reinterpret_cast<uintptr_t>(sThr2) + (unsigned)(ln & 15) * 4u;
+        bool alive = false;
+        static_for<0, NCB>([&](auto nc) __attribute__((always_inline)) {
+            constexpr int n = decltype(nc)::value;
+            if (n >= nl) {
+                float t0, t1, m[2];
+                asm volatile("ds_read_b32 %0, %2 offset:%c3\n\tds_read_b32 %1, %2 offset:%c4" : "=&v"(t0), "=&v"(t1) : "v"(thr_addr), "n"(n * 128), "n"(n * 128 + 64) : "memory");
+#pragma unroll
+                for (int ch = 0; ch < 2; ++ch) {
+                    float a0, a1;
+                    asm volatile("v_max3_f32 %0, %1, %2, %3" : "=v"(a0) : "v"(acc[n][0][ch][0]), "v"(acc[n][0][ch][1]), "v"(acc[n][0][ch][2]));
+                    asm volatile("v_max3_f32 %0, %1, %2, %3" : "=v"(a1) : "v"(acc[n][1][ch][0]), "v"(acc[n][1][ch][1]), "v"(acc[n][1][ch][2]));
+                    asm volatile("v_max3_f32 %0, %1, %2, %3" : "=v"(a0) : "v"(a0), "v"(a1), "v"(acc[n][0][ch][3]));
+                    asm volatile("v_max_f32 %0, %1, %2" : "=v"(m[ch]) : "v"(a0), "v"(acc[n][1][ch][3]));
+                }
+                asm volatile("s_waitcnt lgkmcnt(0)" : "+v"(t0), "+v"(t1) :: "memory");
+                alive = alive | !(m[0] < t0) | !(m[1] < t1);
+            }
+        });
+        const bool dead = __ballot(alive) == 0ull;
+        if (ln == 0) {
+            const unsigned ca = (unsigned)reinterpret_cast<uintptr_t>(sCk), one = 1u;
+            asm volatile("ds_add_u32 %0, %1" :: "v"(ca), "v"(one) : "memory");
+            if (dead) asm volatile("ds_add_u32 %0, %1 offset:4" :: "v"(ca), "v"(one) : "memory");
+        }
+        return dead ? nl : -1;
     }
 
     template <typename Q>
@@ -484,13 +536,13 @@
 #else
 #define P2_BARRIER asm volatile("s_waitcnt lgkmcnt(0)" ::: "memory"); __builtin_amdgcn_s_barrier();
 #endif
-#define P2_STEP(SLOT, LIVE, LAST)                                                                \
+#define P2_STEP(NV, SLOT, LIVE, LAST)                                                            \
         P2_WAIT_LANDED                                                                           \
         P2_STAMP_FINE(0)                                                                         \
         P2_BARRIER                                                                               \
         P2_STAMP_FINE(1)                                                                         \
-        if (LIVE) {                                                                              \
-            stage<SLOT, (SLOT + P2_RING - 1) % P2_RING>(S, loader, pend, (LAST), SLOT == 0 && t == 0, SLOT == 1 && t == 0); \
+        if ((LIVE) && (NV) > 0) {                                                                \
+            stage<((NV) > 0 ? (NV) : 1), SLOT, (SLOT + P2_RING - 1) % P2_RING>(S, loader, pend, (LAST), SLOT == 0 && t == 0, SLOT == 1 && t == 0); \
             pend = !(LAST);                                                                      \
         } else {                                                                                 \
             if (loader) dma_b<(SLOT + P2_RING - 1) % P2_RING>(S);                                \
@@ -508,22 +560,72 @@
             P2_ADVANCE
         }
         if (!SAMPLE) {
+            const bool ck_item = CK && P.csuf && !P.redo_col && P.ck_stage > 0;
+            const float xs = ck_item ? __uint_as_float(P.xsuf[b]) : 0.0f;
             for (int i = tid; i < NCB * 32; i += 64 * P2_WAVES) {
                 const bool wanted = i < m_left && (!P.redo_col || P.redo_col[col0 + i]);
-                sThr[i] = wanted ? P.bound1[col0 + i] - P.eps2[col0 + i] : INFINITY;
+                const float thr = wanted ? P.bound1[col0 + i] - P.eps2[col0 + i] : INFINITY;
+                sThr[i] = thr;
+                if constexpr (CK) { if (ck_item) sThr2[i] = wanted ? ck_thr2(thr, xs, P.csuf[col0 + i], KG * 16) : INFINITY; }
+            }
+            if constexpr (CK) {
+                int verdict = -1;
+                if (ck_item) {
+                    const int nl = min(max((P.m0[b] - cbt0 * 32 + 31) >> 5, 0), NCB);
+                    if (nl <= P2_CK_MAXNL && nl < NCB) {
+                        bool ok = P.ck_mode == 2 || NCB - nl >= 2;
+                        if (ok && P.ck_mode != 2) {
+                            bool bad = false;
+                            for (int i = nl * 32 + lane; i < NCB * 32; i += 64) {
+                                const bool wanted = i < m_left;
+                                const float thr = wanted ? P.bound1[col0 + i] - P.eps2[col0 + i] : INFINITY;
+                                const float t2 = wanted ? ck_thr2(thr, xs, P.csuf[col0 + i], KG * 16) : INFINITY;
+                                bad = bad | !(t2 > 0.0f);
+                            }
+                            ok = __ballot(bad) == 0ull;
+                        }
+                        if (ok) verdict = nl;
+                    }
+                }
+                if (lane == 0) sCkW[w] = verdict;
             }
         }
         for (int vt = 0; vt < nvt; ++vt) {
             bool pend = false;
-            for (int t = 0; t < NSR; t += P2_RING) {
-                P2_STEP(0, true, t + 1 >= NS)
-                P2_STEP(1, t + 1 < NS, t + 2 >= NS)
-                P2_STEP(2, t + 2 < NS, t + 3 >= NS)
+            int t = 0, t_end = NS, n_ep = NCB;
+            if constexpr (CK) {
+                int v;
+                const unsigned wa = (unsigned)reinterpret_cast<uintptr_t>(sCkW + w);
+                asm volatile("ds_read_b32 %0, %1\n\ts_waitcnt lgkmcnt(0)" : "=v"(v) : "v"(wa) : "memory");
+                if (__builtin_amdgcn_readfirstlane(v) >= 0) t_end = P.ck_stage;
+            }
+            for (;;) {
+                for (; t < t_end; t += P2_RING) {
+                    P2_STEP(NCB, 0, true, t + 1 >= t_end)
+                    P2_STEP(NCB, 1, t + 1 < t_end, t + 2 >= t_end)
+                    P2_STEP(NCB, 2, t + 2 < t_end, t + 3 >= t_end)
+                }
+                if (!CK || t_end == NS) break;
+                t_end = NS;
+                const int nl = checkpoint();
+                if (nl < 0) continue;
+                static_for<0, (NCB - 1 < P2_CK_MAXNL ? NCB - 1 : P2_CK_MAXNL) + 1>([&](auto nvc) __attribute__((always_inline)) {
+                    constexpr int NV = decltype(nvc)::value;
+                    if (nl == NV) {
+                        for (; t < NS; t += P2_RING) {
+                            P2_STEP(NV, 0, true, t + 1 >= NS)
+                            P2_STEP(NV, 1, t + 1 < NS, t + 2 >= NS)
+                            P2_STEP(NV, 2, t + 2 < NS, t + 3 >= NS)
+                        }
+                        n_ep = NV;
+                    }
+                });
+                break;
             }
             asm volatile("s_nop 15\n\ts_nop 3" ::: "memory");
             P2_STAMP(2)
             if (SAMPLE) epilogue_sample(vt_rb(vt), n_b, col0, m_left, (ch + 2 * (vt / VPT)) % P2_NSL_BIG, p2_sample_tiles(n_b, P.sample_max) > P2_NSL_BIG, (vt % VPT) * P2_WAVES);
-            else epilogue_emit(rb0 + vt * P2_WAVES, n_b, col0);
+            else epilogue_emit(rb0 + vt * P2_WAVES, n_b, col0, n_ep);
             P2_STAMP(3)
         }
         asm volatile("s_waitcnt vmcnt(0)" ::: "memory");
@@ -551,9 +653,11 @@
     if (epoch_bump && blockIdx.x == 0 && threadIdx.x == 0) { const unsigned e = *epoch_bump + 1u; *epoch_bump = e ? e : 1u; }
 }
 __global__ void front_epoch_bump_kernel(unsigned* epoch_bump) { front_epoch_bump(epoch_bump); }
-__global__ __launch_bounds__(256) void bound_merge2_kernel(const float* __restrict__ lists, long long ncols, float* __restrict__ bound1, unsigned* epoch_bump = nullptr) {
+__global__ __launch_bounds__(256) void bound_merge2_kernel(const float* __restrict__ lists, long long ncols, float* __restrict__ bound1, unsigned* epoch_bump = nullptr,
+                                                           unsigned long long* ck_stats = nullptr) {
     __shared__ float part[4][KPB][64];
     front_epoch_bump(epoch_bump);
+    if (ck_stats && blockIdx.x == 0 && threadIdx.x < 2) ck_stats[threadIdx.x] = 0ull;
     const int c = threadIdx.x & 63, qd = threadIdx.x >> 6;
     const long long col = (long long)blockIdx.x * 64 + c;
     float v[KPB];
@@ -739,6 +843,10 @@
     __shared__ uint2 sList[SAMPLE ? 1 : P2_WAVES * P2_LIST];
     __shared__ float sThr[SAMPLE ? 1 : P2_MAXCB * 32];
     __shared__ __attribute__((aligned(16))) uint4 sPend[SAMPLE ? 1 : P2_WAVES * 64];
+    constexpr bool CKK = !SAMPLE && P2_WAVES == 8;
+    __shared__ float sThr2[CKK ? P2_MAXCB * 32 : 1];
+    __shared__ int sCkW[P2_WAVES];
+    __shared__ unsigned sCk[2];
     __shared__ int s_item[2];
     __shared__ int s_prefix[P2_PREFIX_CAP_K];
     __shared__ int s_gb[P2_PREFIX_CAP_K];
@@ -746,18 +854,22 @@
     ts_first(P.ts_start);
     unsigned long long clk_w0 = 0, clk_c0 = 0;
     if (!SAMPLE) clk_begin(P.ts_end_cell ? P.ts_start : nullptr, clk_w0, clk_c0);
+    if (threadIdx.x < 2) sCk[threadIdx.x] = 0u;
     P2Queue<SAMPLE, 2, 64 * P2_WAVES, P2_PREFIX_CAP_K> queue{P, s_item, s_prefix, s_gb};
     queue.init();
     P2Item item;
     while (queue.next(item)) {
         const int b = item.b, cbt0 = item.cbt0, ch = item.ch, m_use = item.m_use, nt = item.nt;
-#define P2_CASE(N) case N: { Tile2<N, SAMPLE> it{P, (unsigned)reinterpret_cast<uintptr_t>(ring), ring, sList, sThr, sPend}; it.run(b, cbt0, ch, m_use, nt, queue); break; }
+#define P2_CASE(N) case N: { Tile2<N, SAMPLE> it{P, (unsigned)reinterpret_cast<uintptr_t>(ring), ring, sList, sThr, sPend, sThr2, sCkW, sCk}; it.run(b, cbt0, ch, m_use, nt, queue); break; }
         switch (item.ncb_tile) {
             P2_CASE(1) P2_CASE(2) P2_CASE(3) P2_CASE(4) P2_CASE(5) P2_CASE(6)
             P2_CASE(7) P2_CASE(8) P2_CASE(9) P2_CASE(10) P2_CASE(11)
-            default: { Tile2<12, SAMPLE> it{P, (unsigned)reinterpret_cast<uintptr_t>(ring), ring, sList, sThr, sPend}; it.run(b, cbt0, ch, m_use, nt, queue); break; }
+            default: { Tile2<12, SAMPLE> it{P, (unsigned)reinterpret_cast<uintptr_t>(ring), ring, sList, sThr, sPend, sThr2, sCkW, sCk}; it.run(b, cbt0, ch, m_use, nt, queue); break; }
         }
 #undef P2_CASE
+    }
+    if (CKK && P.ck_stats) {
+        if (threadIdx.x < 2 && sCk[threadIdx.x]) atomicAdd(P.ck_stats + threadIdx.x, (unsigned long long)sCk[threadIdx.x]);
     }
     if (!SAMPLE) clk_end(P.ts_end_cell ? P.ts_start : nullptr, ST_P2, clk_w0, clk_c0);
 #ifdef LMI_P2_ENDS
diff --git a/learnedmetricindex_amd/csrc/lmi_prefilter.h b/learnedmetricindex_amd/csrc/lmi_prefilter.h
--- a/learnedmetricindex_amd/csrc/lmi_prefilter.h
+++ b/learnedmetricindex_amd/csrc/lmi_prefilter.h
@@ -74,31 +74,36 @@
 
 __device__ __forceinline__ float norm_guard(int d) { return 1.0001f + (float)d * 5.96046448e-8f; }
 
-__device__ __forceinline__ void row_norms(const float* __restrict__ x, int d, float s, float guard, float& best, float& bestd) {
-    float acc = 0.0f, dl = 0.0f;
+__device__ __forceinline__ void row_norms(const float* __restrict__ x, int d, float s, float guard, int ksuf, float& best, float& bestd, float& bests) {
+    float acc = 0.0f, dl = 0.0f, suf = 0.0f;
     for (int k = 0; k < d; ++k) {
         const float xs = x[k] * s;
-        const float e = (float)(_Float16)xs - xs;
+        const float h = (float)(_Float16)xs;
+        const float e = h - xs;
         acc += xs * xs;
         dl += e * e;
+        if (k >= ksuf) suf += h * h;
     }
     best = fmaxf(best, sqrtf(acc) * guard);
     bestd = fmaxf(bestd, sqrtf(dl) * guard);
+    bests = fmaxf(bests, sqrtf(suf) * guard);
 }
 
 __global__ void bucket_norm_kernel(const float* __restrict__ rows, int d, int pitch, const int* __restrict__ rb_start,
                                    const int* __restrict__ nb_rows, const float* __restrict__ scale,
-                                   unsigned* __restrict__ bnorm_bits, unsigned* __restrict__ bdelta_bits) {
+                                   unsigned* __restrict__ bnorm_bits, unsigned* __restrict__ bdelta_bits,
+                                   int ksuf, unsigned* __restrict__ bsuf_bits) {
     const int b = blockIdx.y;
     const int n_b = nb_rows[b];
     const float s = scale[0];
     const float guard = norm_guard(d);
-    float best = 0.0f, bestd = 0.0f;
+    float best = 0.0f, bestd = 0.0f, bests = 0.0f;
     for (int row = blockIdx.x * blockDim.x + threadIdx.x; row < n_b; row += gridDim.x * blockDim.x) {
-        row_norms(rows + ((size_t)rb_start[b] * 32 + row) * pitch, d, s, guard, best, bestd);
+        row_norms(rows + ((size_t)rb_start[b] * 32 + row) * pitch, d, s, guard, ksuf, best, bestd, bests);
     }
     if (best > 0.0f) atomicMax(bnorm_bits + b, __float_as_uint(best));
     if (bestd > 0.0f) atomicMax(bdelta_bits + b, __float_as_uint(bestd));
+    if (bests > 0.0f) atomicMax(bsuf_bits + b, __float_as_uint(bests));
 }
 
 __global__ void pf_selftest_kernel(int* __restrict__ ok) {
@@ -287,6 +292,11 @@
     const int* redo_bucket;
     const unsigned char* redo_col;
     OverflowLog x;
+    const unsigned* xsuf;
+    const float* csuf;
+    int ck_stage;
+    int ck_mode;
+    unsigned long long* ck_stats;
 };
 __device__ __forceinline__ void cand_store(const PrefilterParams& P, size_t col, unsigned pos, unsigned row, float s) {
     if (__builtin_expect(pos < (unsigned)PF_CAP, 1)) {
```

Result: no change. 2.103 million, median of 6 (+0.7%).
